# kjenike/panagram

Measured on AMD Instinct MI355X. Metric: anchored k-mers/sec building pan-kmer bitmap, higher is better.
Workload: dtype u64

## Files before the change

### panagram_amd/csrc/pg_anchor.hip

```cpp
#include "pg_kernels.h"

#ifndef PG_ANCHOR_PART
#define PG_ANCHOR_PART -1
#endif
#define PG_HAS_PART(n) (PG_ANCHOR_PART == -1 || PG_ANCHOR_PART == (n))
#define PG_MAIN_PART (PG_ANCHOR_PART <= 0)
#if defined(PG_PHASE_TIMING) && PG_ANCHOR_PART != -1
#error "a -DPG_PHASE_TIMING build keeps its counters in one device variable: compile pg_anchor.hip as ONE unit (PG_ANCHOR_PART unset)"
#endif

namespace pg {

hipError_t probe_part0(hipStream_t s, uint32_t w, uint32_t ntiles, const SubTable &st, const uint64_t *seqw, const uint32_t *nmw, const uint32_t *has_n,
                       const SeqDesc *sd, const AnchorDesc *ad, const uint32_t *tile_contig, const uint32_t *sched, uint32_t tile_base, uint8_t *out1,
                       uint32_t nbytes, const RowCols &rc, int rowmode, const FuseArgs *fuse);
hipError_t probe_part1(hipStream_t s, uint32_t w, uint32_t ntiles, const SubTable &st, const uint64_t *seqw, const uint32_t *nmw, const uint32_t *has_n,
                       const SeqDesc *sd, const AnchorDesc *ad, const uint32_t *tile_contig, const uint32_t *sched, uint32_t tile_base, uint8_t *out1,
                       uint32_t nbytes, const RowCols &rc, int rowmode, const FuseArgs *fuse);
hipError_t probe_part2(hipStream_t s, uint32_t w, uint32_t ntiles, const SubTable &st, const uint64_t *seqw, const uint32_t *nmw, const uint32_t *has_n,
                       const SeqDesc *sd, const AnchorDesc *ad, const uint32_t *tile_contig, const uint32_t *sched, uint32_t tile_base, uint8_t *out1,
                       uint32_t nbytes, const RowCols &rc, int rowmode, const FuseArgs *fuse);
hipError_t insert_part0(hipStream_t s, uint32_t win, uint32_t ntiles, const SubTable &st, int w, uint32_t bits, uint32_t count_mode, const uint64_t *seqw,
                        const uint32_t *nmw, const uint32_t *has_n, const SeqDesc *sd, const uint32_t *tile0, uint32_t ncontigs,
                        unsigned long long *counters, uint32_t max_probe);
hipError_t insert_part1(hipStream_t s, uint32_t win, uint32_t ntiles, const SubTable &st, int w, uint32_t bits, uint32_t count_mode, const uint64_t *seqw,
                        const uint32_t *nmw, const uint32_t *has_n, const SeqDesc *sd, const uint32_t *tile0, uint32_t ncontigs,
                        unsigned long long *counters, uint32_t max_probe);
hipError_t insert_part2(hipStream_t s, uint32_t win, uint32_t ntiles, const SubTable &st, int w, uint32_t bits, uint32_t count_mode, const uint64_t *seqw,
                        const uint32_t *nmw, const uint32_t *has_n, const SeqDesc *sd, const uint32_t *tile0, uint32_t ncontigs,
                        unsigned long long *counters, uint32_t max_probe);
hipError_t preload_part1();
hipError_t preload_part2();

constexpr int PROBE_SEQW = ((PROBE_TILE + 31) / 32 + 6 + 3) & ~3;
#ifndef PG_ABLATE
#define PG_ABLATE 0
#endif
constexpr uint32_t PROBE_SEQ_BASES = 32u * PROBE_SEQW;
#ifdef PG_PHASE_TIMING
__device__ unsigned long long pg_phase_cycles[1024 * 16];
#define PG_PH_DECL uint32_t ph_acc[12] = {0, 0, 0, 0, 0, 0, 0, 0, 0, 0, 0, 0}; uint32_t ph_t = (uint32_t)__builtin_readcyclecounter();
#define PG_PH(i) { const uint32_t ph_n = (uint32_t)__builtin_readcyclecounter(); ph_acc[i] += ph_n - ph_t; ph_t = ph_n; }
#define PG_PH_FLUSH { if (threadIdx.x == 0) { for (int ph_i = 0; ph_i < 9; ++ph_i) atomicAdd(&pg_phase_cycles[(blockIdx.x & 1023u) * 16u + ph_i], (unsigned long long)ph_acc[ph_i]); atomicAdd(&pg_phase_cycles[(blockIdx.x & 1023u) * 16u + 9], 1ull); atomicAdd(&pg_phase_cycles[(blockIdx.x & 1023u) * 16u + 10], (unsigned long long)ph_acc[10]); } }
#else
#define PG_PH_DECL
#define PG_PH(i)
#define PG_PH_FLUSH
#endif
__device__ __forceinline__ uint64_t revcomp_window(const uint64_t *rw, uint32_t p, uint64_t kmask, uint32_t rcb) {
    return extract_bases32(reinterpret_cast<const uint32_t *>(rw), rcb - p) & kmask;
}

__device__ __forceinline__ void stage_chunk(uint4 *line, uint32_t slot, int slots, const uint4 v) {
    uint2 *const p = reinterpret_cast<uint2 *>(line);
    p[slot] = make_uint2(v.x, v.y);
    p[slots + slot] = make_uint2(v.z, v.w);
}
template <bool TWO, int SLOTS>
__device__ __forceinline__ int scan_line_lds(const uint4 *line, uint64_t key, uint32_t &m0, uint32_t &m1) {
    uint64_t kk[SLOTS];
#pragma unroll
    for (int j = 0; j < SLOTS / 2; ++j) {
        const uint4 v = line[j];
        kk[2 * j] = (uint64_t)v.x | ((uint64_t)v.y << 32);
        kk[2 * j + 1] = (uint64_t)v.z | ((uint64_t)v.w << 32);
    }
    constexpr uint32_t SLOT_BYTES = 8u, MASK0 = 8u * SLOTS;
    m0 = m1 = 0;
    if constexpr (SLOTS == 8) {
        unsigned long long e[8];
#pragma unroll
        for (int sl = 0; sl < 8; ++sl) e[sl] = __builtin_amdgcn_ballot_w64(kk[sl] == key);
        const unsigned long long b0 = e[1] | e[3] | e[5] | e[7], b1 = e[2] | e[3] | e[6] | e[7], b2 = e[4] | e[5] | e[6] | e[7];
        const unsigned long long any = b0 | b1 | b2 | e[0];
        const bool hit = __builtin_amdgcn_inverse_ballot_w64(any);
#if PG_ABLATE == 6
        if (hit) m0 = (uint32_t)b0 | 1u;
        return hit ? 1 : (kk[SLOTS - 1] == EMPTY_KEY ? 0 : -1);
#elif PG_ABLATE == 7
        m0 = (uint32_t)(kk[0] ^ kk[1] ^ kk[2] ^ kk[3] ^ kk[4] ^ kk[5] ^ kk[6] ^ kk[7]) | 1u;
        return (kk[0] ^ kk[3]) == key ? -1 : 1;
#endif
        if (hit) {
            const uint32_t off = (__builtin_amdgcn_inverse_ballot_w64(b0) ? SLOT_BYTES : 0u) | (__builtin_amdgcn_inverse_ballot_w64(b1) ? 2u * SLOT_BYTES : 0u) |
                                 (__builtin_amdgcn_inverse_ballot_w64(b2) ? 4u * SLOT_BYTES : 0u);
            if constexpr (TWO) {
                const uint2 mk = *reinterpret_cast<const uint2 *>(reinterpret_cast<const uint8_t *>(line) + off + MASK0);
                m0 = mk.x;
                m1 = mk.y;
            } else {
                m0 = *reinterpret_cast<const uint32_t *>(reinterpret_cast<const uint8_t *>(line) + off + MASK0);
            }
        }
        return hit ? 1 : (kk[SLOTS - 1] == EMPTY_KEY ? 0 : -1);
    } else {
        int hit = -1;
#pragma unroll
        for (int sl = 0; sl < SLOTS; ++sl) hit = (kk[sl] == key) ? sl : hit;
        if (hit >= 0) {
            const uint2 mk = *reinterpret_cast<const uint2 *>(reinterpret_cast<const uint8_t *>(line) + (uint32_t)hit * SLOT_BYTES + MASK0);
            m0 = mk.x;
            if (TWO) m1 = mk.y;
        }
        return hit >= 0 ? 1 : (kk[SLOTS - 1] == EMPTY_KEY ? 0 : -1);
    }
}


template <bool TWO, int SLOTS>
__device__ __forceinline__ int scan_line_global(const SubTable &st, uint32_t b, uint64_t key, uint32_t &m0, uint32_t &m1) {
    const uint4 *line = reinterpret_cast<const uint4 *>(st.buckets + (uint64_t)b * (16 * SLOTS));
    uint4 v[SLOTS];
#pragma unroll
    for (int sl = 0; sl < SLOTS; ++sl) v[sl] = line[sl];
    m0 = m1 = 0;
#pragma unroll
    for (int sl = 0; sl < SLOTS; ++sl) {
        const uint64_t kk = (uint64_t)v[sl].x | ((uint64_t)v[sl].y << 32);
        const bool hit = (kk == key);
        m0 = hit ? v[sl].z : m0;
        if (TWO) m1 = hit ? v[sl].w : m1;
    }
    const uint64_t last = (uint64_t)v[SLOTS - 1].x | ((uint64_t)v[SLOTS - 1].y << 32);
    return (m0 | m1) ? 1 : (last == EMPTY_KEY ? 0 : -1);
}

template <bool TWO, int SLOTS>
__device__ __forceinline__ void lane_chase(const SubTable &st, uint64_t key, uint32_t level, uint32_t b, uint32_t step,
                                           uint32_t &m0, uint32_t &m1) {
    for (uint64_t n = 0; n < st.nbuckets + GROUP_CHAIN; ++n) {
        if (scan_line_global<TWO, SLOTS>(st, b, key, m0, m1) >= 0) return;
        level = min(level + 1, GROUP_CHAIN + 1);
        advance_line(key, level, st.nbuckets, b, step);
    }
    m0 = m1 = 0;
}

template <bool FIRST = false>
__device__ __forceinline__ int scan_keys16_lds(const uint4 *line, uint64_t key, uint32_t &slot1) {
    uint64_t kk[16];
#pragma unroll
    for (int c = 0; c < 8; ++c) {
        const uint4 v = line[c];
        kk[2 * c] = (uint64_t)v.x | ((uint64_t)v.y << 32);
        kk[2 * c + 1] = (uint64_t)v.z | ((uint64_t)v.w << 32);
    }
    unsigned long long e[16];
#pragma unroll
    for (int sl = 0; sl < 16; ++sl) e[sl] = __builtin_amdgcn_ballot_w64(kk[sl] == key);
    if constexpr (FIRST) {
        unsigned long long seen = e[0];
#pragma unroll
        for (int sl = 1; sl < 16; ++sl) {
            const unsigned long long m = e[sl];
            e[sl] = m & ~seen;
            seen |= m;
        }
    }
    unsigned long long b[4] = {0, 0, 0, 0}, any = e[0];
#pragma unroll
    for (int sl = 1; sl < 16; ++sl) {
        any |= e[sl];
#pragma unroll
        for (int bit = 0; bit < 4; ++bit)
            if (sl & (1 << bit)) b[bit] |= e[sl];
    }
    const bool hit = __builtin_amdgcn_inverse_ballot_w64(any);
    slot1 = 0;
    if (hit)
        slot1 = 1u + ((__builtin_amdgcn_inverse_ballot_w64(b[0]) ? 1u : 0u) | (__builtin_amdgcn_inverse_ballot_w64(b[1]) ? 2u : 0u) |
                      (__builtin_amdgcn_inverse_ballot_w64(b[2]) ? 4u : 0u) | (__builtin_amdgcn_inverse_ballot_w64(b[3]) ? 8u : 0u));
    return hit ? 1 : (kk[15] == EMPTY_KEY ? 0 : -1);
}

__device__ __forceinline__ void lane_chase_wide(const SubTable &st, uint64_t key, uint32_t level, uint32_t b, uint32_t step,
                                                uint32_t &hline, uint32_t &slot1) {
    hline = slot1 = 0;
    for (uint64_t n = 0; n < st.nbuckets + GROUP_CHAIN; ++n) {
        const uint4 *line = reinterpret_cast<const uint4 *>(st.buckets + (uint64_t)b * (8u * SPLIT_KEYS));
        uint4 v[8];
#pragma unroll
        for (int c = 0; c < 8; ++c) v[c] = line[c];
        uint32_t found = 0;
#pragma unroll
        for (int c = 0; c < 8; ++c) {
            if (((uint64_t)v[c].x | ((uint64_t)v[c].y << 32)) == key) found = 2 * c + 1;
            if (((uint64_t)v[c].z | ((uint64_t)v[c].w << 32)) == key) found = 2 * c + 2;
        }
        if (found) {
            hline = b;
            slot1 = found;
            return;
        }
        if (((uint64_t)v[7].z | ((uint64_t)v[7].w << 32)) == EMPTY_KEY) return;
        level = min(level + 1, GROUP_CHAIN + 1);
        advance_line(key, level, st.nbuckets, b, step);
    }
}

template <int NW>
struct __attribute__((packed, aligned(4))) WordsN {
    uint32_t w[NW];
};
template <int NW, bool NT = false>
__device__ __forceinline__ void copy_words(const uint32_t *src, uint8_t *dst, bool hit) {
    WordsN<NW> v;
#pragma unroll
    for (int i = 0; i < NW; ++i) v.w[i] = 0;
    if (hit) v = *reinterpret_cast<const WordsN<NW> *>(src);
    if constexpr (NW == 4 && NT) {
        typedef uint32_t u32x4 __attribute__((ext_vector_type(4)));
        u32x4 q = {v.w[0], v.w[1], v.w[2], v.w[3]};
        __builtin_nontemporal_store(q, reinterpret_cast<u32x4 *>(dst));
    } else {
        *reinterpret_cast<WordsN<NW> *>(dst) = v;
    }
}
template <int NS>
__device__ __forceinline__ void copy_words_tail(const uint32_t *src, uint8_t *dst, bool hit, uint32_t tail) {
    WordsN<NS + 1> v;
#pragma unroll
    for (int i = 0; i <= NS; ++i) v.w[i] = 0;
    if (hit) v = *reinterpret_cast<const WordsN<NS + 1> *>(src);
    if constexpr (NS > 0) {
        WordsN<NS> o;
#pragma unroll
        for (int i = 0; i < NS; ++i) o.w[i] = v.w[i];
        *reinterpret_cast<WordsN<NS> *>(dst) = o;
    }
    if (NS > 0 && tail > 1) {
        struct __attribute__((packed)) U32 { uint32_t v; };
        reinterpret_cast<U32 *>(dst + 4 * NS + tail - 4)->v = __builtin_amdgcn_alignbit(v.w[NS], v.w[NS > 0 ? NS - 1 : 0], 8u * tail);
    } else {
        for (uint32_t bb = 0; bb < tail; ++bb) dst[4 * NS + bb] = (uint8_t)(v.w[NS] >> (8 * bb));
    }
}
__device__ __forceinline__ void store_row_wide(const uint8_t *masks, uint32_t W, uint32_t nbytes, uint8_t *row, uint32_t hline,
                                               uint32_t slot1) {
    const bool hit = slot1 != 0;
    const uint32_t *mp = reinterpret_cast<const uint32_t *>(masks) + ((uint64_t)hline * SPLIT_KEYS + (slot1 - 1u)) * W;
    uint32_t d = 0;
    const uint32_t full = nbytes / 4;
    const uint32_t tail = nbytes % 4;
    if (nbytes == 16) {
        copy_words<4, true>(mp, row, hit);
        return;
    }
    for (; d + 4 <= full; d += 4) copy_words<4>(mp + d, row + 4 * d, hit);
    if (!tail) {
        if (full - d == 3) copy_words<3>(mp + d, row + 4 * d, hit);
        else if (full - d == 2) copy_words<2>(mp + d, row + 4 * d, hit);
        else if (full - d == 1) copy_words<1>(mp + d, row + 4 * d, hit);
    } else {
        if (full - d == 3) copy_words_tail<3>(mp + d, row + 4 * d, hit, tail);
        else if (full - d == 2) copy_words_tail<2>(mp + d, row + 4 * d, hit, tail);
        else if (full - d == 1) copy_words_tail<1>(mp + d, row + 4 * d, hit, tail);
        else copy_words_tail<0>(mp + d, row + 4 * d, hit, tail);
    }
}

__device__ __forceinline__ int scan_keys_inl(const uint4 *line, uint64_t key, uint32_t S, uint32_t &slot1) {
    uint64_t kk[6];
#pragma unroll
    for (int c = 0; c < 3; ++c) {
        const uint4 v = line[c];
        kk[2 * c] = (uint64_t)v.x | ((uint64_t)v.y << 32);
        kk[2 * c + 1] = (uint64_t)v.z | ((uint64_t)v.w << 32);
    }
    const bool six = S >= 6u;
    slot1 = (six && kk[5] == key) ? 6u : 0u;
#pragma unroll
    for (int sl = 4; sl >= 0; --sl) slot1 = (kk[sl] == key) ? (uint32_t)(sl + 1) : slot1;
    const uint64_t last = six ? kk[5] : kk[4];
    return slot1 ? 1 : (last == EMPTY_KEY ? 0 : -1);
}
__device__ __forceinline__ void masks_inl(const uint4 *line, uint32_t S, uint32_t W, uint32_t slot, uint32_t (&w)[4]) {
    const WordsN<4> v = *reinterpret_cast<const WordsN<4> *>(reinterpret_cast<const uint8_t *>(line) + 8u * S + 4u * W * slot);
    w[0] = v.w[0], w[1] = v.w[1], w[2] = v.w[2], w[3] = v.w[3];
}
template <int NS>
__device__ __forceinline__ void store_words_tail(const uint32_t (&v)[4], uint8_t *dst, uint32_t tail) {
    if (NS == 3 && tail == 0) {
        typedef uint32_t u32x3 __attribute__((ext_vector_type(3), aligned(4)));
        u32x3 q = {v[0], v[1], v[2]};
        __builtin_nontemporal_store(q, reinterpret_cast<u32x3 *>(dst));
        return;
    }
    WordsN<NS> o;
#pragma unroll
    for (int i = 0; i < NS; ++i) o.w[i] = v[i];
    *reinterpret_cast<WordsN<NS> *>(dst) = o;
    if (tail > 1) {
        struct __attribute__((packed)) U32 { uint32_t v; };
        reinterpret_cast<U32 *>(dst + 4 * NS + tail - 4)->v = __builtin_amdgcn_alignbit(v[NS & 3], v[NS - 1], 8u * tail);
    } else if (tail == 1) {
        dst[4 * NS] = (uint8_t)v[NS & 3];
    }
}
__device__ __forceinline__ void store_row_regs(uint8_t *row, uint32_t nbytes, const uint32_t (&w)[4]) {
    if (nbytes == 16) {
        typedef uint32_t u32x4 __attribute__((ext_vector_type(4)));
        u32x4 q = {w[0], w[1], w[2], w[3]};
        __builtin_nontemporal_store(q, reinterpret_cast<u32x4 *>(row));
    } else if (nbytes >= 12) {
        store_words_tail<3>(w, row, nbytes - 12u);
    } else {
        store_words_tail<2>(w, row, nbytes - 8u);
    }
}
__device__ __forceinline__ void store_row_fused(uint8_t *row, uint32_t nbytes, const uint32_t (&w)[4], uint32_t nxt) {
    const uint32_t t = nbytes & 3u;
    const uint32_t keep = (1u << (8u * t)) - 1u;
    typedef uint32_t u32x4u __attribute__((ext_vector_type(4), aligned(1)));
    typedef uint32_t u32x3u __attribute__((ext_vector_type(3), aligned(1)));
    if (nbytes > 12u) {
        u32x4u q = {w[0], w[1], w[2], (w[3] & keep) | (nxt << (8u * t))};
        __builtin_nontemporal_store(q, reinterpret_cast<u32x4u *>(row));
    } else {
        u32x3u q = {w[0], w[1], (w[2] & keep) | (nxt << (8u * t))};
        __builtin_nontemporal_store(q, reinterpret_cast<u32x3u *>(row));
    }
}
__device__ __forceinline__ void lane_chase_inl(const SubTable &st, uint64_t key, uint32_t level, uint32_t b, uint32_t step, uint32_t (&w)[4]) {
// ... 157 lines not shown
        __syncthreads();
        if (level > LEVELS) {
            for (uint32_t e = lane; e < qn; e += 64) {
                uint32_t m0, m1;
                const uint64_t key = canonical_from_le(extract_bases(sw, q_pl[e]), k);
                if constexpr (WIDE && INL) {
                    uint32_t rw4[4];
                    lane_chase_inl(st, key, (uint32_t)level, q_line[e], q_step[e], rw4);
                    if (rw4[0] | rw4[1] | rw4[2] | rw4[3]) store_row_regs(tile_rows + (uint64_t)q_pl[e] * nbytes, nbytes, rw4);
                } else if constexpr (WIDE) {
                    lane_chase_wide(st, key, (uint32_t)level, q_line[e], q_step[e], m0, m1);
                    if (m1) store_row_wide(st.masks, st.W, nbytes, tile_rows + (uint64_t)q_pl[e] * nbytes, m0, m1);
                } else {
                    lane_chase<TWO, SLOTS>(st, key, (uint32_t)level, q_line[e], q_step[e], m0, m1);
                    if constexpr (ROWMODE == 3) cols_or_position(reinterpret_cast<unsigned long long *>(tile_rows), q_pl[e], m0);
                    else if (m0 | m1) store_row<ROWMODE>(tile_rows + (uint64_t)q_pl[e] * nbytes, m0, m1, rc);
                }
            }
            break;
        }
        uint32_t kept = 0;
        for (uint32_t i0 = 0; i0 < qn; i0 += 64) {
            const uint32_t e = i0 + lane;
            const bool act = e < qn;
            const uint32_t ec = act ? e : qn - 1;
            uint32_t line = q_line[ec], step = q_step[ec];
            if (GROUP_CHAIN > 1 && level == 1) {
                step = step_of_group(step, st.nbuckets);
                line = next_line(line, step, st.nbuckets);
            }
            const uint32_t pl = q_pl[ec];
            const uint64_t kmask = kmer_mask(k);
            const uint64_t X = extract_bases32(reinterpret_cast<const uint32_t *>(sw), pl) & kmask;
            const uint64_t key = canonical_from_xb(X, revcomp_window(rw, pl, kmask, PROBE_SEQ_BASES - (uint32_t)k), k);
            const uint32_t prev_line = lane_up1(line);
            const bool leader = act && (lane == 0 || line != prev_line);
            const unsigned long long lmask = __builtin_amdgcn_ballot_w64(leader);
            const uint32_t rid = lanes_le_index(lmask, 0u);
            const uint32_t nruns = (uint32_t)__popcll(lmask);
            uint32_t m0 = 0, m1 = 0;
            [[maybe_unused]] uint32_t rw4[4] = {0, 0, 0, 0};
            int rcode = 0;
            const uint32_t padline = lmask ? (uint32_t)__builtin_amdgcn_readlane((int)line, __builtin_ctzll(lmask)) : 0u;
            for (uint32_t r0 = 0; r0 < nruns; r0 += MAXRUN) {
                const uint32_t nl = min((uint32_t)MAXRUN, nruns - r0);
                if (lane < MAXRUN) lines_w[lane] = padline;
                if (leader && rid - r0 < nl) lines_w[rid - r0] = line;
                __syncthreads();
                uint4 v[STAGE_ITERS];
                uint32_t ln[STAGE_ITERS];
#pragma unroll
                for (int u = 0; u < STAGE_ITERS; ++u) ln[u] = lines_w[u * (64 / SLOTS) + lane / SLOTS];
#pragma unroll
                for (int u = 0; u < STAGE_ITERS; ++u) v[u] = *reinterpret_cast<const uint4 *>(chunk_base + (uint64_t)ln[u] * lbytes);
#pragma unroll
                for (int u = 0; u < STAGE_ITERS; ++u) {
                    const uint32_t idx = u * 64 + lane;
                    if constexpr (WIDE) buf[(idx / SLOTS) * LDS_LINE_U4 + (idx % SLOTS)] = v[u];
                    else stage_chunk(buf + (idx / SLOTS) * LDS_LINE_U4, idx % SLOTS, SLOTS, v[u]);
                }
                __syncthreads();
                if (act && rid - r0 < nl) {
                    if constexpr (WIDE && INL) {
                        rcode = scan_keys_inl(buf + (rid - r0) * LDS_LINE_U4, key, st.slots, m1);
                        if (m1) masks_inl(buf + (rid - r0) * LDS_LINE_U4, st.slots, st.W, m1 - 1u, rw4);
                    } else if constexpr (WIDE) {
                        rcode = scan_keys16_lds(buf + (rid - r0) * LDS_LINE_U4, key, m1);
                        m0 = line;
                    } else {
                        rcode = scan_line_lds<TWO, SLOTS>(buf + (rid - r0) * LDS_LINE_U4, key, m0, m1);
                    }
                }
                __syncthreads();
            }
            const bool again = act && rcode < 0;
            if constexpr (WIDE && INL) {
                if (act && m1) store_row_regs(tile_rows + (uint64_t)pl * nbytes, nbytes, rw4);
            } else if constexpr (WIDE) {
                if (act && m1) store_row_wide(st.masks, st.W, nbytes, tile_rows + (uint64_t)pl * nbytes, m0, m1);
            } else {
                if constexpr (ROWMODE == 3) {
                    if (act) cols_or_position(reinterpret_cast<unsigned long long *>(tile_rows), pl, m0);
                } else {
                    if (act && (m0 | m1)) store_row<ROWMODE>(tile_rows + (uint64_t)pl * nbytes, m0, m1, rc);
                }
            }
            const unsigned long long kmask2 = __builtin_amdgcn_ballot_w64(again);
            if (again) {
                const uint32_t slot = set_lane_index(kmask2, kept);
                uint32_t nl2 = line, ns2 = step;
                if constexpr (LEVELS + 1 < (int)GROUP_CHAIN) nl2 = next_line(line, step, st.nbuckets);
                else advance_line(key, (uint32_t)level + 1, st.nbuckets, nl2, ns2);
                q_line[slot] = nl2;
                q_step[slot] = ns2;
                q_pl[slot] = (uint16_t)pl;
            }
            kept += (uint32_t)__popcll(kmask2);
            __syncthreads();
        }
        qn = kept;
    }
}

#ifndef PG_FUSE_LOAD_SC1
#define PG_FUSE_LOAD_SC1 1
#endif
typedef const __attribute__((address_space(1))) uint8_t *GlobalBytes;
template <int NW>
__device__ __forceinline__ void fuse_load_row(GlobalBytes base, uint32_t off, uint32_t (&w)[NW]) {
    GlobalBytes p = base + off;
#if PG_FUSE_LOAD_SC1
#pragma unroll
    for (int i = 0; i + 1 < NW; i += 2) {
        const unsigned long long v = __hip_atomic_load(reinterpret_cast<const __attribute__((address_space(1))) unsigned long long *>(p + 4 * i), __ATOMIC_RELAXED,
                                                       __HIP_MEMORY_SCOPE_AGENT);
        w[i] = (uint32_t)v, w[i + 1] = (uint32_t)(v >> 32);
    }
    if constexpr (NW & 1)
        w[NW - 1] = __hip_atomic_load(reinterpret_cast<const __attribute__((address_space(1))) uint32_t *>(p + 4 * (NW - 1)), __ATOMIC_RELAXED, __HIP_MEMORY_SCOPE_AGENT);
#else
    const WordsN<NW> v = *reinterpret_cast<const __attribute__((address_space(1))) WordsN<NW> *>(p);
#pragma unroll
    for (int i = 0; i < NW; ++i) w[i] = v.w[i];
#endif
}
__device__ __forceinline__ void fuse_flush_word(const uint32_t (&pl)[5], uint32_t *out16, int lane) {
    uint32_t R[16];
#pragma unroll
    for (int q = 0; q < 8; ++q) {
        uint32_t v = 0;
#pragma unroll
        for (int i = 0; i < 5; ++i) v |= ((pl[i] >> q) & 0x01010101u) << i;
        R[2 * q] = v & 0x00FF00FFu;
        R[2 * q + 1] = (v >> 8) & 0x00FF00FFu;
    }
#define PG_XCHG(HALF, BIT)                                                  \
    {                                                                       \
        const bool up = (lane & BIT) != 0;                                  \
        _Pragma("unroll") for (int i = 0; i < HALF; ++i) {                  \
            const uint32_t send = up ? R[i] : R[i + HALF];                  \
            const uint32_t keep = up ? R[i + HALF] : R[i];                  \
            R[i] = keep + (uint32_t)__shfl_xor((int)send, BIT);             \
        }                                                                   \
    }
    PG_XCHG(8, 32)
    PG_XCHG(4, 16)
    PG_XCHG(2, 8)
    PG_XCHG(1, 4)
#undef PG_XCHG
    R[0] += (uint32_t)__shfl_xor((int)R[0], 2);
    R[0] += (uint32_t)__shfl_xor((int)R[0], 1);
    if ((lane & 3) == 0) {
        const uint32_t idx = (uint32_t)lane >> 2;
        out16[(idx >> 1) + ((idx & 1u) ? 8u : 0u)] = R[0];
    }
}
template <int NWP, bool LASTPASS>
__device__ __forceinline__ void tile_statistics_pass(uint32_t *Hc, GlobalBytes rs, uint32_t npos, uint32_t nbytes, uint32_t woff,
                                                     uint32_t keep_last, uint32_t split, uint32_t N, uint32_t (&pcs)[4], uint32_t *cs_out, int lane) {
    const uint32_t N1 = N + 1u;
    uint32_t ones[NWP], twos[NWP], fours[NWP], eights[NWP], sixteens[NWP], hold4[NWP], hold8[NWP];
#pragma unroll
    for (int w = 0; w < NWP; ++w) ones[w] = twos[w] = fours[w] = eights[w] = sixteens[w] = hold4[w] = hold8[w] = 0;
    uint32_t nx[4][NWP];
    auto request = [&](int g, uint32_t (&dst)[4][NWP]) __attribute__((always_inline)) {
#pragma unroll
        for (int i = 0; i < 4; ++i) {
            const uint32_t r = (uint32_t)(4 * g + i) * 64u + (uint32_t)lane;
            fuse_load_row<NWP>(rs, min(r, npos - 1u) * nbytes + woff, dst[i]);
        }
    };
    request(0, nx);
#pragma unroll
    for (int g = 0; g < 4; ++g) {
        uint32_t rw[4][NWP];
#pragma unroll
        for (int i = 0; i < 4; ++i)
#pragma unroll
            for (int w = 0; w < NWP; ++w) rw[i][w] = nx[i][w];
        if (g < 3) request(g + 1, nx);
        uint32_t pc4 = pcs[g];
#pragma unroll
        for (int i = 0; i < 4; ++i) {
            const uint32_t r = (uint32_t)(4 * g + i) * 64u + (uint32_t)lane;
            const uint32_t vmask = (uint32_t)((int32_t)(r - npos) >> 31);
            if (LASTPASS) rw[i][NWP - 1] &= keep_last;
            uint32_t pc = 0;
#pragma unroll
            for (int w = 0; w < NWP; ++w) {
                rw[i][w] &= vmask;
                pc += (uint32_t)__popc(rw[i][w]);
            }
            if (LASTPASS) {
                pc = min(pc + ((pc4 >> (8 * i)) & 0xFFu), N);
                const uint32_t idx = pc + (N1 & (uint32_t)((int32_t)(split - 1u - r) >> 31));
                atomicAdd(&Hc[idx], vmask & 1u);
            } else {
                pc4 += pc << (8 * i);
            }
        }
        if (!LASTPASS) pcs[g] = pc4;
#pragma unroll
        for (int w = 0; w < NWP; ++w) {
            uint32_t u = ones[w] ^ rw[0][w];
            const uint32_t c2a = (ones[w] & rw[0][w]) | (u & rw[1][w]);
            ones[w] = u ^ rw[1][w];
            u = ones[w] ^ rw[2][w];
            const uint32_t c2b = (ones[w] & rw[2][w]) | (u & rw[3][w]);
            ones[w] = u ^ rw[3][w];
            u = twos[w] ^ c2a;
            const uint32_t c4 = (twos[w] & c2a) | (u & c2b);
            twos[w] = u ^ c2b;
            if ((g & 1) == 0) {
                hold4[w] = c4;
            } else {
                u = fours[w] ^ hold4[w];
                const uint32_t c8 = (fours[w] & hold4[w]) | (u & c4);
                fours[w] = u ^ c4;
                if (g == 1) {
                    hold8[w] = c8;
                } else {
                    u = eights[w] ^ hold8[w];
                    sixteens[w] = (eights[w] & hold8[w]) | (u & c8);
                    eights[w] = u ^ c8;
                }
            }
        }
    }
#pragma unroll
    for (int w = 0; w < NWP; ++w) {
        const uint32_t pl[5] = {ones[w], twos[w], fours[w], eights[w], sixteens[w]};
        fuse_flush_word(pl, cs_out + 16 * w, lane);
    }
}

template <int NW>
__device__ __forceinline__ void tile_statistics(uint32_t *H, const uint8_t *tile_rows, uint32_t npos, uint32_t nbytes, const AnchorDesc &a,
                                                uint32_t tile_start, uint32_t tile, const FuseArgs &fo, int lane) {
    const uint32_t N = fo.ngenomes, N1 = N + 1u, hw = fo.hw;
    const uint32_t nh = 2u * N1;
#ifdef PG_PHASE_TIMING
    uint32_t tph[5] = {0, 0, 0, 0, 0}, tph_t = (uint32_t)__builtin_readcyclecounter();
#define PG_TPH(i) { const uint32_t n_ = (uint32_t)__builtin_readcyclecounter(); tph[i] += n_ - tph_t; tph_t = n_; }
#else
#define PG_TPH(i)
#endif
    __builtin_amdgcn_s_waitcnt(0x0F70);
    __syncthreads();
    PG_TPH(0)
    const uint64_t base = reinterpret_cast<uint64_t>(tile_rows);
    GlobalBytes rs = reinterpret_cast<GlobalBytes>(((uint64_t)(uint32_t)__builtin_amdgcn_readfirstlane((int)(uint32_t)(base >> 32)) << 32) |
                                                   (uint32_t)__builtin_amdgcn_readfirstlane((int)(uint32_t)base));
    const uint32_t r100 = (100u - tile_start % 100u) % 100u + 100u * (uint32_t)lane;
    const bool want100 = fo.out100 != nullptr && r100 < npos;
    uint32_t w100[NW];
    fuse_load_row<NW>(rs, min(r100, npos - 1u) * nbytes, w100);
    for (uint32_t i = lane; i < 4u * nh; i += 64) H[i] = 0;
    const uint64_t bin_end = ((uint64_t)(tile_start / a.binlen) + 1u) * a.binlen;
    const uint32_t split = (uint32_t)min((uint64_t)npos, bin_end - tile_start);
    const uint32_t keep = (nbytes & 3u) ? ((1u << (8u * (nbytes & 3u))) - 1u) : ~0u;
    uint32_t *const Hc = H + ((uint32_t)lane & 3u) * nh;
    uint32_t *cs_out = fo.tile_cs + (uint64_t)tile * fo.csw;
    uint32_t pcs[4] = {0, 0, 0, 0};
    __syncthreads();
    PG_TPH(1)
    if constexpr (NW <= 2) {
        tile_statistics_pass<NW, true>(Hc, rs, npos, nbytes, 0u, keep, split, N, pcs, cs_out, lane);
        PG_TPH(2)
    } else {
        tile_statistics_pass<2, false>(Hc, rs, npos, nbytes, 0u, ~0u, split, N, pcs, cs_out, lane);
        PG_TPH(2)
        tile_statistics_pass<NW - 2, true>(Hc, rs, npos, nbytes, 8u, keep, split, N, pcs, cs_out + 32, lane);
    }
    if (want100) {
        uint8_t *dst = fo.out100 + a.out100_off + (uint64_t)((tile_start + r100) / 100u) * nbytes;
#pragma unroll
        for (int i = 0; i < NW; ++i)
#pragma unroll
            for (int b = 0; b < 4; ++b)
                if ((uint32_t)(4 * i + b) < nbytes) dst[4 * i + b] = (uint8_t)(w100[i] >> (8 * b));
    }
    __syncthreads();
    PG_TPH(3)
    uint32_t *th = fo.tile_hist + (uint64_t)tile * hw;
    for (uint32_t i = lane; i < hw; i += 64) {
        const uint32_t lo = H[2u * i] + H[nh + 2u * i] + H[2u * nh + 2u * i] + H[3u * nh + 2u * i];
        const uint32_t hi = H[2u * i + 1u] + H[nh + 2u * i + 1u] + H[2u * nh + 2u * i + 1u] + H[3u * nh + 2u * i + 1u];
        th[i] = lo | (hi << 16);
    }
    PG_TPH(4)
#ifdef PG_PHASE_TIMING
    if (lane == 0)
        for (int i = 0; i < 5; ++i) atomicAdd(&pg_phase_cycles[(blockIdx.x & 1023u) * 16u + 11 + i], (unsigned long long)tph[i]);
#endif
#undef PG_TPH
}

template <bool TWO, int ROWMODE, int SLOTS, bool WIDE>
constexpr bool probe_pipelined = SLOTS == 8 && !WIDE && ROWMODE != 3 && (ROWMODE == 1 || ROWMODE >= 4 || TWO);
template <int W_C, bool TWO, int ROWMODE, int SLOTS, bool M64, bool WIDE = false, bool INL = false, bool FUSE = false>
__global__ __launch_bounds__(64, ((probe_pipelined<TWO, ROWMODE, SLOTS, WIDE> || INL || FUSE) ? 8 : 1))
__attribute__((amdgpu_num_sgpr(80))) void k_probe(const SubTable st, const uint64_t *__restrict__ seqw,
                                              const uint32_t *__restrict__ nmw, const uint32_t *__restrict__ has_n,
                                              const SeqDesc *__restrict__ sd, const AnchorDesc *__restrict__ ad,
                                              const uint32_t *__restrict__ tile_contig,
                                              const uint32_t *__restrict__ sched, uint32_t tile_base,
                                              uint8_t *__restrict__ out1, uint32_t nbytes, const RowCols rc, const FuseArgs fo) {
    constexpr int LDS_LINE_U4 = SLOTS + 1;
    constexpr int MAXRUN = PROBE_MAXRUN;
    constexpr int STAGE_ITERS = (MAXRUN * SLOTS + 63) / 64;
    constexpr int BUF_U4 = ((STAGE_ITERS * 64 + SLOTS - 1) / SLOTS) * LDS_LINE_U4;
    constexpr int OFF_RW = PROBE_SEQW * 8, OFF_NW = OFF_RW + (PROBE_SEQW + 1) * 8, OFF_LW = OFF_NW + PROBE_SEQW * 4;
    constexpr int QCAP = PROBE_QCAP;
    constexpr int OFF_BUF = (OFF_LW + MAXRUN * 4 + 15) & ~15, OFF_QL = OFF_BUF + BUF_U4 * 16, OFF_QS = OFF_QL + QCAP * 4;
    constexpr int OFF_QP = OFF_QS + QCAP * 4, LDS_BYTES = OFF_QP + QCAP * 2;
    static_assert(OFF_LW <= 1020 || PROBE_TILE > 1024, "the sequence words must stay within reach of ds_read2_b32's offsets");
    __shared__ __attribute__((aligned(16))) uint8_t lds[LDS_BYTES];
    uint64_t *const sw = reinterpret_cast<uint64_t *>(lds);
    uint64_t *const rw = reinterpret_cast<uint64_t *>(lds + OFF_RW);
    uint32_t *const nw = reinterpret_cast<uint32_t *>(lds + OFF_NW);
    uint32_t(*const lines_w)[MAXRUN] = reinterpret_cast<uint32_t(*)[MAXRUN]>(lds + OFF_LW);
    uint4(*const buf)[BUF_U4] = reinterpret_cast<uint4(*)[BUF_U4]>(lds + OFF_BUF);
    uint32_t *const q_line = reinterpret_cast<uint32_t *>(lds + OFF_QL);
    uint32_t *const q_step = reinterpret_cast<uint32_t *>(lds + OFF_QS);
    uint16_t *const q_pl = reinterpret_cast<uint16_t *>(lds + OFF_QP);
    PG_PH_DECL
    const int lane = threadIdx.x;
    const int k = (int)st.k;
    if constexpr (W_C != 0) __builtin_assume(k >= 20 && k <= 32);
    const uint32_t tile = sched ? sched[blockIdx.x + tile_base] : blockIdx.x + tile_base;
    const uint32_t c = tile_contig[tile];
    const AnchorDesc a = ad[c];
    const SeqDesc s = sd[c];
    const uint32_t tile_start = (tile - a.tile0) * PROBE_TILE;
    const uint32_t npos = min((uint32_t)PROBE_TILE, a.nkmers - tile_start);
    const bool hasn = has_n[c] != 0;

    for (int i = lane; i < PROBE_SEQW; i += 64) {
        const uint64_t wi = (uint64_t)(tile_start >> 5) + i;
        const uint64_t wv = wi < s.nwords ? seqw[s.seq_off + wi] : 0ull;
        sw[i] = wv;
        rw[PROBE_SEQW - 1 - i] = pair_reverse64(~wv);
        nw[i] = (hasn && wi < s.nwords) ? nmw[s.seq_off + wi] : 0u;
    }
    if (lane == 0) rw[PROBE_SEQW] = 0;
    __syncthreads();

    const uint64_t kmask = W_C ? (((uint64_t)(k == 32 ? ~0u : ((1u << (2 * k - 32)) - 1u)) << 32) | 0xFFFFFFFFull) : kmer_mask(k);
    const uint32_t rcb = PROBE_SEQ_BASES - (uint32_t)k;
    constexpr int HALO = W_C ? W_C - 1 : 0;
    constexpr bool CARRY = W_C >= 2;
    constexpr bool CUT = W_C != 0;
    const uint32_t m = W_C ? (uint32_t)k - W_C + 1 : 0;
    const uint64_t mm64 = (m >= 32) ? ~0ull : ((1ull << (2 * (m ? m : 1))) - 1);
    __shared__ unsigned long long cols[ROWMODE == 3 ? TILE_SLOTS * COLS_G : 1];
    if constexpr (ROWMODE == 3) {
        for (uint32_t i = lane; i < TILE_SLOTS * COLS_G; i += 64) cols[i] = 0;
        __syncthreads();
    }
#if PG_ABLATE == 9 || PG_ABLATE == 10
    uint8_t *tile_rows = out1 + (uint64_t)(blockIdx.x & 255u) * PROBE_TILE * nbytes;
#else
    uint8_t *tile_rows = ROWMODE == 3 ? reinterpret_cast<uint8_t *>(cols) : out1 + a.out_off + (uint64_t)tile_start * nbytes;
#endif
    uint32_t qn = 0;

    const uint8_t *chunk_base = st.buckets + (uint32_t)(lane % SLOTS) * 16u;
    const uint32_t lbytes = INL ? st.layout * 64u : st.slots * (WIDE ? 8u : 16u);

    struct Front {
        uint64_t key;
        uint32_t grp, line, rid, nruns, padline;
        uint32_t adv;
        uint32_t ln[STAGE_ITERS];
        unsigned long long rmask, amask, lmask;
    };
    auto carry_at = [&](const uint32_t b0) __attribute__((always_inline)) {
        uint32_t y = ~0u;
        if constexpr (CARRY) {
            const uint32_t q = b0 + (uint32_t)min(lane, HALO - 1);
            const uint64_t fa = extract_bases32(reinterpret_cast<const uint32_t *>(sw), q) & mm64;
            const uint64_t fr = extract_bases32(reinterpret_cast<const uint32_t *>(rw), PROBE_SEQ_BASES - q - m) & mm64;
            const uint32_t h = M64 ? mmer_rank(fa < fr ? fa : fr) : mz_order(min((uint32_t)fa, (uint32_t)fr));
            y = h;
        }
        return y;
    };
    uint32_t carry = ~0u;
    auto front = [&](const uint32_t b0) __attribute__((always_inline)) {
        Front f;
        const int32_t pl = (int32_t)(b0 + lane);
        f.rmask = __builtin_amdgcn_ballot_w64(pl < (int32_t)npos);
        const uint32_t pq = (uint32_t)pl;
        const uint64_t X = extract_bases32(reinterpret_cast<const uint32_t *>(sw), pq) & kmask;
        const uint64_t B = revcomp_window(rw, pq, kmask, rcb);
        f.key = ~(X > B ? X : B) & kmask;
        f.amask = f.rmask;
        if (hasn) f.amask &= __builtin_amdgcn_ballot_w64(extract_nmask(nw, pq, k) == 0);
        [[maybe_unused]] uint32_t own = 0;
        if (W_C) {
            constexpr uint32_t off = (uint32_t)HALO;
            if constexpr (!M64) {
                const uint32_t mm32 = (uint32_t)mm64;
                const uint32_t fa = __builtin_amdgcn_alignbit((uint32_t)(X >> 32), (uint32_t)X, 2 * off) & mm32;
                const uint32_t fr = __builtin_amdgcn_alignbit((uint32_t)(B >> 32), (uint32_t)B, 2 * (HALO - off)) & mm32;
                f.grp = mz_order(min(fa, fr));
            } else {
                const uint64_t fa = (X >> (2 * off)) & mm64;
                const uint64_t fr = (B >> (2 * (HALO - off))) & mm64;
                f.grp = mmer_rank(fa < fr ? fa : fr);
            }
#ifdef PG_DUMMY_VALU
            {
                uint32_t dm = f.grp;
#pragma unroll
                for (int i = 0; i < PG_DUMMY_VALU; ++i) asm volatile("v_alignbit_b32 %0, %0, %1, 3" : "+v"(dm) : "v"((uint32_t)lane));
                if (dm == 0x12345u && lane == 77) out1[0] = 1;
            }
#endif
            if constexpr (CARRY) {
                own = f.grp;
                uint32_t suffix = __builtin_amdgcn_inverse_ballot_w64((1ull << HALO) - 1ull) ? carry : ~0u;
                f.grp = sliding_min_suffix<W_C >= 2 ? W_C : 2>(f.grp, suffix);
                f.grp = min(f.grp, suffix);
            } else {
                f.grp = sliding_min<W_C ? W_C : 1>(f.grp);
            }
        } else {
            f.grp = group_of_key(f.key);
        }
        f.line = home_of_group(f.grp, st.nbuckets);
        f.lmask = f.amask & (~(f.amask << 1) | differs_from_lane_below(f.line));
        f.rid = run_ids(f.lmask);
        uint32_t lanes_kept = 64u;
        if constexpr (CUT) {
            const unsigned long long keep = __builtin_amdgcn_sicmp((int32_t)f.rid, MAXRUN, 40 );
            f.amask &= keep;
            f.rmask &= keep;
            f.lmask &= keep;
            lanes_kept = (uint32_t)__popcll(keep);
        }
        f.adv = lanes_kept;
        if constexpr (CARRY) {
            carry = (uint32_t)__builtin_amdgcn_ds_bpermute((int)(((uint32_t)lane << 2) + ((lanes_kept - HALO) << 2)), (int)own);
        }
        f.nruns = (uint32_t)__popcll(f.lmask);
        int first_run;
        asm("s_ff1_i32_b64 %0, %1" : "=s"(first_run) : "s"(f.lmask));
        f.padline = (uint32_t)__builtin_amdgcn_readlane((int)f.line, first_run & 63);
#if PG_ABLATE == 3
        if (f.line != 0xDEADBEEFu) f.nruns = 0;
#endif
        const bool leader = __builtin_amdgcn_inverse_ballot_w64(f.lmask);
        if (lane < MAXRUN) lines_w[0][lane] = f.padline;
        if (leader && f.rid < (uint32_t)MAXRUN) lines_w[0][f.rid] = f.line;
        __syncthreads();
#pragma unroll
        for (int it = 0; it < STAGE_ITERS; ++it) f.ln[it] = lines_w[0][it * (64 / SLOTS) + lane / SLOTS];
        return f;
    };
    struct Lines {
        uint4 v[STAGE_ITERS];
    };
    auto issue = [&](const Front &f, const uint32_t r0) __attribute__((always_inline)) {
        Lines L;
        uint32_t ln[STAGE_ITERS];
        if (r0 != 0u) {
            const uint32_t nl = min((uint32_t)MAXRUN, f.nruns - r0);
            const bool leader = __builtin_amdgcn_inverse_ballot_w64(f.lmask);
            if (lane < MAXRUN) lines_w[0][lane] = f.padline;
            if (leader && f.rid - r0 < nl) lines_w[0][f.rid - r0] = f.line;
            __syncthreads();
        }
#pragma unroll
        for (int it = 0; it < STAGE_ITERS; ++it) {
            if (r0 != 0u) ln[it] = lines_w[0][it * (64 / SLOTS) + lane / SLOTS];
            else ln[it] = f.ln[it];
#if PG_ABLATE == 1
            ln[it] &= 511u;
#endif
        }
#pragma unroll
        for (int it = 0; it < STAGE_ITERS; ++it) L.v[it] = *reinterpret_cast<const uint4 *>(chunk_base + (uint64_t)ln[it] * lbytes);
        return L;
    };
    auto back = [&](const Front &f, const Lines &L, const uint32_t b0, auto &&after_staging) __attribute__((always_inline)) {
        const bool act = __builtin_amdgcn_inverse_ballot_w64(f.amask), inrange = __builtin_amdgcn_inverse_ballot_w64(f.rmask);
        const int32_t pl = (int32_t)(b0 + lane);
        uint32_t m0 = 0, m1 = 0;
        [[maybe_unused]] uint32_t rw4[4] = {0, 0, 0, 0};
        int rcode = 0;
        auto stage = [&](const Lines &S) __attribute__((always_inline)) {
            uint4 *const mine = buf[0] + ((uint32_t)lane / SLOTS) * LDS_LINE_U4;
#pragma unroll
            for (int it = 0; it < STAGE_ITERS; ++it) {
                if constexpr (WIDE) mine[it * (64 / SLOTS) * LDS_LINE_U4 + ((uint32_t)lane % SLOTS)] = S.v[it];
                else stage_chunk(mine + it * (64 / SLOTS) * LDS_LINE_U4, (uint32_t)lane % SLOTS, SLOTS, S.v[it]);
            }
            __syncthreads();
        };
        auto scan = [&](const uint32_t r0) __attribute__((always_inline)) {
            const uint32_t nl = min((uint32_t)MAXRUN, f.nruns - r0);
#if PG_ABLATE == 5
            if (act && f.rid - r0 < nl) {
                rcode = 1;
                m0 = m1 = reinterpret_cast<const uint32_t *>(buf[0] + (f.rid - r0) * LDS_LINE_U4)[2];
            }
#else
            if (act && f.rid - r0 < nl) {
                if constexpr (WIDE && INL) {
                    rcode = scan_keys_inl(buf[0] + (f.rid - r0) * LDS_LINE_U4, f.key, st.slots, m1);
                    if (m1) masks_inl(buf[0] + (f.rid - r0) * LDS_LINE_U4, st.slots, st.W, m1 - 1u, rw4);
                } else if constexpr (WIDE) {
                    rcode = scan_keys16_lds(buf[0] + (f.rid - r0) * LDS_LINE_U4, f.key, m1);
                    m0 = f.line;
                } else {
                    rcode = scan_line_lds<TWO, SLOTS>(buf[0] + (f.rid - r0) * LDS_LINE_U4, f.key, m0, m1);
                }
            }
#endif
            __syncthreads();
        };
        PG_PH(1)
        __builtin_amdgcn_s_waitcnt(0x0F70);
        PG_PH(2)
        stage(L);
        PG_PH(3)
        after_staging();
        PG_PH(4)
        scan(0u);
        PG_PH(5)
        if constexpr (!CUT)
        for (uint32_t r0 = MAXRUN; r0 < f.nruns; r0 += MAXRUN) {
            const Lines X = issue(f, r0);
            __builtin_amdgcn_s_waitcnt(0x0F70);
            stage(X);
            scan(r0);
        }
        const unsigned long long omask = f.amask & __builtin_amdgcn_sicmp(rcode, 0, 40);
        const bool ovf = __builtin_amdgcn_inverse_ballot_w64(omask);
        if (omask) {
            uint32_t step, nx;
            if constexpr (GROUP_CHAIN == 1) {
                key_sequence(f.key, st.nbuckets, nx, step);
            } else {
                step = f.grp;
                nx = f.line;
            }
            const uint32_t slot = set_lane_index(omask, qn);
            if (ovf) {
                q_line[slot] = nx;
                q_step[slot] = step;
                q_pl[slot] = (uint16_t)pl;
            }
            qn += (uint32_t)__popcll(omask);
        }
        PG_PH(10)
        if constexpr (WIDE && INL) {
            const bool fuse = (nbytes & 3u) != 0u && b0 + (uint32_t)__popcll(f.rmask) < npos;
            if (fuse) {
                const uint32_t mine = inrange ? rw4[0] : 0u;
                const uint32_t nxt = (uint32_t)__builtin_amdgcn_update_dpp(0, (int)mine, 0x130 , 0xf, 0xf, true);
                if (inrange) store_row_fused(tile_rows + (uint64_t)(uint32_t)pl * nbytes, nbytes, rw4, nxt);
            } else if (inrange) {
                store_row_regs(tile_rows + (uint64_t)(uint32_t)pl * nbytes, nbytes, rw4);
            }
        } else if constexpr (WIDE) {
#if PG_ABLATE == 2
            if (inrange && m0 == 0xDEADBEEFu && m1 == 77u)
#elif PG_ABLATE == 8 || PG_ABLATE == 10
            if (m1) m0 = 0, m1 = 1;
            if (inrange)
#else
            if (st.W == 4u && (nbytes & 3u) != 0u && b0 + (uint32_t)__popcll(f.rmask) < npos) {
                uint32_t v4[4] = {0, 0, 0, 0};
                if (inrange && m1) {
                    const WordsN<4> g = *reinterpret_cast<const WordsN<4> *>(reinterpret_cast<const uint32_t *>(st.masks) + ((uint64_t)m0 * SPLIT_KEYS + (m1 - 1u)) * 4u);
                    v4[0] = g.w[0], v4[1] = g.w[1], v4[2] = g.w[2], v4[3] = g.w[3];
                }
                const uint32_t nxt = (uint32_t)__builtin_amdgcn_update_dpp(0, (int)v4[0], 0x130 , 0xf, 0xf, true);
                if (inrange) store_row_fused(tile_rows + (uint64_t)(uint32_t)pl * nbytes, nbytes, v4, nxt);
            } else if (inrange)
#endif
                store_row_wide(st.masks, st.W, nbytes, tile_rows + (uint64_t)(uint32_t)pl * nbytes, m0, m1);
        } else if constexpr (ROWMODE == 3) {
            const uint32_t w0 = b0 >> 6, sh = b0 & 63u;
            for (uint32_t j = 0; j < rc.col0; ++j) {
                const unsigned long long shifted = __ballot(inrange && ((m0 >> j) & 1u));
                if (lane == 0 && shifted) {
                    cols[w0 * COLS_G + j] |= shifted << sh;
                    if (sh && (shifted >> (64u - sh))) cols[(w0 + 1) * COLS_G + j] |= shifted >> (64u - sh);
                }
            }
        } else {
            if (ROWMODE == 6 && b0 + (uint32_t)__popcll(f.rmask) < npos) {
                const uint32_t mine = inrange ? m0 : 0u;
                const uint32_t nxt = (uint32_t)__builtin_amdgcn_update_dpp(0, (int)mine, 0x130 , 0xf, 0xf, true);
                struct __attribute__((packed)) U32 { uint32_t v; };
                if (inrange) reinterpret_cast<U32 *>(tile_rows + (uint32_t)pl * 3u)->v = (m0 & 0xFFFFFFu) | (nxt << 24);
            } else if constexpr (ROWMODE == 6) {
                const uint32_t nxt = (uint32_t)__builtin_amdgcn_update_dpp(0, (int)m0, 0x130 , 0xf, 0xf, false);
                const uint32_t o4 = (uint32_t)reinterpret_cast<uintptr_t>(tile_rows) & 3u;
                const uint32_t j = ((uint32_t)pl - o4) & 3u;
                const uint32_t lo = (nxt << 24) | (m0 & 0xFFFFFFu);
                const uint32_t dw = __builtin_amdgcn_alignbit(nxt >> 8, lo, 8u * j);
                const unsigned long long nextin = f.rmask >> 1;
                const unsigned long long dmask = f.rmask & nextin & __builtin_amdgcn_ballot_w64(j != 3u);
                const unsigned long long fmask = f.rmask & (1ull | ~nextin);
                uint8_t *row = tile_rows + (uint32_t)pl * 3u;
                if (__builtin_amdgcn_inverse_ballot_w64(dmask)) *reinterpret_cast<uint32_t *>(row + j) = dw;
                if (__builtin_amdgcn_inverse_ballot_w64(fmask)) store_row<ROWMODE>(row, m0, m1, rc);
            } else
#if PG_ABLATE == 2
            if (inrange && m0 == 0xDEADBEEFu)
#else
            if (ROWMODE == 0 && TWO && rc.words == 3u && nbytes >= 5u && b0 + (uint32_t)__popcll(f.rmask) < npos) {
                const uint32_t mine = inrange ? m0 : 0u;
                const uint32_t nxt = (uint32_t)__builtin_amdgcn_update_dpp(0, (int)mine, 0x130 , 0xf, 0xf, true);
                if (inrange) {
                    typedef uint32_t u32x2u __attribute__((ext_vector_type(2), aligned(1)));
                    const uint32_t t8 = 8u * (nbytes - 4u);
                    u32x2u q = {m0, (m1 & ((1u << t8) - 1u)) | (nxt << t8)};
                    *reinterpret_cast<u32x2u *>(tile_rows + (uint32_t)pl * nbytes) = q;
                }
            } else if (inrange)
#endif
                store_row<ROWMODE>(tile_rows + (ROWMODE == 1 ? (uint32_t)pl : ROWMODE == 4 ? (uint32_t)pl * 4u : ROWMODE == 5 ? (uint32_t)pl * 2u : ROWMODE == 6 ? (uint32_t)pl * 3u : (uint32_t)pl * nbytes), m0, m1, rc);
        }
        PG_PH(6)
    };
    constexpr bool PIPE = probe_pipelined<TWO, ROWMODE, SLOTS, WIDE>;
    constexpr int LEVELS = (W_C >= 6 && !TWO && !WIDE && PROBE_STAGED_LEVELS > 1) ? 1 : PROBE_STAGED_LEVELS;
    static_assert(QCAP >= 128, "an early drain must leave room for a batch");
    constexpr uint32_t QROOM = QCAP - 64;
    uint32_t b0 = 0;
    if constexpr (PIPE) {
        Lines L;
#pragma unroll
        for (int it = 0; it < STAGE_ITERS; ++it) L.v[it] = make_uint4(0, 0, 0, 0);
        PG_PH(0)
        carry = carry_at(0u);
        Front cur = front(0u);
        L = issue(cur, 0u);
        for (;;) {
            PG_PH(7)
            const uint32_t b1 = b0 + cur.adv;
            const bool more = b1 < npos;
            Front nxt = cur;
            __builtin_amdgcn_sched_barrier(0);
            if (more) nxt = front(b1);
            __builtin_amdgcn_sched_barrier(0);
            back(cur, L, b0, [&]() __attribute__((always_inline)) {
                if (more) L = issue(nxt, 0u);
            });
            __builtin_amdgcn_sched_barrier(0);
            b0 = b1;
            if (!more || qn > QROOM) break;
            cur = nxt;
        }
    } else {
        {
            carry = carry_at(0u);
            const Front f = front(0u);
            const Lines L = issue(f, 0u);
            back(f, L, 0u, [] {});
            b0 = f.adv;
        }
        while (b0 < npos && qn <= QROOM) {
            const Front f = front(b0);
            const Lines L = issue(f, 0u);
            back(f, L, b0, [] {});
            b0 += f.adv;
        }
    }
    PG_PH(7)
    for (;;) {
        drain_queue<TWO, ROWMODE, SLOTS, MAXRUN, WIDE, LEVELS, INL>(st, qn, sw, rw, q_line, q_step, q_pl, lines_w[0], buf[0], tile_rows, nbytes, rc, lane);
        qn = 0;
        if (b0 >= npos) break;
        __syncthreads();
        carry = carry_at(b0);
        while (b0 < npos && qn <= QROOM) {
            const Front f = front(b0);
            const Lines L = issue(f, 0u);
            back(f, L, b0, [] {});
            b0 += f.adv;
        }
    }
    PG_PH(8)
    PG_PH_FLUSH
    if constexpr (FUSE) {
        static_assert(ROWMODE != 1 && ROWMODE != 3 && LDS_BYTES >= 4 * 4 * 2 * 129, "fused statistics: rows of 2..16 bytes; four copies of 2 x 129 histogram counters in LDS");
        const AnchorDesc *ad2 = ad;
        const uint32_t *tc2 = tile_contig, *sched2 = sched;
        asm volatile("" : "+s"(ad2), "+s"(tc2), "+s"(sched2));
        const uint32_t tile2 = sched2 ? sched2[blockIdx.x + tile_base] : blockIdx.x + tile_base;
        const AnchorDesc a2 = ad2[tc2[tile2]];
        if (a2.binlen >= (uint32_t)PROBE_TILE) {
            const uint32_t ts2 = (tile2 - a2.tile0) * PROBE_TILE;
            const uint32_t np2 = min((uint32_t)PROBE_TILE, a2.nkmers - ts2);
            const uint8_t *rows2 = out1 + a2.out_off + (uint64_t)ts2 * nbytes;
            uint32_t *H = reinterpret_cast<uint32_t *>(lds);
            if constexpr (WIDE) {
                if (nbytes <= 12u) tile_statistics<3>(H, rows2, np2, nbytes, a2, ts2, tile2, fo, lane);
                else tile_statistics<4>(H, rows2, np2, nbytes, a2, ts2, tile2, fo, lane);
            } else {
                tile_statistics<TWO ? 2 : 1>(H, rows2, np2, nbytes, a2, ts2, tile2, fo, lane);
            }
        }
    }
    if constexpr (ROWMODE == 3) {
        __syncthreads();
        const uint32_t width = nbytes, trel = tile - tile_base;
        unsigned long long *dst = reinterpret_cast<unsigned long long *>(out1) + (uint64_t)trel * TILE_SLOTS * width;
        for (uint32_t i = lane; i < TILE_SLOTS * width; i += 64) dst[i] = cols[(i / width) * COLS_G + i % width];
    }
}

constexpr int INSERT_QCAP = 256;

template <bool COUNT, bool CLAIM = true>
__device__ __forceinline__ int wave_insert_batch(const SubTable &st, bool valid, uint64_t key, uint32_t grp, int w, uint32_t bits,
                                                 uint32_t max_probe, int lane) {
    const uint32_t kstride = key_stride(st), slots = st.slots;
    uint32_t b = home_of_group(grp, st.nbuckets), step = step_of_group(grp, st.nbuckets), probes = 0;
    int s = -1;
    bool done = !valid, fresh = false;
    int r = 0;
    auto shfl64 = [](uint64_t v, int src) __attribute__((always_inline)) {
        return (uint64_t)(uint32_t)__shfl((int)(uint32_t)v, src) | ((uint64_t)(uint32_t)__shfl((int)(uint32_t)(v >> 32), src) << 32);
    };
    auto resolve = [&](uint32_t sl, bool claimed) __attribute__((always_inline)) {
        uint32_t *mp = mask_ptr(st, b, sl, (uint32_t)w);
        if (COUNT) {
            if (*mp < 0xFFFFFF00u) atomicAdd(mp, bits);
        } else if (claimed) {
            *reinterpret_cast<volatile uint32_t *>(mp) = bits;
        } else {
            const uint32_t cur = *mp;
            if ((cur & bits) != bits) *reinterpret_cast<volatile uint32_t *>(mp) = cur | bits;
        }
        r = claimed ? 1 : 0;
        done = true;
    };
    while (__ballot(!done)) {
        if (!done && s >= (int)slots) {
            if (++probes >= max_probe) {
                done = true;
                r = -1;
            } else {
                advance_line(key, probes, st.nbuckets, b, step);
                s = -1;
            }
        }
        if (!done && s < 0) {
            uint8_t *base = st.buckets + (uint64_t)b * line_bytes(st);
            int hit = -1, fr = -1;
            for (uint32_t s0 = 0; s0 < slots; s0 += 8) {
                uint64_t kk[8];
#pragma unroll
                for (int i = 0; i < 8; ++i) {
                    kk[i] = __hip_atomic_load(reinterpret_cast<unsigned long long *>(base + kstride * (s0 + i)), __ATOMIC_RELAXED,
                                              __HIP_MEMORY_SCOPE_AGENT);
                    if (s0 + (uint32_t)i >= slots) kk[i] = TOMB_KEY;
                }
                int h8 = -1, f8 = -1;
#pragma unroll
                for (int i = 7; i >= 0; --i) {
                    h8 = (kk[i] == key) ? i : h8;
                    f8 = (kk[i] == EMPTY_KEY) ? i : f8;
                }
                if (hit < 0 && h8 >= 0) hit = (int)s0 + h8;
                if (fr < 0 && f8 >= 0) fr = (int)s0 + f8;
            }
            if (hit >= 0) resolve((uint32_t)hit, false);
            else if (!CLAIM && fr >= 0) done = true;
            else {
                s = fr >= 0 ? fr : (int)slots;
                fresh = true;
            }
        }
        if constexpr (!CLAIM) continue;
        if (!COUNT) {
            const bool sp = !done && fresh && s < (int)slots;
            const unsigned long long spmask = __ballot(sp);
            if (spmask) {
                const uint64_t gaddr = sp ? reinterpret_cast<uint64_t>(key_ptr(st, b, (uint32_t)s)) : 0;
                const uint64_t gprev = (uint64_t)(uint32_t)__shfl_up((int)(uint32_t)gaddr, 1) | ((uint64_t)(uint32_t)__shfl_up((int)(uint32_t)(gaddr >> 32), 1) << 32);
                const bool gl = sp && (lane == 0 || gprev != gaddr);
                const unsigned long long glmask = __ballot(gl);
                const unsigned long long below = glmask & ((2ull << lane) - 1ull);
                const int g0 = below ? 63 - __builtin_clzll(below) : lane;
                const unsigned long long ends = (glmask | ~spmask) & ~((2ull << g0) - 1ull);
                const int gend = ends ? __builtin_ctzll(ends) : 64;
                const uint32_t mm = sp ? min((uint32_t)(gend - g0), slots - (uint32_t)s) : 0u;
                const int t = s + (lane - g0);
                const bool part = sp && t < (int)slots;
                uint64_t content = 0;
                bool won = false;
                if (part) {
                    const unsigned long long cur = atomicCAS(key_ptr(st, b, (uint32_t)t), (unsigned long long)EMPTY_KEY, (unsigned long long)key);
                    won = cur == EMPTY_KEY;
                    content = won ? key : cur;
                }
                int pos = -1;
                for (uint32_t i = 0; i < slots; ++i) {
                    const uint64_t c = shfl64(content, min(g0 + (int)i, 63));
                    if (i < mm && pos < 0 && c == key) pos = s + (int)i;
                }
                if (sp) {
                    if (pos >= 0) {
                        const bool mine = part && won && pos == t;
                        if (part && won && pos != t) *reinterpret_cast<volatile unsigned long long *>(key_ptr(st, b, (uint32_t)t)) = TOMB_KEY;
                        resolve((uint32_t)pos, mine);
                    } else {
                        s += (int)mm;
                    }
                }
            }
        }
        fresh = false;
        const bool want = !done && s >= 0 && s < (int)slots;
        unsigned long long *kp = want ? key_ptr(st, b, (uint32_t)s) : nullptr;
        const uint64_t addr = reinterpret_cast<uint64_t>(kp);
        const uint64_t prev = (uint64_t)(uint32_t)__shfl_up((int)(uint32_t)addr, 1) | ((uint64_t)(uint32_t)__shfl_up((int)(uint32_t)(addr >> 32), 1) << 32);
        const bool leader = want && (lane == 0 || prev != addr);
        uint64_t content = 0;
        bool won = false;
        if (leader) {
            const unsigned long long cur = atomicCAS(kp, (unsigned long long)EMPTY_KEY, (unsigned long long)key);
            won = cur == EMPTY_KEY;
            content = won ? key : cur;
        }
        const unsigned long long lmask = __builtin_amdgcn_ballot_w64(leader);
        if (__ballot(want)) {
            const unsigned long long below = lmask & ((2ull << lane) - 1ull);
            const int mine = below ? 63 - __builtin_clzll(below) : lane;
            const uint64_t got = (uint64_t)(uint32_t)__shfl((int)(uint32_t)content, mine) | ((uint64_t)(uint32_t)__shfl((int)(uint32_t)(content >> 32), mine) << 32);
            if (want) {
                if (got == key) resolve((uint32_t)s, leader && won);
                else ++s;
            }
        }
    }
    return r;
}

template <int W_C, bool M64>
__global__ __launch_bounds__(64) void k_insert_tile(const SubTable st, int w, uint32_t bits, uint32_t count_mode,
                                                    const uint64_t *__restrict__ seqw, const uint32_t *__restrict__ nmw,
                                                    const uint32_t *__restrict__ has_n, const SeqDesc *__restrict__ sd,
                                                    const uint32_t *__restrict__ tile0, uint32_t ncontigs,
                                                    unsigned long long *__restrict__ counters, uint32_t max_probe) {
    constexpr int SLOTS = 8;
    constexpr int LDS_LINE_U4 = SLOTS + 1;
    constexpr int STAGE_ITERS = (PROBE_MAXRUN * SLOTS + 63) / 64;
    __shared__ uint64_t sw[PROBE_SEQW];
    __shared__ uint64_t rw[PROBE_SEQW + 1];
    __shared__ uint32_t nw[PROBE_SEQW];
    __shared__ uint32_t lines_w[PROBE_MAXRUN];
    __shared__ uint4 buf[((STAGE_ITERS * 64 + SLOTS - 1) / SLOTS) * LDS_LINE_U4];
    __shared__ uint32_t q_grp[INSERT_QCAP];
    __shared__ uint16_t q_pl[INSERT_QCAP];
    const int lane = threadIdx.x;
    const int k = (int)st.k;
    const bool split = st.layout == LAYOUT_SPLIT;
    const bool update_only = (count_mode & 2u) != 0;
    count_mode &= 1u;
    const uint32_t tile = blockIdx.x;
    uint32_t c = 0;
    {
        uint32_t lo = 0, hi = ncontigs;
        while (hi - lo > 1) {
            const uint32_t mid = (lo + hi) >> 1;
            if (tile0[mid] <= tile) lo = mid;
            else hi = mid;
        }
        c = lo;
    }
    const SeqDesc s = sd[c];
    const uint32_t nkmers = (uint32_t)(s.len - (uint64_t)k + 1);
    const uint32_t tile_start = (tile - tile0[c]) * PROBE_TILE;
    const uint32_t npos = min((uint32_t)PROBE_TILE, nkmers - tile_start);
    const bool hasn = has_n[c] != 0;
    for (int i = lane; i < PROBE_SEQW; i += 64) {
        const uint64_t wi = (uint64_t)(tile_start >> 5) + i;
        const uint64_t wv = wi < s.nwords ? seqw[s.seq_off + wi] : 0ull;
        sw[i] = wv;
        rw[PROBE_SEQW - 1 - i] = pair_reverse64(~wv);
        nw[i] = (hasn && wi < s.nwords) ? nmw[s.seq_off + wi] : 0u;
    }
    if (lane == 0) rw[PROBE_SEQW] = 0;
    __syncthreads();
    const uint64_t kmask = W_C ? (((uint64_t)(k == 32 ? ~0u : ((1u << (2 * k - 32)) - 1u)) << 32) | 0xFFFFFFFFull) : kmer_mask(k);
    const uint32_t rcb = PROBE_SEQ_BASES - (uint32_t)k;
    constexpr int HALO = W_C ? W_C - 1 : 0;
    constexpr int STRIDE = 64 - HALO;
    const uint32_t m = W_C ? (uint32_t)k - W_C + 1 : 0;
    const uint64_t mm64 = (m >= 32) ? ~0ull : ((1ull << (2 * (m ? m : 1))) - 1);
    uint32_t qn = 0, claimed = 0;
    bool overflowed = false;

    auto drain = [&]() {
        __syncthreads();
        for (uint32_t e0 = 0; e0 < qn; e0 += 64) {
            const uint32_t e = e0 + lane;
            const bool valid = e < qn;
            const uint32_t ec = valid ? e : qn - 1;
            const uint64_t key = canonical_from_le(extract_bases32(reinterpret_cast<const uint32_t *>(sw), q_pl[ec]), k);
            const int r = update_only ? wave_insert_batch<false, false>(st, valid, key, q_grp[ec], w, bits, max_probe, lane)
                          : count_mode ? wave_insert_batch<true>(st, valid, key, q_grp[ec], w, bits, max_probe, lane)
                                       : wave_insert_batch<false>(st, valid, key, q_grp[ec], w, bits, max_probe, lane);
            overflowed |= __ballot(r < 0) != 0;
            claimed += (uint32_t)__popcll(__ballot(r > 0));
        }
        qn = 0;
        __syncthreads();
    };

    uint32_t adv = STRIDE;
    for (uint32_t b = 0; b < npos; b += adv) {
        const int32_t pl = (int32_t)(b + lane) - HALO;
        const bool inrange = pl >= (int32_t)b && pl < (int32_t)npos;
        const uint32_t pq = (uint32_t)max(pl, 0);
        const uint64_t X = extract_bases32(reinterpret_cast<const uint32_t *>(sw), pq) & kmask;
        const uint64_t B = revcomp_window(rw, pq, kmask, rcb);
        const uint64_t key = ~(X > B ? X : B) & kmask;
        bool act = inrange;
        if (hasn) act = act && (extract_nmask(nw, pq, k) == 0);
        uint32_t grp;
        if (W_C) {
            const uint32_t off = (uint32_t)(pl + HALO) - pq;
            if constexpr (!M64) {
                const uint32_t mm32 = (uint32_t)mm64;
                const uint32_t fa = __builtin_amdgcn_alignbit((uint32_t)(X >> 32), (uint32_t)X, 2 * off) & mm32;
                const uint32_t fr = __builtin_amdgcn_alignbit((uint32_t)(B >> 32), (uint32_t)B, 2 * (HALO - off)) & mm32;
                grp = mz_order(min(fa, fr));
            } else {
                const uint64_t fa = (X >> (2 * off)) & mm64;
                const uint64_t fr = (B >> (2 * (HALO - off))) & mm64;
                grp = mmer_rank(fa < fr ? fa : fr);
            }
            grp = sliding_min<W_C ? W_C : 1>(grp);
        } else {
            grp = group_of_key(key);
        }
        const uint32_t line = home_of_group(grp, st.nbuckets);
        const uint32_t prev_line = lane_up1(line);
        unsigned long long amask = __builtin_amdgcn_ballot_w64(act);
        unsigned long long lmask = amask & (~(amask << 1) | __builtin_amdgcn_ballot_w64(line != prev_line));
        const uint32_t rid = lanes_le_index(lmask, 0u);
        if constexpr (W_C != 0) {
            const unsigned long long keep = __builtin_amdgcn_sicmp((int32_t)rid, PROBE_MAXRUN, 40 );
            amask &= keep;
            lmask &= keep;
            act = __builtin_amdgcn_inverse_ballot_w64(amask);
            adv = (uint32_t)__popcll(keep) - HALO;
        }
        const bool leader = __builtin_amdgcn_inverse_ballot_w64(lmask);
        const uint32_t nruns = (uint32_t)__popcll(lmask);
        bool found = false, full = true;
        for (uint32_t r0 = 0; r0 < nruns; r0 += PROBE_MAXRUN) {
            const uint32_t nl = min((uint32_t)PROBE_MAXRUN, nruns - r0);
            if (leader && rid - r0 < nl) lines_w[rid - r0] = line;
            __syncthreads();
            uint4 v[STAGE_ITERS];
#pragma unroll
            for (int it = 0; it < STAGE_ITERS; ++it) {
                const uint32_t ls = min((uint32_t)(it * (64 / SLOTS) + lane / SLOTS), nl - 1u);
                v[it] = *reinterpret_cast<const uint4 *>(st.buckets + (((uint64_t)lines_w[ls] * 128u) | ((lane % SLOTS) * 16u)));
            }
#pragma unroll
            for (int it = 0; it < STAGE_ITERS; ++it) {
                const uint32_t idx = it * 64 + lane;
                buf[(idx / SLOTS) * LDS_LINE_U4 + (idx % SLOTS)] = v[it];
            }
            __syncthreads();
            if (act && rid - r0 < nl) {
                const uint4 *ln = buf + (rid - r0) * LDS_LINE_U4;
                uint32_t *mp = nullptr;
                uint32_t cur = 0;
                if (st.layout == LAYOUT_INLINE) {
                    uint32_t slot1;
                    full = scan_keys_inl(ln, key, st.slots, slot1) < 0;
                    if (slot1) {
                        found = true;
                        mp = mask_ptr(st, line, slot1 - 1u, (uint32_t)w);
                        cur = *reinterpret_cast<const volatile uint32_t *>(mp);
                    }
                } else if (split) {
                    uint32_t slot1;
                    full = scan_keys16_lds<true>(ln, key, slot1) < 0;
                    if (slot1) {
                        found = true;
                        mp = reinterpret_cast<uint32_t *>(st.masks) + ((uint64_t)line * SPLIT_KEYS + (slot1 - 1u)) * st.W + (uint32_t)w;
                        cur = *reinterpret_cast<const volatile uint32_t *>(mp);
                    }
                } else {
                    uint32_t m0, m1;
                    uint64_t kk[8];
#pragma unroll
                    for (int sl = 0; sl < 8; ++sl) kk[sl] = *reinterpret_cast<const uint64_t *>(ln + sl);
                    unsigned long long e[8];
#pragma unroll
                    for (int sl = 0; sl < 8; ++sl) e[sl] = __builtin_amdgcn_ballot_w64(kk[sl] == key);
                    {
                        unsigned long long seen = e[0];
#pragma unroll
                        for (int sl = 1; sl < 8; ++sl) {
                            const unsigned long long m = e[sl];
                            e[sl] = m & ~seen;
                            seen |= m;
                        }
                    }
                    const unsigned long long b0 = e[1] | e[3] | e[5] | e[7], b1 = e[2] | e[3] | e[6] | e[7], b2 = e[4] | e[5] | e[6] | e[7];
                    full = kk[7] != EMPTY_KEY;
                    (void)m0;
                    (void)m1;
                    if (__builtin_amdgcn_inverse_ballot_w64(b0 | b1 | b2 | e[0])) {
                        found = true;
                        const uint32_t off = (__builtin_amdgcn_inverse_ballot_w64(b0) ? 16u : 0u) | (__builtin_amdgcn_inverse_ballot_w64(b1) ? 32u : 0u) |
                                             (__builtin_amdgcn_inverse_ballot_w64(b2) ? 64u : 0u);
                        cur = *reinterpret_cast<const uint32_t *>(reinterpret_cast<const uint8_t *>(ln) + off + 8 + 4 * w);
                        mp = reinterpret_cast<uint32_t *>(st.buckets + (uint64_t)line * 128u + off + 8 + 4 * w);
                    }
                }
                if (found) {
                    if (count_mode) {
                        if (cur < 0xFFFFFF00u) atomicAdd(mp, bits);
                    } else if ((cur & bits) != bits) {
                        *reinterpret_cast<volatile uint32_t *>(mp) = cur | bits;
                    }
                }
            }
            __syncthreads();
        }
        const bool todo = act && !found && (!update_only || full);
        const unsigned long long tmask = __builtin_amdgcn_ballot_w64(todo);
        if (tmask) {
            if (qn + 64 > (uint32_t)INSERT_QCAP) drain();
            if (todo) {
                const uint32_t slot = lanes_le_index(tmask, qn);
                q_grp[slot] = grp;
                q_pl[slot] = (uint16_t)pl;
            }
            qn += (uint32_t)__popcll(tmask);
        }
    }
    if (qn) drain();
    if (lane == 0) {
        if (claimed) atomicAdd(&counters[0], (unsigned long long)claimed);
        if (overflowed) atomicOr(reinterpret_cast<unsigned int *>(&counters[1]), 1u);
    }
}

template <int W_C, bool TWO, int ROWMODE, int SLOTS>
static hipError_t probe_t(hipStream_t s, uint32_t ntiles, const SubTable &st, const uint64_t *seqw, const uint32_t *nmw,
                          const uint32_t *has_n, const SeqDesc *sd, const AnchorDesc *ad, const uint32_t *tile_contig,
                          const uint32_t *sched, uint32_t tile_base, uint8_t *out1, uint32_t nbytes, const RowCols &rc, const FuseArgs *fuse) {
    const bool m64 = W_C && st.m > 16;
    if constexpr (SLOTS == 8 && ROWMODE != 1 && ROWMODE != 3) {
        if (fuse) {
            if (m64)
                hipLaunchKernelGGL((k_probe<W_C, TWO, ROWMODE, SLOTS, true, false, false, true>), dim3(ntiles), dim3(64), 0, s, st, seqw, nmw, has_n, sd, ad,
                                   tile_contig, sched, tile_base, out1, nbytes, rc, *fuse);
            else
                hipLaunchKernelGGL((k_probe<W_C, TWO, ROWMODE, SLOTS, false, false, false, true>), dim3(ntiles), dim3(64), 0, s, st, seqw, nmw, has_n, sd, ad,
                                   tile_contig, sched, tile_base, out1, nbytes, rc, *fuse);
            return hipGetLastError();
        }
    }
    if (fuse) return hipErrorInvalidValue;
    const FuseArgs none = {nullptr, nullptr, nullptr, 0, 0, 0};
    if (m64)
        hipLaunchKernelGGL((k_probe<W_C, TWO, ROWMODE, SLOTS, true>), dim3(ntiles), dim3(64), 0, s, st, seqw, nmw, has_n, sd, ad,
                           tile_contig, sched, tile_base, out1, nbytes, rc, none);
    else
        hipLaunchKernelGGL((k_probe<W_C, TWO, ROWMODE, SLOTS, false>), dim3(ntiles), dim3(64), 0, s, st, seqw, nmw, has_n, sd, ad,
                           tile_contig, sched, tile_base, out1, nbytes, rc, none);
    return hipGetLastError();
}

template <int W_C>
static hipError_t probe_w(hipStream_t s, uint32_t ntiles, const SubTable &st, const uint64_t *seqw, const uint32_t *nmw,
                          const uint32_t *has_n, const SeqDesc *sd, const AnchorDesc *ad, const uint32_t *tile_contig,
                          const uint32_t *sched, uint32_t tile_base, uint8_t *out1, uint32_t nbytes, const RowCols &rc, int rowmode,
                          const FuseArgs *fuse = nullptr) {
#define PG_A s, ntiles, st, seqw, nmw, has_n, sd, ad, tile_contig, sched, tile_base, out1, nbytes, rc, fuse
#define PG_K s, st, seqw, nmw, has_n, sd, ad, tile_contig, sched, tile_base, out1, nbytes, rc
    const FuseArgs none = {nullptr, nullptr, nullptr, 0, 0, 0};
    const bool m64 = W_C && st.m > 16;
    if (st.layout == LAYOUT_INLINE || st.layout == LAYOUT_SPLIT) {
        const bool inl = st.layout == LAYOUT_INLINE;
        if (fuse && (nbytes > 16u || !PG_FUSE_WIDE)) return hipErrorInvalidValue;
        if (inl) {
            if (fuse) {
#if PG_FUSE_WIDE
                if (m64) hipLaunchKernelGGL((k_probe<W_C, false, 0, 8, true, true, true, true>), dim3(ntiles), dim3(64), 0, PG_K, *fuse);
                else hipLaunchKernelGGL((k_probe<W_C, false, 0, 8, false, true, true, true>), dim3(ntiles), dim3(64), 0, PG_K, *fuse);
#endif
            } else {
                if (m64) hipLaunchKernelGGL((k_probe<W_C, false, 0, 8, true, true, true>), dim3(ntiles), dim3(64), 0, PG_K, none);
                else hipLaunchKernelGGL((k_probe<W_C, false, 0, 8, false, true, true>), dim3(ntiles), dim3(64), 0, PG_K, none);
            }
        } else {
            if (fuse) {
#if PG_FUSE_WIDE
                if (m64) hipLaunchKernelGGL((k_probe<W_C, false, 0, 8, true, true, false, true>), dim3(ntiles), dim3(64), 0, PG_K, *fuse);
                else hipLaunchKernelGGL((k_probe<W_C, false, 0, 8, false, true, false, true>), dim3(ntiles), dim3(64), 0, PG_K, *fuse);
#endif
            } else {
                if (m64) hipLaunchKernelGGL((k_probe<W_C, false, 0, 8, true, true>), dim3(ntiles), dim3(64), 0, PG_K, none);
                else hipLaunchKernelGGL((k_probe<W_C, false, 0, 8, false, true>), dim3(ntiles), dim3(64), 0, PG_K, none);
            }
        }
        return hipGetLastError();
    }
    if (st.slots == 16) {
        if (st.W == 2) {
            if (rowmode == 2) return probe_t<W_C, true, 2, 16>(PG_A);
            return probe_t<W_C, true, 0, 16>(PG_A);
        }
        if (rowmode == 1) return probe_t<W_C, false, 1, 16>(PG_A);
        return probe_t<W_C, false, 0, 16>(PG_A);
    }
    if (st.W == 2) {
        if (rowmode == 2) return probe_t<W_C, true, 2, 8>(PG_A);
        return probe_t<W_C, true, 0, 8>(PG_A);
    }
    if (rowmode == 3) return probe_t<W_C, false, 3, 8>(PG_A);
    if (rowmode == 1) return probe_t<W_C, false, 1, 8>(PG_A);
    if (rowmode == 4) return probe_t<W_C, false, 4, 8>(PG_A);
    if (rowmode == 5) return probe_t<W_C, false, 5, 8>(PG_A);
    if (rowmode == 6) return probe_t<W_C, false, 6, 8>(PG_A);
    return probe_t<W_C, false, 0, 8>(PG_A);
#undef PG_A
#undef PG_K
}

template <int W_C>
static hipError_t insert_tiles_w(hipStream_t s, uint32_t ntiles, const SubTable &st, int w, uint32_t bits, uint32_t count_mode,
                                 const uint64_t *seqw, const uint32_t *nmw, const uint32_t *has_n, const SeqDesc *sd,
                                 const uint32_t *tile0, uint32_t ncontigs, unsigned long long *counters, uint32_t max_probe) {
    if (W_C && st.m > 16)
        hipLaunchKernelGGL((k_insert_tile<W_C, true>), dim3(ntiles), dim3(64), 0, s, st, w, bits, count_mode, seqw, nmw, has_n, sd,
                           tile0, ncontigs, counters, max_probe);
    else
        hipLaunchKernelGGL((k_insert_tile<W_C, false>), dim3(ntiles), dim3(64), 0, s, st, w, bits, count_mode, seqw, nmw, has_n, sd,
                           tile0, ncontigs, counters, max_probe);
    return hipGetLastError();
}

#define PG_PROBE_ARGS hipStream_t s, uint32_t w, uint32_t ntiles, const SubTable &st, const uint64_t *seqw, const uint32_t *nmw, const uint32_t *has_n, \
                      const SeqDesc *sd, const AnchorDesc *ad, const uint32_t *tile_contig, const uint32_t *sched, uint32_t tile_base, uint8_t *out1,          \
                      uint32_t nbytes, const RowCols &rc, int rowmode, const FuseArgs *fuse
#define PG_PROBE_CASE(W) case W: return probe_w<W>(s, ntiles, st, seqw, nmw, has_n, sd, ad, tile_contig, sched, tile_base, out1, nbytes, rc, rowmode, fuse);
#define PG_INSERT_ARGS hipStream_t s, uint32_t win, uint32_t ntiles, const SubTable &st, int w, uint32_t bits, uint32_t count_mode, const uint64_t *seqw, \
                       const uint32_t *nmw, const uint32_t *has_n, const SeqDesc *sd, const uint32_t *tile0, uint32_t ncontigs,                          \
                       unsigned long long *counters, uint32_t max_probe
#define PG_INSERT_CASE(W) case W: return insert_tiles_w<W>(s, ntiles, st, w, bits, count_mode, seqw, nmw, has_n, sd, tile0, ncontigs, counters, max_probe);
#if PG_HAS_PART(1)
hipError_t preload_part1() {
    hipFuncAttributes fa;
    return hipFuncGetAttributes(&fa, reinterpret_cast<const void *>(k_insert_tile<6, false>));
}
#endif
#if PG_HAS_PART(2)
hipError_t preload_part2() {
    hipFuncAttributes fa;
    return hipFuncGetAttributes(&fa, reinterpret_cast<const void *>(k_insert_tile<7, false>));
}
#endif
#if PG_HAS_PART(0)
hipError_t probe_part0(PG_PROBE_ARGS) {
    switch (w) { PG_PROBE_CASE(0) PG_PROBE_CASE(3) PG_PROBE_CASE(4) default: return hipErrorInvalidValue; }
}
hipError_t insert_part0(PG_INSERT_ARGS) {
    switch (win) { PG_INSERT_CASE(0) PG_INSERT_CASE(3) PG_INSERT_CASE(4) default: return hipErrorInvalidValue; }
}
#endif
#if PG_HAS_PART(1)
hipError_t probe_part1(PG_PROBE_ARGS) {
    switch (w) { PG_PROBE_CASE(5) PG_PROBE_CASE(6) default: return hipErrorInvalidValue; }
}
hipError_t insert_part1(PG_INSERT_ARGS) {
    switch (win) { PG_INSERT_CASE(5) PG_INSERT_CASE(6) default: return hipErrorInvalidValue; }
}
#endif
#if PG_HAS_PART(2)
hipError_t probe_part2(PG_PROBE_ARGS) {
    switch (w) { PG_PROBE_CASE(7) PG_PROBE_CASE(8) default: return hipErrorInvalidValue; }
}
hipError_t insert_part2(PG_INSERT_ARGS) {
    switch (win) { PG_INSERT_CASE(7) PG_INSERT_CASE(8) default: return hipErrorInvalidValue; }
}
#endif
#undef PG_PROBE_ARGS
#undef PG_PROBE_CASE
#undef PG_INSERT_ARGS
#undef PG_INSERT_CASE

#if PG_MAIN_PART
static hipError_t probe_window(hipStream_t s, uint32_t w, uint32_t ntiles, const SubTable &st, const uint64_t *seqw, const uint32_t *nmw,
                               const uint32_t *has_n, const SeqDesc *sd, const AnchorDesc *ad, const uint32_t *tile_contig, const uint32_t *sched,
                               uint32_t tile_base, uint8_t *out1, uint32_t nbytes, const RowCols &rc, int rowmode, const FuseArgs *fuse) {
    auto *part = (w == 0 || w == 3 || w == 4) ? probe_part0 : (w == 5 || w == 6) ? probe_part1 : (w == 7 || w == 8) ? probe_part2 : nullptr;
    if (!part) return hipErrorInvalidValue;
    return part(s, w, ntiles, st, seqw, nmw, has_n, sd, ad, tile_contig, sched, tile_base, out1, nbytes, rc, rowmode, fuse);
}

static int row_mode(uint32_t nbytes, const RowCols &rc) {
    if (nbytes == 1) return 1;
    if (nbytes == 8 && rc.col0 == 0 && rc.nb0 == 4 && rc.nb1 == 4) return 2;
    if (nbytes == 4 && rc.col0 == 0 && rc.nb0 == 4 && rc.nb1 == 0) return 4;
    if (nbytes == 2 && rc.col0 == 0 && rc.nb1 == 0) return 5;
    if (nbytes == 3 && rc.col0 == 0 && rc.nb1 == 0) return 6;
    return 0;
}

hipError_t launch_anchor(hipStream_t s, const TableDesc &T, const uint64_t *seqw, const uint32_t *nmw,
                         const uint32_t *has_n, const SeqDesc *sd, const AnchorDesc *ad, const uint32_t *tile_contig,
                         const uint32_t *sched, uint32_t tile_base, uint32_t ntiles, uint8_t *out1, uint64_t out1_bytes,
                         uint32_t columns_width, const FuseArgs *fuse) {
    if (ntiles == 0) return hipSuccess;
    const uint32_t nbytes = (T.ngenomes + 7) / 8;
    hipError_t e = hipSuccess;
    (void)out1_bytes;
    if (fuse && (columns_width || T.nsub != 1 || !fuse_rows_ok(nbytes) || fuse->ngenomes != T.ngenomes ||
                 (T.sub[0].layout == LAYOUT_SLOTS && T.sub[0].slots != 8)))
        return hipErrorInvalidValue;
    if (columns_width) {
        const SubTable &st = T.sub[0];
        if (T.nsub != 1 || st.layout != LAYOUT_SLOTS || st.W != 1 || st.slots != 8 || T.ngenomes > (uint32_t)COLS_G ||
            columns_width > (uint32_t)COLS_G || columns_width < T.ngenomes)
            return hipErrorInvalidValue;
        RowCols rc;
        rc.col0 = T.ngenomes;
        rc.nb0 = rc.nb1 = rc.words = 0;
        const uint32_t w = st.m ? st.k - st.m + 1 : 0;
        return probe_window(s, w, ntiles, st, seqw, nmw, has_n, sd, ad, tile_contig, sched, tile_base, out1, columns_width, rc, 3, nullptr);
    }
    for (uint32_t si = 0; si < T.nsub; ++si) {
        const SubTable &st = T.sub[si];
        RowCols rc;
        rc.col0 = 4 * st.word0;
        rc.nb0 = min(4u, nbytes - rc.col0);
        rc.nb1 = (st.W == 2 && nbytes > rc.col0 + 4) ? min(4u, nbytes - rc.col0 - 4) : 0;
        rc.words = (nbytes % 4 == 0 && rc.nb0 == 4 && (rc.nb1 == 0 || rc.nb1 == 4)) ? 1u : (nbytes == 2 ? 2u : 0u);
        if (T.nsub == 1 && (nbytes == 3 || (nbytes >= 5 && nbytes <= 7))) rc.words = 3u;
        if (rc.words == 1 && rc.nb1 == 4 && rc.col0 % 8 == 0 && nbytes % 8 == 0) rc.words = 4u;
        const int rm = (T.nsub == 1) ? row_mode(nbytes, rc) : 0;
        const uint32_t w = st.m ? st.k - st.m + 1 : 0;
        e = probe_window(s, w, ntiles, st, seqw, nmw, has_n, sd, ad, tile_contig, sched, tile_base, out1, nbytes, rc, rm, fuse);
        if (e != hipSuccess) return e;
    }
    return e;
}

#ifdef PG_PHASE_TIMING
}
extern "C" int pg_debug_phase_cycles(unsigned long long *out16, int reset) {
    hipDeviceSynchronize();
    static unsigned long long all[1024 * 16];
    if (hipMemcpyFromSymbol(all, HIP_SYMBOL(pg::pg_phase_cycles), sizeof all) != hipSuccess) return -1;
    for (int i = 0; i < 16; ++i) out16[i] = 0;
    for (int b = 0; b < 1024; ++b)
        for (int i = 0; i < 16; ++i) out16[i] += all[b * 16 + i];
    if (reset) {
        for (auto &x : all) x = 0;
        if (hipMemcpyToSymbol(HIP_SYMBOL(pg::pg_phase_cycles), all, sizeof all) != hipSuccess) return -1;
    }
    return 0;
}
namespace pg {
#endif
hipError_t preload_anchor_kernels() {
    hipFuncAttributes fa;
    hipError_t e = hipFuncGetAttributes(&fa, reinterpret_cast<const void *>(k_insert_tile<4, false>));
    if (e == hipSuccess) e = preload_part1();
    if (e == hipSuccess) e = preload_part2();
    return e;
}

hipError_t launch_insert_tiles(hipStream_t s, const SubTable &st, int w, uint32_t bits, int count_mode, const uint64_t *seqw,
                               const uint32_t *nmw, const uint32_t *has_n, const SeqDesc *sd, const uint32_t *tile0,
                               uint32_t ncontigs, uint32_t ntiles, unsigned long long *counters, uint32_t max_probe) {
    if (ntiles == 0) return hipSuccess;
    const uint32_t win = st.m ? st.k - st.m + 1 : 0;
    auto *part = (win == 0 || win == 3 || win == 4) ? insert_part0 : (win == 5 || win == 6) ? insert_part1 : (win == 7 || win == 8) ? insert_part2 : nullptr;
    if (!part) return hipErrorInvalidValue;
    return part(s, win, ntiles, st, w, bits, (uint32_t)count_mode, seqw, nmw, has_n, sd, tile0, ncontigs, counters, max_probe);
}
#endif

}
```

### panagram_amd/csrc/pg_api.hip

```cpp
#include "../../include/panagram_hip.h"
#include "pg_kernels.h"
#include "pg_guard.h"

#include <algorithm>
#include <atomic>
#include <condition_variable>
#include <cmath>
#include <cstdarg>
#include <cstdio>
#include <cstdlib>
#include <cstring>
#include <memory>
#include <mutex>
#include <string>
#include <system_error>
#include <thread>
#include <vector>

using namespace pg;

static thread_local std::string g_err;

static int fail(int code, const char *fmt, ...) {
    char buf[512];
    va_list ap;
    va_start(ap, fmt);
    vsnprintf(buf, sizeof buf, fmt, ap);
    va_end(ap);
    g_err = buf;
    return code;
}

#define HIP_TRY(expr)                                                                          \
    do {                                                                                       \
        hipError_t e_ = (expr);                                                                \
        if (e_ != hipSuccess)                                                                  \
            return fail(PG_E_HIP, "%s failed: %s (%s:%d)", #expr, hipGetErrorString(e_), __FILE__, __LINE__); \
    } while (0)

extern "C" const char *pg_last_error(void) { return g_err.c_str(); }
int pg_set_error(int code, const char *msg) {
    g_err = msg ? msg : "";
    return code;
}
extern "C" const char *pg_version(void) { return "panagram_hip 0.2 gfx950"; }
extern "C" uint32_t pg_tile_positions(void) { return (uint32_t)PROBE_TILE; }

struct pg_ctx {
    int device;
    hipStream_t own_stream;
    hipStream_t stream;
    hipStream_t aux_stream;
    std::atomic<int> refs{0};
    bool dead = false;
    struct DfSet {
        uint8_t *d_slots[2] = {nullptr, nullptr}, *d_packed[2] = {nullptr, nullptr}, *h_slots[2] = {nullptr, nullptr};
        uint32_t *d_sizes[2] = {nullptr, nullptr}, *d_offs[2] = {nullptr, nullptr}, *h_sizes[2] = {nullptr, nullptr};
        uint32_t *d_crc = nullptr, *d_hist = nullptr;
        void *d_code = nullptr;
        bool ready = false, busy = false;
    } df[4];
    std::mutex df_mu;
    std::condition_variable df_cv;
    struct RowBuf {
        uint8_t *p;
        uint64_t cap;
    };
    std::vector<RowBuf> row_cache;
    std::mutex row_mu;
};

struct SubHost {
    SubTable d;
    uint64_t count;
};

struct pg_table {
    pg_ctx *ctx;
    int k, ngenomes, ndbs;
    uint32_t m;
    bool m_pinned = false;
    uint32_t cosched = 0;
    uint64_t expected = 0;
    double load0 = 0.375;
    uint64_t first_len = 0;
    uint64_t max_len = 0;
    std::vector<SubHost> subs;
    unsigned long long *d_counters;
    unsigned long long *h_counters = nullptr;
    uint32_t *d_tile0 = nullptr;
    size_t tile0_cap = 0;
    double spill = 0;
    std::atomic<int> refs{0};
    bool dead = false;
    std::mutex write_mu;
};
#define TABLE_WRITER(t) std::lock_guard<std::mutex> writer_guard_((t)->write_mu)

struct pg_seqset {
    pg_ctx *ctx;
    uint32_t n;
    std::vector<SeqDesc> desc;
    uint64_t total_words;
    uint64_t *d_seqw;
    uint32_t *d_nmw;
    uint32_t *d_has_n;
    SeqDesc *d_desc;
    void *d_stage;
    size_t stage_cap;
    std::vector<std::string> names;
    std::atomic<int> refs{0};
    bool dead = false;
};

struct pg_result {
    pg_ctx *ctx;
    pg_table *tbl;
    const pg_seqset *seqs;
    uint32_t N;
    int k;
    uint32_t flags;
    uint32_t lowres_step = 100;
    std::vector<AnchorDesc> ad;
    std::vector<uint64_t> nrows100;
    AnchorDesc *d_ad;
    uint32_t *d_tile_contig;
    uint32_t *d_sched = nullptr;
    std::vector<uint32_t> sched_bounds;
    uint32_t ntiles;
    uint8_t *d_out1;
    uint64_t out1_bytes;
    uint64_t out1_cap = 0;
    uint8_t *d_out100;
    uint64_t out100_bytes;
    uint32_t *d_bins;
    uint64_t total_bins;
    unsigned long long *d_colsums;
    hipEvent_t ev[4];
    bool ev_ok, ev_epi;
    bool rows_valid = false;
    struct EvSet {
        hipEvent_t e[4];
        bool probe, epi;
    };
    std::vector<EvSet> ev_hist, ev_free;
    struct Chunk {
        uint32_t s0, s1, r0, nr, tiles;
    };
    std::vector<Chunk> chunks;
    uint2 *d_ranges = nullptr;
    bool chunks_ready = false;
    std::vector<hipEvent_t> chunk_ev;
    size_t hist_skip = 0;
    double probe_ms_sum = 0, epi_ms_sum = 0;
    uint32_t probe_runs = 0, epi_runs = 0;
    int fuse_state = 0;
    uint32_t *d_tile_hist = nullptr, *d_tile_cs = nullptr;
    uint2 *d_small = nullptr;
    uint32_t n_small = 0, small_tiles = 0;
    uint32_t fused_runs = 0;
};
static constexpr size_t EV_RING = 128;

static constexpr uint32_t MAX_PROBE = 512;
static constexpr double GROW_AT = 0.55;
#ifndef PG_INLINE_LAYOUT
#define PG_INLINE_LAYOUT 1
#endif
static constexpr double TARGET_LOAD = 0.375;
static constexpr double HARD_LOAD = 0.85;

static int use_device(const pg_ctx *c) {
    HIP_TRY(hipSetDevice(c->device));
    return PG_OK;
}

extern "C" int pg_ctx_create(int device_id, pg_ctx **out) {
    PG_API_BEGIN
    if (!out) return fail(PG_E_INVALID, "pg_ctx_create: out is NULL");
    int n = 0;
    hipError_t e = hipGetDeviceCount(&n);
    if (e != hipSuccess || n == 0)
        return fail(PG_E_HIP, "no HIP device visible (%s); libpanagram_hip has no CPU fallback",
                    e == hipSuccess ? "device count 0" : hipGetErrorString(e));
    if (device_id < 0 || device_id >= n) return fail(PG_E_INVALID, "device %d out of range (0..%d)", device_id, n - 1);
    HIP_TRY(hipSetDevice(device_id));
    pg_ctx *c = new pg_ctx();
    c->device = device_id;
    hipError_t se = hipStreamCreateWithFlags(&c->own_stream, hipStreamNonBlocking);
    if (se != hipSuccess) {
        delete c;
        return fail(PG_E_HIP, "hipStreamCreate failed: %s", hipGetErrorString(se));
    }
    c->stream = c->own_stream;
    se = hipStreamCreateWithFlags(&c->aux_stream, hipStreamNonBlocking);
    if (se != hipSuccess) {
        hipStreamDestroy(c->own_stream);
        delete c;
        return fail(PG_E_HIP, "hipStreamCreate failed: %s", hipGetErrorString(se));
    }
    hipError_t pe = preload_table_kernels();
    if (pe == hipSuccess) pe = preload_anchor_kernels();
    if (pe == hipSuccess) pe = preload_rows_kernels();
    if (pe == hipSuccess) pe = preload_deflate_kernels();
    if (pe != hipSuccess) {
        hipStreamDestroy(c->aux_stream);
        hipStreamDestroy(c->own_stream);
        delete c;
        return fail(PG_E_HIP, "loading the gfx950 kernels failed: %s (is this an MI355X?)", hipGetErrorString(pe));
    }
    *out = c;
    return PG_OK;
    PG_API_END
}

static void df_free_buffers(pg_ctx::DfSet &d);
static void ctx_free(pg_ctx *c) {
    hipSetDevice(c->device);
    hipStreamSynchronize(c->stream);
    hipStreamSynchronize(c->aux_stream);
    for (auto &b : c->row_cache) hipFree(b.p);
    c->row_cache.clear();
    for (auto &d : c->df) df_free_buffers(d);
    hipStreamDestroy(c->aux_stream);
    hipStreamDestroy(c->own_stream);
    delete c;
}
static void ctx_release(pg_ctx *c) {
    if (--c->refs == 0 && c->dead) ctx_free(c);
}

static constexpr uint64_t ROW_CACHE_MIN = 1ull << 30;
static void row_cache_trim(pg_ctx *c) {
    std::lock_guard<std::mutex> lk(c->row_mu);
    for (auto &b : c->row_cache) hipFree(b.p);
    c->row_cache.clear();
}
static hipError_t row_alloc(pg_ctx *c, uint64_t bytes, uint8_t **out, uint64_t *cap) {
    {
        std::lock_guard<std::mutex> lk(c->row_mu);
        for (size_t i = 0; i < c->row_cache.size(); ++i)
            if (c->row_cache[i].cap >= bytes && c->row_cache[i].cap <= 2 * bytes) {
                *out = c->row_cache[i].p;
                *cap = c->row_cache[i].cap;
                c->row_cache.erase(c->row_cache.begin() + (long)i);
                return hipSuccess;
            }
    }
    hipError_t e = hipMalloc(reinterpret_cast<void **>(out), bytes);
    if (e != hipSuccess) {
        (void)hipGetLastError();
        row_cache_trim(c);
        e = hipMalloc(reinterpret_cast<void **>(out), bytes);
    }
    *cap = bytes;
    return e;
}
static void row_free(pg_ctx *c, uint8_t *p, uint64_t cap) {
    if (!p) return;
    if (cap >= ROW_CACHE_MIN && !c->dead) {
        std::lock_guard<std::mutex> lk(c->row_mu);
        if (c->row_cache.size() < 2) {
            c->row_cache.push_back({p, cap});
            return;
        }
    }
    hipFree(p);
}

extern "C" int pg_host_alloc(pg_ctx *c, uint64_t nbytes, void **out) {
    PG_API_BEGIN
    if (!c || !out) return fail(PG_E_INVALID, "pg_host_alloc: NULL argument");
    if (int r = use_device(c)) return r;
    *out = nullptr;
    hipError_t e = hipHostMalloc(out, std::max<uint64_t>(nbytes, 1), hipHostMallocDefault);
    if (e != hipSuccess) {
        (void)hipGetLastError();
        *out = nullptr;
        return fail(PG_E_HIP, "hipHostMalloc(%llu bytes) failed: %s", (unsigned long long)nbytes, hipGetErrorString(e));
    }
    return PG_OK;
    PG_API_END
}

extern "C" int pg_host_free(pg_ctx *c, void *p) {
    PG_API_BEGIN
    if (!c) return fail(PG_E_INVALID, "ctx is NULL");
    if (!p) return PG_OK;
    if (int r = use_device(c)) return r;
    HIP_TRY(hipHostFree(p));
    return PG_OK;
    PG_API_END
}

extern "C" int pg_ctx_mem_info(pg_ctx *c, uint64_t *free_bytes, uint64_t *total_bytes) {
    PG_API_BEGIN
    if (!c) return fail(PG_E_INVALID, "ctx is NULL");
    if (int r = use_device(c)) return r;
    size_t f = 0, t = 0;
    HIP_TRY(hipMemGetInfo(&f, &t));
    {
        std::lock_guard<std::mutex> lk(c->row_mu);
        for (auto &b : c->row_cache) f += b.cap;
    }
    if (free_bytes) *free_bytes = f;
    if (total_bytes) *total_bytes = t;
    return PG_OK;
    PG_API_END
}

extern "C" int pg_ctx_trim(pg_ctx *c) {
    PG_API_BEGIN
    if (!c) return fail(PG_E_INVALID, "ctx is NULL");
    if (int r = use_device(c)) return r;
    row_cache_trim(c);
    return PG_OK;
    PG_API_END
}

extern "C" int pg_ctx_destroy(pg_ctx *c) {
    PG_API_BEGIN
    if (!c || c->dead) return PG_OK;
    c->dead = true;
    if (c->refs == 0) ctx_free(c);
    return PG_OK;
    PG_API_END
}

extern "C" int pg_device_alloc(pg_ctx *c, uint64_t bytes, void **out) {
    PG_API_BEGIN
    if (!c || !out) return fail(PG_E_INVALID, "pg_device_alloc: NULL argument");
    if (int r = use_device(c)) return r;
    void *p = nullptr;
    HIP_TRY(hipMalloc(&p, std::max<uint64_t>(bytes, 16)));
    hipError_t e = hipMemsetAsync(p, 0, std::max<uint64_t>(bytes, 16), c->stream);
    if (e != hipSuccess) {
        hipFree(p);
        return fail(PG_E_HIP, "hipMemsetAsync failed: %s", hipGetErrorString(e));
    }
    *out = p;
    return PG_OK;
    PG_API_END
}
extern "C" int pg_device_memset(pg_ctx *c, void *p, int value, uint64_t bytes) {
    PG_API_BEGIN
    if (!c || (!p && bytes)) return fail(PG_E_INVALID, "pg_device_memset: NULL argument");
    if (int r = use_device(c)) return r;
    if (bytes) HIP_TRY(hipMemsetAsync(p, value, bytes, c->stream));
    return PG_OK;
    PG_API_END
}
extern "C" int pg_device_free(pg_ctx *c, void *p) {
    PG_API_BEGIN
    if (!c) return fail(PG_E_INVALID, "ctx is NULL");
    if (!p) return PG_OK;
    if (int r = use_device(c)) return r;
    HIP_TRY(hipStreamSynchronize(c->stream));
    HIP_TRY(hipFree(p));
    return PG_OK;
    PG_API_END
}

extern "C" int pg_ctx_set_stream(pg_ctx *c, void *s, int use_own) {
    PG_API_BEGIN
    if (!c) return fail(PG_E_INVALID, "ctx is NULL");
    c->stream = use_own ? c->own_stream : reinterpret_cast<hipStream_t>(s);
    return PG_OK;
    PG_API_END
}

extern "C" int pg_ctx_synchronize(pg_ctx *c) {
    PG_API_BEGIN
    if (!c) return fail(PG_E_INVALID, "ctx is NULL");
    if (int r = use_device(c)) return r;
    HIP_TRY(hipStreamSynchronize(c->stream));
    HIP_TRY(hipStreamSynchronize(c->aux_stream));
    return PG_OK;
    PG_API_END
}

static uint64_t next_prime(uint64_t n) {
    if (n < 3) return 3;
    n |= 1;
    for (;; n += 2) {
        bool prime = true;
        for (uint64_t d = 3; d * d <= n; d += 2)
            if (n % d == 0) {
                prime = false;
                break;
            }
        if (prime) return n;
    }
}

static void free_sub(SubTable &d) {
    if (d.buckets) hipFree(d.buckets);
    if (d.masks) hipFree(d.masks);
    d.buckets = d.masks = nullptr;
}

static int alloc_sub(pg_ctx *ctx, uint32_t W, uint32_t word0, uint32_t k, uint32_t m, uint32_t slots, uint64_t nbuckets,
                     uint32_t layout, SubTable *out) {
    if (nbuckets < 64) nbuckets = 64;
    nbuckets = next_prime(nbuckets);
    if (nbuckets > 0x80000000ull) return fail(PG_E_CAPACITY, "sub-table would exceed 2^31 lines (256 GB of key lines)");
    SubTable t;
    t.W = W;
    t.word0 = word0;
    t.k = k;
    t.m = m;
    t.slots = slots;
    t.layout = layout;
    t.nbuckets = nbuckets;
    t.buckets = t.masks = nullptr;
    auto grab = [&](uint64_t bytes, uint8_t **p) {
        hipError_t e = hipMalloc(reinterpret_cast<void **>(p), bytes);
        if (e != hipSuccess) {
            (void)hipGetLastError();
            row_cache_trim(ctx);
            e = hipMalloc(reinterpret_cast<void **>(p), bytes);
        }
        return e;
    };
    const uint64_t key_bytes = nbuckets * line_bytes(t), mask_bytes = layout == LAYOUT_SPLIT ? nbuckets * slots * 4ull * W : 0;
    hipError_t e = grab(key_bytes, &t.buckets);
    if (e == hipSuccess && mask_bytes) e = grab(mask_bytes, &t.masks);
    if (e != hipSuccess) {
        free_sub(t);
        return fail(PG_E_HIP, "hipMalloc(%llu bytes) for k-mer table failed: %s", (unsigned long long)(key_bytes + mask_bytes),
                    hipGetErrorString(e));
// ... 1319 lines not shown
        if (e_up == hipSuccess && hipMalloc(reinterpret_cast<void **>(&d_hdr), (size_t)HDR_CAP * 8) == hipSuccess &&
            hipMalloc(reinterpret_cast<void **>(&d_nhdr), 4) == hipSuccess) {
            hipStream_t st = ctx->stream;
            if (launch_text_headers(st, d_text, nbytes, d_hdr, HDR_CAP, d_nhdr) == hipSuccess &&
                hipMemcpyAsync(&nh, d_nhdr, 4, hipMemcpyDeviceToHost, st) == hipSuccess && hipStreamSynchronize(st) == hipSuccess && nh <= HDR_CAP) {
                hdrs.resize(nh);
                if (nh == 0 || hipMemcpy(hdrs.data(), d_hdr, (size_t)nh * 8, hipMemcpyDeviceToHost) == hipSuccess) {
                    std::sort(hdrs.begin(), hdrs.end());
                    have_hdrs = true;
                }
            }
        }
        (void)hipGetLastError();
        if (d_hdr) hipFree(d_hdr);
        if (d_nhdr) hipFree(d_nhdr);
    }
    size_t hdr_at = 0;
    auto next_header = [&](uint64_t from) -> uint64_t {
        if (have_hdrs) {
            while (hdr_at < hdrs.size() && hdrs[hdr_at] < from) ++hdr_at;
            return hdr_at < hdrs.size() ? hdrs[hdr_at] : nbytes;
        }
        uint64_t p = from;
        while (p < nbytes) {
            const void *q = memchr(text + p, '>', nbytes - p);
            if (!q) return nbytes;
            p = (uint64_t)(static_cast<const unsigned char *>(q) - text);
            if (p == 0 || text[p - 1] == '\n') return p;
            ++p;
        }
        return nbytes;
    };
    uint64_t h = next_header(0);
    while (h < nbytes) {
        const void *q = memchr(text + h, '\n', nbytes - h);
        const uint64_t eol = q ? (uint64_t)(static_cast<const unsigned char *>(q) - text) : nbytes;
        uint64_t a = h + 1;
        while (a < eol && host_is_ws(text[a])) ++a;
        uint64_t b = a;
        while (b < eol && !host_is_ws(text[b])) ++b;
        Rec r;
        r.name.assign(reinterpret_cast<const char *>(text + a), b - a);
        r.s = std::min<uint64_t>(eol + 1, nbytes);
        const uint64_t hn = next_header(r.s);
        r.e = hn;
        recs.push_back(r);
        h = hn;
    }
    const uint32_t nrec = (uint32_t)recs.size();
    std::vector<uint64_t> ub(nrec);
    std::vector<TextChunk> chunks;
    std::vector<uint64_t> chunk0(nrec + 1, 0);
    for (uint32_t i = 0; i < nrec; ++i) {
        ub[i] = recs[i].e - recs[i].s;
        chunk0[i] = chunks.size();
        for (uint64_t p = recs[i].s; p < recs[i].e;) {
            const uint64_t lim = std::min<uint64_t>(recs[i].e, (p / 4096 + 1) * 4096);
            TextChunk c;
            c.off = p;
            c.len = (uint32_t)(lim - p);
            c.rec = i;
            chunks.push_back(c);
            p = lim;
        }
    }
    chunk0[nrec] = chunks.size();
    pg_seqset *s = nullptr;
    if (int r = pg_seqset_create(ctx, nrec, ub.data(), &s)) return r;
    for (auto &r : recs) s->names.push_back(r.name);
    if (nrec == 0) {
        *out = s;
        return PG_OK;
    }
    hipStream_t st = ctx->stream;
    const uint64_t nch = chunks.size();
    TextChunk *d_chunks = nullptr;
    uint64_t *d_chunk0 = nullptr, *d_base = nullptr, *d_len = nullptr;
    uint32_t *d_counts = nullptr;
    std::vector<uint64_t> lens(nrec, 0);
    hipError_t e = hipSuccess;
    auto ok = [&](hipError_t x) {
        if (e == hipSuccess) e = x;
        return e == hipSuccess;
    };
    if (ok(hipMalloc(reinterpret_cast<void **>(&d_chunks), std::max<uint64_t>(nch, 1) * sizeof(TextChunk))) &&
        ok(hipMalloc(reinterpret_cast<void **>(&d_chunk0), (nrec + 1) * 8)) &&
        ok(hipMalloc(reinterpret_cast<void **>(&d_base), std::max<uint64_t>(nch, 1) * 8)) &&
        ok(hipMalloc(reinterpret_cast<void **>(&d_len), nrec * 8)) &&
        ok(hipMalloc(reinterpret_cast<void **>(&d_counts), std::max<uint64_t>(nch, 1) * 4))) {
        if (up.th.joinable()) up.th.join();
        ok(e_up);
        if (nch) ok(hipMemcpyAsync(d_chunks, chunks.data(), nch * sizeof(TextChunk), hipMemcpyHostToDevice, st));
        ok(hipMemcpyAsync(d_chunk0, chunk0.data(), (nrec + 1) * 8, hipMemcpyHostToDevice, st));
        if (e == hipSuccess)
            ok(launch_text_pack(st, d_text, d_chunks, nch, d_chunk0, nrec, d_counts, d_base, d_len, s->d_desc, s->d_seqw,
                                s->d_nmw, s->d_has_n));
        ok(hipMemcpyAsync(lens.data(), d_len, nrec * 8, hipMemcpyDeviceToHost, st));
        ok(hipStreamSynchronize(st));
        if (e == hipSuccess) {
            for (uint32_t i = 0; i < nrec; ++i) s->desc[i].len = lens[i];
            ok(hipMemcpyAsync(s->d_desc, s->desc.data(), nrec * sizeof(SeqDesc), hipMemcpyHostToDevice, st));
            ok(hipStreamSynchronize(st));
        }
    }
    if (e != hipSuccess) (void)hipStreamSynchronize(st);
    hipFree(d_chunks);
    hipFree(d_chunk0);
    hipFree(d_base);
    hipFree(d_len);
    hipFree(d_counts);
    if (e != hipSuccess) {
        pg_seqset_destroy(s);
        return fail(PG_E_HIP, "FASTA packing failed: %s", hipGetErrorString(e));
    }
    *out = s;
    return PG_OK;
    PG_API_END
}

static int seqset_concat(pg_ctx *ctx, const pg_seqset *const *sets, const uint32_t *first, const uint32_t *count,
                         uint32_t nsets, pg_seqset **out) {
    if (!ctx || !out || (nsets && !sets)) return fail(PG_E_INVALID, "pg_seqset_concat: NULL argument");
    std::vector<uint64_t> lens;
    for (uint32_t i = 0; i < nsets; ++i) {
        if (!sets[i] || sets[i]->ctx != ctx) return fail(PG_E_INVALID, "pg_seqset_concat: seqset %u is NULL or of another context", i);
        const uint32_t f = first ? first[i] : 0, n = first ? count[i] : sets[i]->n;
        if ((uint64_t)f + n > sets[i]->n) return fail(PG_E_INVALID, "pg_seqset_concat_ranges: contigs %u..%u of seqset %u out of range", f, f + n, i);
        for (uint32_t j = f; j < f + n; ++j) lens.push_back(sets[i]->desc[j].len);
    }
    pg_seqset *s = nullptr;
    if (int r = pg_seqset_create(ctx, (uint32_t)lens.size(), lens.data(), &s)) return r;
    hipStream_t st = ctx->stream;
    hipError_t e = hipSuccess;
    std::vector<SeqCopy> jobs;
    jobs.reserve(lens.size());
    uint64_t max_words = 0;
    uint32_t c = 0;
    for (uint32_t i = 0; i < nsets; ++i) {
        const pg_seqset *src = sets[i];
        const uint32_t f = first ? first[i] : 0, n = first ? count[i] : src->n;
        for (uint32_t j = f; j < f + n; ++j, ++c) {
            SeqCopy q;
            q.src_seqw = src->d_seqw;
            q.src_nmw = src->d_nmw;
            q.src_has_n = src->d_has_n + j;
            q.src_off = src->desc[j].seq_off;
            q.dst_off = s->desc[c].seq_off;
            q.nwords = std::min(src->desc[j].nwords, s->desc[c].nwords);
            max_words = std::max(max_words, q.nwords);
            jobs.push_back(q);
            s->names.push_back(j < src->names.size() ? src->names[j] : std::string());
        }
    }
    SeqCopy *d_jobs = nullptr;
    if (!jobs.empty()) {
        e = hipMalloc(reinterpret_cast<void **>(&d_jobs), jobs.size() * sizeof(SeqCopy));
        if (e == hipSuccess) e = hipMemcpyAsync(d_jobs, jobs.data(), jobs.size() * sizeof(SeqCopy), hipMemcpyHostToDevice, st);
        if (e == hipSuccess) e = launch_seq_gather(st, d_jobs, (uint32_t)jobs.size(), max_words, s->d_seqw, s->d_nmw, s->d_has_n);
    }
    if (e == hipSuccess) e = hipStreamSynchronize(st);
    if (d_jobs) hipFree(d_jobs);
    if (e != hipSuccess) {
        pg_seqset_destroy(s);
        return fail(PG_E_HIP, "pg_seqset_concat: %s", hipGetErrorString(e));
    }
    *out = s;
    return PG_OK;
}

extern "C" int pg_seqset_concat(pg_ctx *ctx, const pg_seqset *const *sets, uint32_t nsets, pg_seqset **out) {
    PG_API_BEGIN
    return seqset_concat(ctx, sets, nullptr, nullptr, nsets, out);
    PG_API_END
}

extern "C" int pg_seqset_concat_ranges(pg_ctx *ctx, const pg_seqset *const *sets, const uint32_t *first_contig,
                                       const uint32_t *ncontigs, uint32_t nsets, pg_seqset **out) {
    PG_API_BEGIN
    if (nsets && (!first_contig || !ncontigs)) return fail(PG_E_INVALID, "pg_seqset_concat_ranges: NULL argument");
    return seqset_concat(ctx, sets, first_contig, ncontigs, nsets, out);
    PG_API_END
}

extern "C" int pg_seqset_slice(pg_ctx *ctx, const pg_seqset *src, uint32_t n, const uint32_t *contig, const uint64_t *start,
                               const uint64_t *len, pg_seqset **out) {
    PG_API_BEGIN
    if (!ctx || !src || !out || (n && (!contig || !start || !len))) return fail(PG_E_INVALID, "pg_seqset_slice: NULL argument");
    if (src->ctx != ctx) return fail(PG_E_INVALID, "pg_seqset_slice: the seqset belongs to another context");
    for (uint32_t i = 0; i < n; ++i) {
        if (contig[i] >= src->n) return fail(PG_E_INVALID, "pg_seqset_slice: contig %u out of range (0..%u)", contig[i], src->n ? src->n - 1 : 0);
        if (start[i] & 31u) return fail(PG_E_INVALID, "pg_seqset_slice: piece %u starts at base %llu — starts must be multiples of 32", i, (unsigned long long)start[i]);
        if (start[i] > src->desc[contig[i]].len || len[i] > src->desc[contig[i]].len - start[i])
            return fail(PG_E_INVALID, "pg_seqset_slice: piece %u (%llu + %llu) exceeds contig %u of %llu bases", i, (unsigned long long)start[i],
                        (unsigned long long)len[i], contig[i], (unsigned long long)src->desc[contig[i]].len);
    }
    pg_seqset *s = nullptr;
    if (int r = pg_seqset_create(ctx, n, len, &s)) return r;
    hipStream_t st = ctx->stream;
    hipError_t e = hipSuccess;
    for (uint32_t i = 0; i < n && e == hipSuccess; ++i) {
        const SeqDesc &from = src->desc[contig[i]];
        const uint64_t w0 = start[i] >> 5, nw = (len[i] + 31) >> 5;
        if (nw) {
            e = hipMemcpyAsync(s->d_seqw + s->desc[i].seq_off, src->d_seqw + from.seq_off + w0, nw * 8, hipMemcpyDeviceToDevice, st);
            if (e == hipSuccess)
                e = hipMemcpyAsync(s->d_nmw + s->desc[i].seq_off, src->d_nmw + from.seq_off + w0, nw * 4, hipMemcpyDeviceToDevice, st);
        }
        if (e == hipSuccess) e = hipMemcpyAsync(s->d_has_n + i, src->d_has_n + contig[i], 4, hipMemcpyDeviceToDevice, st);
        std::string nm = contig[i] < src->names.size() ? src->names[contig[i]] : std::string();
        s->names.push_back(nm + ":" + std::to_string((unsigned long long)start[i]));
    }
    if (e == hipSuccess) e = launch_seq_tailmask(st, s->d_desc, n, s->d_seqw, s->d_nmw);
    if (e == hipSuccess) e = hipStreamSynchronize(st);
    if (e != hipSuccess) {
        pg_seqset_destroy(s);
        return fail(PG_E_HIP, "pg_seqset_slice: %s", hipGetErrorString(e));
    }
    *out = s;
    return PG_OK;
    PG_API_END
}

extern "C" uint32_t pg_seqset_ncontigs(const pg_seqset *s) { return s ? s->n : 0; }

extern "C" int pg_seqset_contig(const pg_seqset *s, uint32_t idx, const char **name, uint64_t *len) {
    PG_API_BEGIN
    if (!s) return fail(PG_E_INVALID, "seqset is NULL");
    if (idx >= s->n) return fail(PG_E_INVALID, "contig %u out of range", idx);
    if (name) *name = idx < s->names.size() ? s->names[idx].c_str() : "";
    if (len) *len = s->desc[idx].len;
    return PG_OK;
    PG_API_END
}

extern "C" int pg_seqset_describe(const pg_seqset *s, uint64_t *lens, char *names, uint64_t names_cap, uint64_t *names_bytes) {
    PG_API_BEGIN
    if (!s) return fail(PG_E_INVALID, "seqset is NULL");
    uint64_t need = 0;
    for (uint32_t i = 0; i < s->n; ++i) {
        if (lens) lens[i] = s->desc[i].len;
        need += (i < s->names.size() ? s->names[i].size() : 0) + 1;
    }
    if (names_bytes) *names_bytes = need;
    if (names) {
        if (names_cap < need) return fail(PG_E_INVALID, "pg_seqset_describe: %llu bytes of names, room for %llu", (unsigned long long)need, (unsigned long long)names_cap);
        char *p = names;
        for (uint32_t i = 0; i < s->n; ++i) {
            if (i < s->names.size()) {
                memcpy(p, s->names[i].data(), s->names[i].size());
                p += s->names[i].size();
            }
            *p++ = 0;
        }
    }
    return PG_OK;
    PG_API_END
}

extern "C" int pg_seqset_unpack(const pg_seqset *s, uint32_t idx, char *out) {
    PG_API_BEGIN
    if (!s || !out) return fail(PG_E_INVALID, "pg_seqset_unpack: NULL argument");
    if (idx >= s->n) return fail(PG_E_INVALID, "contig %u out of range", idx);
    if (int r = use_device(s->ctx)) return r;
    const SeqDesc &d = s->desc[idx];
    const uint64_t nw = (d.len + 31) / 32;
    std::vector<uint64_t> w(nw);
    std::vector<uint32_t> nm(nw);
    if (nw) {
        HIP_TRY(hipMemcpyAsync(w.data(), s->d_seqw + d.seq_off, nw * 8, hipMemcpyDeviceToHost, s->ctx->stream));
        HIP_TRY(hipMemcpyAsync(nm.data(), s->d_nmw + d.seq_off, nw * 4, hipMemcpyDeviceToHost, s->ctx->stream));
        HIP_TRY(hipStreamSynchronize(s->ctx->stream));
    }
    for (uint64_t i = 0; i < d.len; ++i)
        out[i] = ((nm[i >> 5] >> (i & 31)) & 1u) ? 'N' : "ACGT"[(w[i >> 5] >> (2 * (i & 31))) & 3u];
    return PG_OK;
    PG_API_END
}

extern "C" uint64_t pg_seqset_total_kmers(const pg_seqset *s, int k) {
    uint64_t t = 0;
    if (s)
        for (auto &d : s->desc)
            if (d.len >= (uint64_t)k) t += d.len - k + 1;
    return t;
}

static TableDesc make_desc(const pg_table *t) {
    TableDesc T;
    memset(&T, 0, sizeof T);
    T.nsub = (uint32_t)t->subs.size();
    for (uint32_t i = 0; i < T.nsub; ++i) T.sub[i] = t->subs[i].d;
    T.ndbs = t->ndbs;
    T.k = t->k;
    T.ngenomes = t->ngenomes;
    return T;
}

struct ResultGeom {
    uint32_t lowres_step = 100;
    uint64_t max_bin_len = 200000;
    uint32_t min_bin_count = 100;
};

static int result_create(pg_ctx *ctx, pg_table *t, int k, uint32_t N, const pg_seqset *sq, uint32_t flags,
                         const ResultGeom &geo, pg_result **out) {
    if (ctx != sq->ctx) return fail(PG_E_INVALID, "table / context and seqset belong to different contexts");
    if (geo.lowres_step < 1 || geo.max_bin_len < 1 || geo.min_bin_count < 1)
        return fail(PG_E_INVALID, "lowres_step, max_bin_len and min_bin_count must be >= 1");
    if (int r = use_device(ctx)) return r;
    const uint32_t nbytes = (N + 7) / 8;
    pg_result *r = new pg_result();
    r->ctx = ctx;
    r->tbl = t;
    r->seqs = sq;
    r->N = N;
    r->k = k;
    if (t) ++t->refs;
    else ++ctx->refs;
    ++const_cast<pg_seqset *>(sq)->refs;
    r->flags = flags;
    r->lowres_step = geo.lowres_step;
    r->d_ad = nullptr;
    r->d_tile_contig = nullptr;
    r->d_out1 = r->d_out100 = nullptr;
    r->d_bins = nullptr;
    r->d_colsums = nullptr;
    r->ev_ok = r->ev_epi = false;
    for (auto &e : r->ev) e = nullptr;
    uint64_t o1 = 0, o100 = 0, bins = 0, tiles = 0;
    std::vector<uint32_t> tile_contig;
    for (uint32_t c = 0; c < sq->n; ++c) {
        const uint64_t len = sq->desc[c].len;
        const uint64_t nk = len >= (uint64_t)k ? len - k + 1 : 0;
        if (nk > 0xFFFFFFF0ull) {
            pg_result_destroy(r);
            return fail(PG_E_INVALID, "contig %u has %llu k-mers; contigs must stay below 2^32 (as in KMC)", c, (unsigned long long)nk);
        }
        AnchorDesc a;
        a.nkmers = (uint32_t)nk;
        uint64_t binlen = geo.max_bin_len;
        if (nk / binlen < geo.min_bin_count) binlen = nk / geo.min_bin_count;
        if (binlen == 0) binlen = 1;
        a.binlen = (uint32_t)binlen;
        a.nbins = (uint32_t)((nk + binlen - 1) / binlen);
        a.out_off = o1;
        a.out100_off = o100;
        a.bin_off = bins;
        a.tile0 = (uint32_t)tiles;
        const uint64_t n100 = (nk + geo.lowres_step - 1) / geo.lowres_step;
        r->nrows100.push_back(n100);
        o1 += (nk * nbytes + 15) & ~15ull;
        o100 += n100 * nbytes;
        bins += a.nbins;
        const uint64_t nt = (nk + PROBE_TILE - 1) / PROBE_TILE;
        for (uint64_t i = 0; i < nt; ++i) tile_contig.push_back(c);
        tiles += nt;
        r->ad.push_back(a);
    }
    if (tiles > 0x7FFFFFFFull) {
        pg_result_destroy(r);
        return fail(PG_E_INVALID, "too many tiles in one launch");
    }
    r->ntiles = (uint32_t)tiles;
    r->out1_bytes = o1;
    r->out100_bytes = o100;
    r->total_bins = bins;
    hipStream_t st = ctx->stream;
    hipError_t e;
    if ((e = hipMalloc(reinterpret_cast<void **>(&r->d_ad), std::max<size_t>(1, r->ad.size()) * sizeof(AnchorDesc))) == hipSuccess &&
        (e = hipMalloc(reinterpret_cast<void **>(&r->d_tile_contig), std::max<size_t>(1, tile_contig.size()) * 4)) == hipSuccess &&
        (e = row_alloc(ctx, (flags & PG_ANCHOR_COLUMNS_ONLY) ? 16 : std::max<uint64_t>(16, o1) + 16, &r->d_out1, &r->out1_cap)) == hipSuccess &&
        (e = hipMalloc(reinterpret_cast<void **>(&r->d_out100), std::max<uint64_t>(16, o100))) == hipSuccess &&
        (e = hipMalloc(reinterpret_cast<void **>(&r->d_bins), std::max<uint64_t>(1, bins) * (N + 1) * 4)) == hipSuccess &&
        (e = hipMalloc(reinterpret_cast<void **>(&r->d_colsums), std::max<size_t>(1, r->ad.size()) * N * 8)) == hipSuccess) {
        if (!r->ad.empty())
            e = hipMemcpyAsync(r->d_ad, r->ad.data(), r->ad.size() * sizeof(AnchorDesc), hipMemcpyHostToDevice, st);
        if (e == hipSuccess && !tile_contig.empty())
            e = hipMemcpyAsync(r->d_tile_contig, tile_contig.data(), tile_contig.size() * 4, hipMemcpyHostToDevice, st);
        if (e == hipSuccess && !t) e = hipMemsetAsync(r->d_out1, 0, std::max<uint64_t>(16, o1), st);
        if (e == hipSuccess) e = hipStreamSynchronize(st);
    }
    if (e != hipSuccess) {
        pg_result_destroy(r);
        return fail(PG_E_HIP, "result allocation failed: %s", hipGetErrorString(e));
    }
    *out = r;
    return PG_OK;
}

extern "C" int pg_result_create(pg_table *t, const pg_seqset *sq, uint32_t flags, pg_result **out) {
    PG_API_BEGIN
    if (!t || !sq || !out) return fail(PG_E_INVALID, "pg_result_create: NULL argument");
    return result_create(t->ctx, t, t->k, (uint32_t)t->ngenomes, sq, flags, ResultGeom(), out);
    PG_API_END
}

extern "C" int pg_result_create_ex(pg_table *t, const pg_seqset *sq, uint32_t flags, uint32_t lowres_step,
                                   uint64_t max_bin_len, uint32_t min_bin_count, pg_result **out) {
    PG_API_BEGIN
    if (!t || !sq || !out) return fail(PG_E_INVALID, "pg_result_create_ex: NULL argument");
    ResultGeom g;
    g.lowres_step = lowres_step;
    g.max_bin_len = max_bin_len;
    g.min_bin_count = min_bin_count;
    return result_create(t->ctx, t, t->k, (uint32_t)t->ngenomes, sq, flags, g, out);
    PG_API_END
}

extern "C" int pg_result_create_rows(pg_ctx *ctx, int k, int ngenomes, const pg_seqset *sq, uint32_t flags,
                                     uint32_t lowres_step, uint64_t max_bin_len, uint32_t min_bin_count, pg_result **out) {
    PG_API_BEGIN
    if (!ctx || !sq || !out) return fail(PG_E_INVALID, "pg_result_create_rows: NULL argument");
    if (k < 1 || k > 32) return fail(PG_E_INVALID, "k=%d unsupported (1..32)", k);
    if (ngenomes < 1) return fail(PG_E_INVALID, "ngenomes must be >= 1");
    ResultGeom g;
    g.lowres_step = lowres_step;
    g.max_bin_len = max_bin_len;
    g.min_bin_count = min_bin_count;
    return result_create(ctx, nullptr, k, (uint32_t)ngenomes, sq, flags | PG_ANCHOR_ROWS_ONLY, g, out);
    PG_API_END
}

extern "C" int pg_result_destroy(pg_result *r) {
    PG_API_BEGIN
    if (!r) return PG_OK;
    hipSetDevice(r->ctx->device);
    hipStreamSynchronize(r->ctx->stream);
    hipStreamSynchronize(r->ctx->aux_stream);
    hipFree(r->d_ad);
    hipFree(r->d_tile_contig);
    row_free(r->ctx, r->d_out1, r->out1_cap);
    hipFree(r->d_out100);
    hipFree(r->d_bins);
    hipFree(r->d_colsums);
    if (r->d_sched) hipFree(r->d_sched);
    if (r->d_ranges) hipFree(r->d_ranges);
    if (r->d_tile_hist) hipFree(r->d_tile_hist);
    if (r->d_tile_cs) hipFree(r->d_tile_cs);
    if (r->d_small) hipFree(r->d_small);
    for (auto e : r->chunk_ev) hipEventDestroy(e);
    for (auto *v : {&r->ev_hist, &r->ev_free})
        for (auto &s : *v)
            for (auto &e : s.e)
                if (e) hipEventDestroy(e);
    pg_table *t = r->tbl;
    pg_ctx *c = r->ctx;
    pg_seqset *sq = const_cast<pg_seqset *>(r->seqs);
    delete r;
    if (t) table_release(t);
    else ctx_release(c);
    seqset_release(sq);
    return PG_OK;
    PG_API_END
}

static int build_chunks(pg_result *r, const uint32_t *sched) {
    r->chunks.clear();
    r->chunks_ready = true;
    if (r->d_ranges) {
        hipFree(r->d_ranges);
        r->d_ranges = nullptr;
    }
    const char *env = getenv("PG_RUN_CHUNKS");
    const uint32_t nbytes = (r->N + 7) / 8;
    uint32_t K = env ? (uint32_t)atoi(env) : ((nbytes == 8 && r->ntiles >= (4u << 20)) ? 16u : 1u);
    const char *mt = getenv("PG_CHUNK_MIN_TILES");
    K = std::min(K, r->ntiles / std::max(1u, mt ? (uint32_t)atoi(mt) : 32768u));
    if (K < 2) return PG_OK;
    std::vector<uint2> ranges;
    for (uint32_t c = 0; c < K; ++c) {
        pg_result::Chunk ch;
        ch.s0 = (uint32_t)((uint64_t)r->ntiles * c / K);
        ch.s1 = (uint32_t)((uint64_t)r->ntiles * (c + 1) / K);
        ch.r0 = (uint32_t)ranges.size();
        ch.tiles = ch.s1 - ch.s0;
        if (!sched) {
            ranges.push_back(make_uint2(ch.s0, ch.s1));
        } else {
            std::vector<uint2> runs;
            for (uint32_t i = ch.s0; i < ch.s1; ++i) {
                if (!runs.empty() && runs.back().y == sched[i]) ++runs.back().y;
                else runs.push_back(make_uint2(sched[i], sched[i] + 1));
            }
            std::sort(runs.begin(), runs.end(), [](const uint2 &a, const uint2 &b) { return a.x < b.x; });
            for (const uint2 &u : runs) {
                if (ranges.size() > ch.r0 && ranges.back().y == u.x) ranges.back().y = u.y;
                else ranges.push_back(u);
            }
        }
        ch.nr = (uint32_t)ranges.size() - ch.r0;
        if (ch.nr > 512) {
            r->chunks.clear();
            return PG_OK;
        }
        r->chunks.push_back(ch);
    }
    HIP_TRY(hipMalloc(reinterpret_cast<void **>(&r->d_ranges), ranges.size() * sizeof(uint2)));
    HIP_TRY(hipMemcpy(r->d_ranges, ranges.data(), ranges.size() * sizeof(uint2), hipMemcpyHostToDevice));
    while (r->chunk_ev.size() < r->chunks.size()) {
        hipEvent_t e;
        HIP_TRY(hipEventCreateWithFlags(&e, hipEventDisableTiming));
        r->chunk_ev.push_back(e);
    }
    return PG_OK;
}

static int coschedule(pg_result *r, const uint32_t *contig_group, uint32_t piece_tiles, const uint32_t *range_first,
                      uint32_t nranges, const uint32_t *contig_class = nullptr) {
    if (int e = use_device(r->ctx)) return e;
    hipStream_t st = r->ctx->stream;
    HIP_TRY(hipStreamSynchronize(st));
    HIP_TRY(hipStreamSynchronize(r->ctx->aux_stream));
    if (r->d_sched) {
        hipFree(r->d_sched);
        r->d_sched = nullptr;
    }
    r->sched_bounds.clear();
    r->chunks.clear();
    r->chunks_ready = false;
    if (!contig_group || r->ntiles == 0) return PG_OK;
    const bool auto_piece = piece_tiles == 0;
    const size_t nc = r->ad.size();
    std::vector<uint32_t> firsts;
    if (range_first && nranges) {
        for (uint32_t i = 0; i < nranges; ++i) {
            if (range_first[i] >= nc || (i && range_first[i] <= range_first[i - 1]) || (!i && range_first[0] != 0))
                return fail(PG_E_INVALID, "pg_result_coschedule_ranges: range starts must begin at contig 0 and increase");
            firsts.push_back(range_first[i]);
        }
    } else {
        firsts.push_back(0);
    }
    firsts.push_back((uint32_t)nc);
    struct Piece {
        double at;
        uint32_t g, first;
    };
    std::vector<uint32_t> sched;
    sched.reserve(r->ntiles);
    std::vector<std::vector<uint32_t>> members;
    if (contig_class) {
        std::vector<std::pair<uint32_t, uint32_t>> byclass;
        for (size_t c = 0; c < nc; ++c) byclass.emplace_back(contig_class[c], (uint32_t)c);
        std::stable_sort(byclass.begin(), byclass.end(), [](auto &x, auto &y) { return x.first < y.first; });
        for (size_t i = 0; i < byclass.size(); ++i) {
            if (i == 0 || byclass[i].first != byclass[i - 1].first) members.emplace_back();
            members.back().push_back(byclass[i].second);
        }
        r->sched_bounds.push_back(0);
    } else {
        for (size_t ri = 0; ri + 1 < firsts.size(); ++ri) {
            members.emplace_back();
            for (uint32_t c = firsts[ri]; c < firsts[ri + 1]; ++c) members.back().push_back(c);
            r->sched_bounds.push_back(r->ad[firsts[ri]].tile0);
        }
    }
    for (const auto &mem : members) {
        uint32_t ngroups = 0;
        for (uint32_t c : mem) ngroups = std::max(ngroups, contig_group[c] + 1);
        std::vector<std::vector<uint32_t>> tiles(ngroups);
        for (uint32_t c : mem) {
            const uint32_t nt = (uint32_t)(((uint64_t)r->ad[c].nkmers + PROBE_TILE - 1) / PROBE_TILE);
            for (uint32_t i = 0; i < nt; ++i) tiles[contig_group[c]].push_back(r->ad[c].tile0 + i);
        }
        if (auto_piece) piece_tiles = ngroups <= 32 ? 64u : std::max(8u, 512u / ngroups);
        std::vector<Piece> pieces;
        for (uint32_t g = 0; g < ngroups; ++g) {
            const size_t np = (tiles[g].size() + piece_tiles - 1) / piece_tiles;
            for (size_t i = 0; i < np; ++i) pieces.push_back({(double)i / (double)np, g, (uint32_t)(i * piece_tiles)});
        }
        std::stable_sort(pieces.begin(), pieces.end(), [](const Piece &x, const Piece &y) { return x.at < y.at; });
        for (const Piece &p : pieces) {
            const size_t end = std::min<size_t>(tiles[p.g].size(), (size_t)p.first + piece_tiles);
            for (size_t i = p.first; i < end; ++i) sched.push_back(tiles[p.g][i]);
        }
    }
    r->sched_bounds.push_back(r->ntiles);
    if (sched.size() != r->ntiles) return fail(PG_E_INVALID, "internal: schedule does not cover the tiles");
    HIP_TRY(hipMalloc(reinterpret_cast<void **>(&r->d_sched), (size_t)r->ntiles * 4));
    HIP_TRY(hipMemcpyAsync(r->d_sched, sched.data(), (size_t)r->ntiles * 4, hipMemcpyHostToDevice, st));
    HIP_TRY(hipStreamSynchronize(st));
    if (!(r->flags & PG_ANCHOR_ROWS_ONLY)) return build_chunks(r, sched.data());
    return PG_OK;
}

extern "C" int pg_result_coschedule(pg_result *r, const uint32_t *contig_group, uint32_t piece_tiles) {
    PG_API_BEGIN
    if (!r) return fail(PG_E_INVALID, "result is NULL");
    return coschedule(r, contig_group, piece_tiles, nullptr, 0);
    PG_API_END
}

extern "C" int pg_result_coschedule_classes(pg_result *r, const uint32_t *contig_group, const uint32_t *contig_class,
                                            uint32_t piece_tiles) {
    PG_API_BEGIN
    if (!r) return fail(PG_E_INVALID, "result is NULL");
    if (contig_group && !contig_class) return fail(PG_E_INVALID, "pg_result_coschedule_classes: contig_class is NULL");
    return coschedule(r, contig_group, piece_tiles, nullptr, 0, contig_class);
    PG_API_END
}

extern "C" int pg_result_coschedule_ranges(pg_result *r, const uint32_t *contig_group, uint32_t piece_tiles,
                                           const uint32_t *range_first_contig, uint32_t nranges) {
    PG_API_BEGIN
    if (!r) return fail(PG_E_INVALID, "result is NULL");
    return coschedule(r, contig_group, piece_tiles, range_first_contig, nranges);
    PG_API_END
}

static int enqueue_epilogue(pg_result *r, hipStream_t st) {
    const uint32_t N = r->N;
    HIP_TRY(hipMemsetAsync(r->d_bins, 0, std::max<uint64_t>(1, r->total_bins) * (N + 1) * 4, st));
    HIP_TRY(hipMemsetAsync(r->d_colsums, 0, std::max<size_t>(1, r->ad.size()) * N * 8, st));
    const uint32_t kflags = (r->flags & PG_ANCHOR_COLSUMS) | (r->lowres_step == 100 ? 0u : 2u);
    HIP_TRY(launch_rows_epilogue(st, N, r->d_ad, r->d_tile_contig, r->ntiles, r->d_out1, r->d_out100, r->d_bins,
                                 r->d_colsums, kflags));
    if (r->lowres_step != 100)
        HIP_TRY(launch_lowres(st, N, r->d_ad, r->d_tile_contig, r->ntiles, r->d_out1, r->d_out100, r->lowres_step));
    return PG_OK;
}

static bool fuse_enabled() {
    const char *e = getenv("PG_FUSE_STATS");
    return e && *e == '1';
}
static bool fuse_table_ok(const TableDesc &T, uint32_t N) {
    return T.nsub == 1 && T.ngenomes == N && !(T.sub[0].layout == LAYOUT_SLOTS && T.sub[0].slots != 8);
}
static int prepare_fuse(pg_result *r, const TableDesc &T) {
    if (r->fuse_state) return PG_OK;
    r->fuse_state = -1;
    const uint32_t nbytes = (r->N + 7) / 8;
    if (!fuse_rows_ok(nbytes) || !fuse_table_ok(T, r->N)) return PG_OK;
    std::vector<uint2> small;
    uint64_t small_tiles = 0, fused_tiles = 0;
    for (const AnchorDesc &a : r->ad) {
        const uint32_t nt = (uint32_t)(((uint64_t)a.nkmers + PROBE_TILE - 1) / PROBE_TILE);
        if (!nt) continue;
        if (a.binlen >= (uint32_t)PROBE_TILE) {
            fused_tiles += nt;
            continue;
        }
        small_tiles += nt;
        if (!small.empty() && small.back().y == a.tile0) small.back().y = a.tile0 + nt;
        else small.push_back(make_uint2(a.tile0, a.tile0 + nt));
    }
    if (!fused_tiles || small.size() > 16384) return PG_OK;
    const size_t hb = (size_t)r->ntiles * fuse_hist_words(r->N) * 4, cb = (size_t)r->ntiles * fuse_cs_words(r->N) * 4;
    if (hipMalloc(reinterpret_cast<void **>(&r->d_tile_hist), hb) != hipSuccess || hipMalloc(reinterpret_cast<void **>(&r->d_tile_cs), cb) != hipSuccess ||
        (!small.empty() && hipMalloc(reinterpret_cast<void **>(&r->d_small), small.size() * sizeof(uint2)) != hipSuccess)) {
        (void)hipGetLastError();
        if (r->d_tile_hist) hipFree(r->d_tile_hist);
        if (r->d_tile_cs) hipFree(r->d_tile_cs);
        r->d_tile_hist = r->d_tile_cs = nullptr;
        return PG_OK;
    }
    if (!small.empty()) HIP_TRY(hipMemcpy(r->d_small, small.data(), small.size() * sizeof(uint2), hipMemcpyHostToDevice));
    r->n_small = (uint32_t)small.size();
    r->small_tiles = (uint32_t)small_tiles;
    r->fuse_state = 1;
    return PG_OK;
}
static FuseArgs fuse_args(const pg_result *r) {
    FuseArgs fa;
    fa.out100 = r->lowres_step == 100 ? r->d_out100 : nullptr;
    fa.tile_hist = r->d_tile_hist;
    fa.tile_cs = r->d_tile_cs;
    fa.ngenomes = r->N;
    fa.hw = fuse_hist_words(r->N);
    fa.csw = fuse_cs_words(r->N);
    return fa;
}
static int enqueue_fused_epilogue(pg_result *r, hipStream_t st, const FuseArgs &fa) {
    const uint32_t N = r->N;
    HIP_TRY(hipMemsetAsync(r->d_bins, 0, std::max<uint64_t>(1, r->total_bins) * (N + 1) * 4, st));
    HIP_TRY(hipMemsetAsync(r->d_colsums, 0, std::max<size_t>(1, r->ad.size()) * N * 8, st));
    HIP_TRY(launch_tile_reduce(st, fa, r->d_ad, r->d_tile_contig, r->ntiles, r->d_bins, r->d_colsums, (r->flags & PG_ANCHOR_COLSUMS) ? 1u : 0u));
    const uint32_t kflags = (r->flags & PG_ANCHOR_COLSUMS) | (r->lowres_step == 100 ? 0u : 2u);
    if (r->n_small)
        HIP_TRY(launch_rows_epilogue(st, N, r->d_ad, r->d_tile_contig, r->ntiles, r->d_out1, r->d_out100, r->d_bins, r->d_colsums, kflags,
                                     r->d_small, r->n_small, r->small_tiles));
    if (r->lowres_step != 100)
        HIP_TRY(launch_lowres(st, N, r->d_ad, r->d_tile_contig, r->ntiles, r->d_out1, r->d_out100, r->lowres_step));
    return PG_OK;
}

static int join_result(pg_result *r) {
    if (r->ev_epi) HIP_TRY(hipStreamWaitEvent(r->ctx->stream, r->ev[3], 0));
    return PG_OK;
}

static int fold_timing(pg_result *r, const pg_result::EvSet &s) {
    HIP_TRY(hipEventSynchronize(s.e[s.epi ? 3 : 1]));
    float a = 0, b = 0;
    if (s.probe) {
        HIP_TRY(hipEventElapsedTime(&a, s.e[0], s.e[1]));
        r->probe_ms_sum += a;
        ++r->probe_runs;
    }
    if (s.epi) {
        HIP_TRY(hipEventElapsedTime(&b, s.e[2], s.e[3]));
        r->epi_ms_sum += b;
        ++r->epi_runs;
    }
    return PG_OK;
}

static int next_events(pg_result *r, bool probe) {
    if (r->ev_hist.size() >= EV_RING) {
        if (r->hist_skip) --r->hist_skip;
        else if (int e = fold_timing(r, r->ev_hist.front())) return e;
        r->ev_free.push_back(r->ev_hist.front());
        r->ev_hist.erase(r->ev_hist.begin());
    }
    pg_result::EvSet s;
    if (!r->ev_free.empty()) {
        s = r->ev_free.back();
        r->ev_free.pop_back();
    } else {
        for (auto &e : s.e) {
            e = nullptr;
            HIP_TRY(hipEventCreate(&e));
        }
    }
    s.probe = probe;
    s.epi = false;
    r->ev_hist.push_back(s);
    for (int i = 0; i < 4; ++i) r->ev[i] = s.e[i];
    return PG_OK;
}

static int contig_tiles(const pg_result *r, uint32_t first, uint32_t n, uint32_t *t0, uint32_t *nt) {
    if ((uint64_t)first + n > r->ad.size()) return fail(PG_E_INVALID, "contigs %u..%u out of range (the result has %zu)", first, first + n, r->ad.size());
    if (n == 0) {
        *t0 = *nt = 0;
        return PG_OK;
    }
    const AnchorDesc &a = r->ad[first], &z = r->ad[first + n - 1];
    *t0 = a.tile0;
    *nt = z.tile0 + (uint32_t)(((uint64_t)z.nkmers + PROBE_TILE - 1) / PROBE_TILE) - a.tile0;
    return PG_OK;
}

static bool sched_covers(const pg_result *r, uint32_t t0, uint32_t nt) {
    if (!r->d_sched) return false;
    const auto &b = r->sched_bounds;
    return std::binary_search(b.begin(), b.end(), t0) && std::binary_search(b.begin(), b.end(), t0 + nt);
}

static int run_chunks(pg_result *r, const TableDesc &T) {
    hipStream_t st = r->ctx->stream, aux = r->ctx->aux_stream;
    if (const char *e = getenv("PG_CHUNK_SAME_STREAM"); e && *e == '1') aux = st;
    const uint32_t N = r->N;
    const uint32_t kflags = (r->flags & PG_ANCHOR_COLSUMS) | (r->lowres_step == 100 ? 0u : 2u);
    HIP_TRY(hipEventRecord(r->ev[0], st));
    for (size_t c = 0; c < r->chunks.size(); ++c) {
        const pg_result::Chunk &ch = r->chunks[c];
        HIP_TRY(launch_anchor(st, T, r->seqs->d_seqw, r->seqs->d_nmw, r->seqs->d_has_n, r->seqs->d_desc, r->d_ad, r->d_tile_contig,
                              r->d_sched, ch.s0, ch.s1 - ch.s0, r->d_out1, r->out1_bytes, 0));
        HIP_TRY(hipEventRecord(r->chunk_ev[c], st));
        HIP_TRY(hipStreamWaitEvent(aux, r->chunk_ev[c], 0));
        if (c == 0) {
            HIP_TRY(hipEventRecord(r->ev[2], aux));
            HIP_TRY(hipMemsetAsync(r->d_bins, 0, std::max<uint64_t>(1, r->total_bins) * (N + 1) * 4, aux));
            HIP_TRY(hipMemsetAsync(r->d_colsums, 0, std::max<size_t>(1, r->ad.size()) * N * 8, aux));
        }
        HIP_TRY(launch_rows_epilogue(aux, N, r->d_ad, r->d_tile_contig, r->ntiles, r->d_out1, r->d_out100, r->d_bins, r->d_colsums,
                                     kflags, r->d_ranges + ch.r0, ch.nr, ch.tiles));
    }
    HIP_TRY(hipEventRecord(r->ev[1], st));
    if (r->lowres_step != 100)
        HIP_TRY(launch_lowres(aux, N, r->d_ad, r->d_tile_contig, r->ntiles, r->d_out1, r->d_out100, r->lowres_step));
    HIP_TRY(hipEventRecord(r->ev[3], aux));
    r->ev_ok = r->ev_epi = true;
    r->ev_hist.back().epi = true;
    return PG_OK;
}

static int anchor_run(pg_result *r, uint32_t tile_base, uint32_t ntiles, bool whole, uint32_t columns_width = 0,
                      void *d_columns = nullptr) {
    pg_table *t = r->tbl;
    if (!t) return fail(PG_E_INVALID, "this result is a rows container (pg_result_create_rows): it has no table to probe");
    if (int e = use_device(r->ctx)) return e;
    hipStream_t st = r->ctx->stream, aux = r->ctx->aux_stream;
    if (int e = join_result(r)) return e;
    if (int e = next_events(r, true)) return e;
    TableDesc T = make_desc(t);
    const bool stats = whole && !columns_width && !(r->flags & PG_ANCHOR_ROWS_ONLY);
    bool fuse = false;
    if (stats && fuse_enabled()) {
        if (int e = prepare_fuse(r, T)) return e;
        fuse = r->fuse_state == 1 && fuse_table_ok(T, r->N);
    }
    if (stats && !fuse) {
        if (!r->chunks_ready)
            if (int e = build_chunks(r, nullptr)) return e;
        if (r->chunks.size() > 1) return run_chunks(r, T);
    }
    const FuseArgs fa = fuse_args(r);
    HIP_TRY(hipEventRecord(r->ev[0], st));
    HIP_TRY(launch_anchor(st, T, r->seqs->d_seqw, r->seqs->d_nmw, r->seqs->d_has_n, r->seqs->d_desc, r->d_ad,
                          r->d_tile_contig, sched_covers(r, tile_base, ntiles) ? r->d_sched : nullptr, tile_base, ntiles,
                          columns_width ? static_cast<uint8_t *>(d_columns) : r->d_out1, r->out1_bytes, columns_width, fuse ? &fa : nullptr));
    HIP_TRY(hipEventRecord(r->ev[1], st));
    r->ev_ok = true;
    r->ev_epi = false;
    if (stats) {
        HIP_TRY(hipStreamWaitEvent(aux, r->ev[1], 0));
        HIP_TRY(hipEventRecord(r->ev[2], aux));
        if (fuse) {
            if (int e = enqueue_fused_epilogue(r, aux, fa)) return e;
            ++r->fused_runs;
        } else if (int e = enqueue_epilogue(r, aux)) return e;
        HIP_TRY(hipEventRecord(r->ev[3], aux));
        r->ev_epi = true;
        r->ev_hist.back().epi = true;
    }
    return PG_OK;
}

extern "C" int pg_anchor_run(pg_result *r) {
    PG_API_BEGIN
    if (!r) return fail(PG_E_INVALID, "result is NULL");
    if (r->flags & PG_ANCHOR_COLUMNS_ONLY) return fail(PG_E_INVALID, "a PG_ANCHOR_COLUMNS_ONLY result has no rows: use pg_anchor_run_columns_range");
    return anchor_run(r, 0, r->ntiles, true);
    PG_API_END
}

extern "C" int pg_anchor_run_range(pg_result *r, uint32_t first_contig, uint32_t ncontigs) {
    PG_API_BEGIN
    if (!r) return fail(PG_E_INVALID, "result is NULL");
    if (r->flags & PG_ANCHOR_COLUMNS_ONLY) return fail(PG_E_INVALID, "a PG_ANCHOR_COLUMNS_ONLY result has no rows: use pg_anchor_run_columns_range");
    if (!(r->flags & PG_ANCHOR_ROWS_ONLY)) return fail(PG_E_INVALID, "pg_anchor_run_range needs a PG_ANCHOR_ROWS_ONLY result");
    uint32_t t0, nt;
    if (int e = contig_tiles(r, first_contig, ncontigs, &t0, &nt)) return e;
    return anchor_run(r, t0, nt, false);
    PG_API_END
}

extern "C" int pg_result_columns_direct(const pg_result *r, uint32_t width) {
    PG_API_BEGIN
    if (!r || !r->tbl) return 0;
    const pg_table *t = r->tbl;
    return t->subs.size() == 1 && t->subs[0].d.layout == LAYOUT_SLOTS && t->subs[0].d.W == 1 && t->subs[0].d.slots == 8 &&
           t->ngenomes <= 8 && width <= 8 && (int)width >= t->ngenomes;
    PG_API_END
}

extern "C" int pg_anchor_run_columns_range(pg_result *r, uint32_t first_contig, uint32_t ncontigs, uint32_t width, void *d_dst) {
    PG_API_BEGIN
    if (!r || !d_dst) return fail(PG_E_INVALID, "pg_anchor_run_columns_range: NULL argument");
    if (!pg_result_columns_direct(r, width))
        return fail(PG_E_INVALID, "pg_anchor_run_columns_range: needs a table of up to 8 genomes (8-slot lines) and width in ngenomes..8");
    uint32_t t0, nt;
    if (int e = contig_tiles(r, first_contig, ncontigs, &t0, &nt)) return e;
    return anchor_run(r, t0, nt, false, width, d_dst);
    PG_API_END
}

extern "C" int pg_result_timing(pg_result *r, float *probe_ms, float *epilogue_ms) {
    PG_API_BEGIN
    if (!r) return fail(PG_E_INVALID, "result is NULL");
    if (!r->ev_ok) return fail(PG_E_INVALID, "pg_anchor_run has not been called on this result");
    if (int e = use_device(r->ctx)) return e;
    HIP_TRY(hipEventSynchronize(r->ev[r->ev_epi ? 3 : 1]));
    float a = 0, b = 0;
    HIP_TRY(hipEventElapsedTime(&a, r->ev[0], r->ev[1]));
    if (r->ev_epi) HIP_TRY(hipEventElapsedTime(&b, r->ev[2], r->ev[3]));
    if (probe_ms) *probe_ms = a;
    if (epilogue_ms) *epilogue_ms = b;
    return PG_OK;
    PG_API_END
}

extern "C" int pg_result_fused_runs(const pg_result *r, uint32_t *n) {
    PG_API_BEGIN
    if (!r || !n) return fail(PG_E_INVALID, "pg_result_fused_runs: NULL argument");
    *n = r->fused_runs;
    return PG_OK;
    PG_API_END
}

extern "C" int pg_result_timing_reset(pg_result *r) {
    PG_API_BEGIN
    if (!r) return fail(PG_E_INVALID, "result is NULL");
    while (r->ev_hist.size() > 1) {
        r->ev_free.push_back(r->ev_hist.front());
        r->ev_hist.erase(r->ev_hist.begin());
    }
    r->hist_skip = r->ev_hist.size();
    r->probe_ms_sum = r->epi_ms_sum = 0;
    r->probe_runs = r->epi_runs = 0;
    return PG_OK;
    PG_API_END
}

extern "C" int pg_result_timing_mean(pg_result *r, double *probe_ms, double *epilogue_ms, uint32_t *nruns) {
    PG_API_BEGIN
    if (!r) return fail(PG_E_INVALID, "result is NULL");
    if (int e = use_device(r->ctx)) return e;
    const double a0 = r->probe_ms_sum, b0 = r->epi_ms_sum;
    const uint32_t pn0 = r->probe_runs, en0 = r->epi_runs;
    int rc = PG_OK;
    for (size_t i = r->hist_skip; i < r->ev_hist.size() && !rc; ++i) rc = fold_timing(r, r->ev_hist[i]);
    if (!rc) {
        if (probe_ms) *probe_ms = r->probe_runs ? r->probe_ms_sum / r->probe_runs : 0.0;
        if (epilogue_ms) *epilogue_ms = r->epi_runs ? r->epi_ms_sum / r->epi_runs : 0.0;
        if (nruns) *nruns = r->probe_runs;
    }
    r->probe_ms_sum = a0;
    r->epi_ms_sum = b0;
    r->probe_runs = pn0;
    r->epi_runs = en0;
    return rc;
    PG_API_END
}

extern "C" uint64_t pg_result_columns_bytes(const pg_result *r, uint32_t width) {
    return r ? (uint64_t)r->ntiles * (PROBE_TILE / 8) * width : 0;
}

extern "C" uint64_t pg_result_columns_bytes_range(const pg_result *r, uint32_t width, uint32_t first_contig, uint32_t ncontigs) {
    uint32_t t0, nt;
    if (!r || contig_tiles(r, first_contig, ncontigs, &t0, &nt)) return 0;
    return (uint64_t)nt * (PROBE_TILE / 8) * width;
}

extern "C" int pg_result_extract_columns_range(pg_result *r, uint32_t g0, uint32_t width, uint32_t first_contig,
                                               uint32_t ncontigs, void *d_dst) {
    PG_API_BEGIN
    if (!r || !d_dst) return fail(PG_E_INVALID, "pg_result_extract_columns: NULL argument");
    if (!r->ev_ok && !r->rows_valid) return fail(PG_E_INVALID, "the result holds no rows yet");
    uint32_t t0, nt;
    if (int e = contig_tiles(r, first_contig, ncontigs, &t0, &nt)) return e;
    if (int e = use_device(r->ctx)) return e;
    HIP_TRY(launch_cols_extract(r->ctx->stream, r->N, r->d_ad, r->d_tile_contig, t0, nt, r->d_out1, g0, width, d_dst));
    return PG_OK;
    PG_API_END
}

extern "C" int pg_result_extract_columns(pg_result *r, uint32_t g0, uint32_t width, void *d_dst) {
    PG_API_BEGIN
    if (!r) return fail(PG_E_INVALID, "pg_result_extract_columns: NULL argument");
    return pg_result_extract_columns_range(r, g0, width, 0, (uint32_t)r->ad.size(), d_dst);
    PG_API_END
}

extern "C" int pg_result_merge_columns_range(pg_result *r, const void *d_src, uint32_t part0, uint32_t nparts, uint32_t per,
                                             uint32_t first_contig, uint32_t ncontigs, int accumulate,
                                             uint64_t part_stride_bytes) {
    PG_API_BEGIN
    if (!r || !d_src) return fail(PG_E_INVALID, "pg_result_merge_columns: NULL argument");
    if (per == 0 || nparts == 0) return fail(PG_E_INVALID, "pg_result_merge_columns: empty partition");
    uint32_t t0, nt;
    if (int e = contig_tiles(r, first_contig, ncontigs, &t0, &nt)) return e;
    const uint64_t own = (uint64_t)nt * (PROBE_TILE / 8) * per;
    if (part_stride_bytes == 0) part_stride_bytes = own;
    if (part_stride_bytes < own || part_stride_bytes % 8) return fail(PG_E_INVALID, "pg_result_merge_columns_range: bad block stride");
    if (int e = use_device(r->ctx)) return e;
    if (int e = join_result(r)) return e;
    HIP_TRY(launch_cols_merge(r->ctx->stream, r->N, r->d_ad, r->d_tile_contig, t0, nt, r->d_out1, d_src, part0, nparts,
                              part_stride_bytes / 8, per, accumulate ? 1u : 0u));
    r->rows_valid = true;
    return PG_OK;
    PG_API_END
}

extern "C" int pg_result_merge_columns(pg_result *r, const void *d_src, uint32_t nparts, uint32_t per) {
    PG_API_BEGIN
    if (!r) return fail(PG_E_INVALID, "pg_result_merge_columns: NULL argument");
    return pg_result_merge_columns_range(r, d_src, 0, nparts, per, 0, (uint32_t)r->ad.size(), 0, 0);
    PG_API_END
}

extern "C" int pg_rows_epilogue(pg_result *r) {
    PG_API_BEGIN
    if (!r) return fail(PG_E_INVALID, "result is NULL");
    if (int e = use_device(r->ctx)) return e;
    if (int e = join_result(r)) return e;
    hipStream_t st = r->ctx->stream;
    if (int e = next_events(r, false)) return e;
    HIP_TRY(hipEventRecord(r->ev[0], st));
    HIP_TRY(hipEventRecord(r->ev[1], st));
    HIP_TRY(hipEventRecord(r->ev[2], st));
    if (int e = enqueue_epilogue(r, st)) return e;
    HIP_TRY(hipEventRecord(r->ev[3], st));
    r->ev_ok = true;
    r->ev_epi = true;
    r->ev_hist.back().epi = true;
    return PG_OK;
    PG_API_END
}

static constexpr uint32_t CRC_TAB_WORDS = DF_CRC_TAB_WORDS;
static const uint32_t *crc_tables_host() {
    static uint32_t tab[CRC_TAB_WORDS];
    static std::once_flag once;
    std::call_once(once, [] {
        for (uint32_t i = 0; i < 256; ++i) {
            uint32_t c = i;
            for (int k = 0; k < 8; ++k) c = (c & 1) ? 0xEDB88320u ^ (c >> 1) : c >> 1;
            tab[i] = c;
        }
        for (uint32_t k = 1; k < 4; ++k)
            for (uint32_t b = 0; b < 256; ++b) tab[256 * k + b] = (tab[256 * (k - 1) + b] >> 8) ^ tab[tab[256 * (k - 1) + b] & 255u];
        uint32_t *T0 = tab + 1024;
        for (uint32_t k = 0; k < 4; ++k)
            for (uint32_t b = 0; b < 256; ++b) {
                uint32_t s = b << (8 * k);
                for (uint32_t z = 0; z < DF_CHUNK_BYTES; ++z) s = tab[s & 255u] ^ (s >> 8);
                T0[256 * k + b] = s;
            }
        for (uint32_t j = 1; j < DF_CRC_LEVELS; ++j) {
            const uint32_t *P = tab + 1024 + 1024 * (j - 1);
            uint32_t *T = tab + 1024 + 1024 * j;
            auto apply = [&](uint32_t x) { return P[x & 255u] ^ P[256 + ((x >> 8) & 255u)] ^ P[512 + ((x >> 16) & 255u)] ^ P[768 + (x >> 24)]; };
            for (uint32_t k = 0; k < 4; ++k)
                for (uint32_t b = 0; b < 256; ++b) T[256 * k + b] = apply(apply(b << (8 * k)));
        }
    });
    return tab;
}

#ifndef PG_DF_BATCH
#define PG_DF_BATCH 1024
#endif
static constexpr uint32_t DF_BATCH = PG_DF_BATCH;

static pg_ctx::DfSet *df_acquire(pg_ctx *ctx) {
    std::unique_lock<std::mutex> lk(ctx->df_mu);
    for (;;) {
        for (auto &d : ctx->df)
            if (!d.busy) {
                d.busy = true;
                return &d;
            }
        ctx->df_cv.wait(lk);
    }
}
static void df_release(pg_ctx *ctx, pg_ctx::DfSet *D) {
    {
        std::lock_guard<std::mutex> lk(ctx->df_mu);
        D->busy = false;
    }
    ctx->df_cv.notify_one();
}
static void df_free_buffers(pg_ctx::DfSet &d) {
    for (int i = 0; i < 2; ++i) {
        if (d.d_slots[i]) hipFree(d.d_slots[i]);
        if (d.d_packed[i]) hipFree(d.d_packed[i]);
        if (d.d_sizes[i]) hipFree(d.d_sizes[i]);
        if (d.d_offs[i]) hipFree(d.d_offs[i]);
        if (d.h_slots[i]) hipHostFree(d.h_slots[i]);
        if (d.h_sizes[i]) hipHostFree(d.h_sizes[i]);
        d.d_slots[i] = d.d_packed[i] = d.h_slots[i] = nullptr;
        d.d_sizes[i] = d.d_offs[i] = d.h_sizes[i] = nullptr;
    }
    if (d.d_crc) hipFree(d.d_crc);
    if (d.d_hist) hipFree(d.d_hist);
    if (d.d_code) hipFree(d.d_code);
    d.d_crc = d.d_hist = nullptr;
    d.d_code = nullptr;
    d.ready = false;
}

static int write_bgzf_gpu(pg_result *r, const uint8_t *src, const std::vector<std::pair<uint64_t, uint64_t>> &segs_in,
                          uint64_t total, uint32_t row, const char *gz_path, const char *gzi_path) {
    static const unsigned char EOF_BLOCK[28] = {0x1f, 0x8b, 0x08, 0x04, 0, 0, 0, 0, 0, 0xff, 0x06, 0x00, 0x42, 0x43,
                                                0x02, 0x00, 0x1b, 0x00, 0x03, 0x00, 0, 0, 0, 0, 0, 0, 0, 0};
    pg_ctx *ctx = r->ctx;
    const uint64_t nblocks = (total + 65279) / 65280;
    std::vector<PaySeg> segs;
    uint64_t l = 0;
    for (auto &sg : segs_in) {
        segs.push_back({l, sg.first});
        l += sg.second;
    }
    segs.push_back({total, 0});
    FILE *f = fopen(gz_path, "wb");
    if (!f) return fail(PG_E_IO, "cannot open %s for writing", gz_path);
    pg_ctx::DfSet *D = df_acquire(ctx);
    hipStream_t cs = nullptr;
    PaySeg *d_segs = nullptr;
    hipEvent_t done[2] = {nullptr, nullptr}, copied[2] = {nullptr, nullptr};
    hipError_t e = hipStreamCreateWithFlags(&cs, hipStreamNonBlocking);
    auto ok = [&](hipError_t x) {
        if (e == hipSuccess) e = x;
        return e == hipSuccess;
    };
    if (!D->ready) {
        ok(hipMalloc(reinterpret_cast<void **>(&D->d_crc), CRC_TAB_WORDS * 4));
        ok(hipMalloc(reinterpret_cast<void **>(&D->d_hist), DF_HIST_WORDS * 4));
        ok(hipMalloc(&D->d_code, DF_CODE_BYTES));
        for (int i = 0; i < 2; ++i) {
            ok(hipMalloc(reinterpret_cast<void **>(&D->d_slots[i]), (size_t)DF_BATCH * 65536));
            ok(hipMalloc(reinterpret_cast<void **>(&D->d_packed[i]), (size_t)DF_BATCH * 65536));
            ok(hipMalloc(reinterpret_cast<void **>(&D->d_sizes[i]), (size_t)DF_BATCH * 4));
            ok(hipMalloc(reinterpret_cast<void **>(&D->d_offs[i]), (size_t)(DF_BATCH + 1) * 4));
            ok(hipHostMalloc(reinterpret_cast<void **>(&D->h_slots[i]), (size_t)DF_BATCH * 65536, 0));
            ok(hipHostMalloc(reinterpret_cast<void **>(&D->h_sizes[i]), (size_t)(DF_BATCH + 1) * 4, 0));
        }
        if (e == hipSuccess) {
            ok(hipMemcpyAsync(D->d_crc, crc_tables_host(), CRC_TAB_WORDS * 4, hipMemcpyHostToDevice, cs));
            ok(hipStreamSynchronize(cs));
        }
        D->ready = e == hipSuccess;
        if (!D->ready) df_free_buffers(*D);
    }
    ok(hipMalloc(reinterpret_cast<void **>(&d_segs), segs.size() * sizeof(PaySeg)));
    for (int i = 0; i < 2; ++i) {
        ok(hipEventCreateWithFlags(&done[i], hipEventDisableTiming));
        ok(hipEventCreateWithFlags(&copied[i], hipEventDisableTiming));
    }
    if (e == hipSuccess) {
        ok(hipMemcpyAsync(d_segs, segs.data(), segs.size() * sizeof(PaySeg), hipMemcpyHostToDevice, cs));
        ok(hipStreamWaitEvent(cs, r->ev[r->ev_epi ? 3 : 1], 0));
    }
    if (e == hipSuccess && nblocks) ok(launch_deflate_code(cs, src, d_segs, (uint32_t)segs.size() - 1, total, row, D->d_hist, D->d_code));
    std::vector<uint64_t> coffs, uoffs;
    uint64_t cpos = 0;
    int rc = PG_OK;
    auto issue = [&](uint64_t b0, int slot) {
        const uint32_t nb = (uint32_t)std::min<uint64_t>(DF_BATCH, nblocks - b0);
        hipError_t x = hipMemsetAsync(D->d_slots[slot], 0, (size_t)nb * 65536, cs);
        if (x == hipSuccess)
            x = launch_row_deflate(cs, src, d_segs, (uint32_t)segs.size() - 1, total, b0, nb, row, D->d_crc, D->d_code, D->d_slots[slot],
                                   D->d_sizes[slot], getenv("PG_DEFLATE_FORCE_STORED") ? (uint32_t)atoi(getenv("PG_DEFLATE_FORCE_STORED")) : 0u, D->d_offs[slot], D->d_packed[slot]);
        if (x == hipSuccess)
            x = hipMemcpyAsync(D->h_sizes[slot], D->d_offs[slot], (size_t)(nb + 1) * 4, hipMemcpyDeviceToHost, cs);
        if (x == hipSuccess) x = hipEventRecord(done[slot], cs);
        return x;
    };
    if (e == hipSuccess && nblocks) ok(issue(0, 0));
    int slot = 0;
    for (uint64_t b0 = 0; e == hipSuccess && rc == PG_OK && b0 < nblocks; b0 += DF_BATCH, slot ^= 1) {
        const uint32_t nb = (uint32_t)std::min<uint64_t>(DF_BATCH, nblocks - b0);
        if (!ok(hipEventSynchronize(done[slot]))) break;
        const uint32_t *offs = D->h_sizes[slot];
        const uint32_t bytes = offs[nb];
        if (bytes < 26u * nb || bytes > nb * 65536ull) {
            rc = fail(PG_E_IO, "GPU deflate produced %u bytes for %u blocks", bytes, nb);
            break;
        }
        if (!ok(hipMemcpyAsync(D->h_slots[slot], D->d_packed[slot], bytes, hipMemcpyDeviceToHost, cs))) break;
        if (!ok(hipEventRecord(copied[slot], cs))) break;
        if (b0 + DF_BATCH < nblocks && !ok(issue(b0 + DF_BATCH, slot ^ 1))) break;
        if (!ok(hipEventSynchronize(copied[slot]))) break;
        for (uint32_t i = 0; i < nb; ++i) {
            coffs.push_back(cpos + offs[i]);
            uoffs.push_back((b0 + i) * 65280ull);
        }
        if (fwrite(D->h_slots[slot], 1, bytes, f) != bytes) {
            rc = fail(PG_E_IO, "short write to BGZF file");
            break;
        }
        cpos += bytes;
    }
    if (e != hipSuccess) rc = fail(PG_E_HIP, "pg_result_write_bgzf (GPU deflate): %s", hipGetErrorString(e));
    if (cs) hipStreamSynchronize(cs);
    df_release(ctx, D);
    const std::string keep = rc ? g_err : std::string();
    if (!rc && fwrite(EOF_BLOCK, 1, sizeof EOF_BLOCK, f) != sizeof EOF_BLOCK) rc = fail(PG_E_IO, "short write of BGZF EOF block");
    if (fclose(f) != 0 && !rc) rc = fail(PG_E_IO, "fclose failed on BGZF file");
    if (!rc && gzi_path) {
        FILE *g = fopen(gzi_path, "wb");
        if (!g) rc = fail(PG_E_IO, "cannot open %s", gzi_path);
        else {
            const uint64_t ng = coffs.empty() ? 0 : coffs.size() - 1;
            bool good = fwrite(&ng, 8, 1, g) == 1;
            for (size_t i = 1; good && i < coffs.size(); ++i) good = fwrite(&coffs[i], 8, 1, g) == 1 && fwrite(&uoffs[i], 8, 1, g) == 1;
            if (fclose(g) != 0) good = false;
            if (!good) rc = fail(PG_E_IO, "short write to .gzi");
        }
    }
    if (!keep.empty()) g_err = keep;
    hipFree(d_segs);
    for (int i = 0; i < 2; ++i) {
        if (done[i]) hipEventDestroy(done[i]);
        if (copied[i]) hipEventDestroy(copied[i]);
    }
    if (cs) hipStreamDestroy(cs);
    return rc;
}

extern "C" int pg_result_write_bgzf(pg_result *r, int step, const char *gz_path, const char *gzi_path, int level,
                                    int nthreads) {
    PG_API_BEGIN
    if (!r) return fail(PG_E_INVALID, "pg_result_write_bgzf: NULL argument");
    return pg_result_write_bgzf_range(r, step, 0, (uint32_t)r->ad.size(), gz_path, gzi_path, level, nthreads);
    PG_API_END
}

extern "C" int pg_result_write_bgzf_range(pg_result *r, int step, uint32_t first_contig, uint32_t ncontigs,
                                          const char *gz_path, const char *gzi_path, int level, int nthreads) {
    PG_API_BEGIN
    if (!r || !gz_path) return fail(PG_E_INVALID, "pg_result_write_bgzf: NULL argument");
    if ((uint64_t)first_contig + ncontigs > r->ad.size())
        return fail(PG_E_INVALID, "contigs %u..%u out of range", first_contig, first_contig + ncontigs);
    if (step != 1 && step != 100 && (uint32_t)step != r->lowres_step)
        return fail(PG_E_INVALID, "step must be 1 or the result's low-resolution step (%u; 100 is accepted as its alias)", r->lowres_step);
    if (!r->ev_ok) return fail(PG_E_INVALID, "pg_anchor_run has not been called on this result");
    if (step == 100 && (r->flags & PG_ANCHOR_ROWS_ONLY) && !r->ev_epi)
        return fail(PG_E_INVALID, "rows-only result: bitmap.100 needs pg_rows_epilogue first");
    if (int e = use_device(r->ctx)) return e;
    const uint8_t *src = step == 1 ? r->d_out1 : r->d_out100;
    const uint32_t nbytes_row = (r->N + 7) / 8;
    std::vector<std::pair<uint64_t, uint64_t>> segs;
    uint64_t total = 0;
    for (size_t i = first_contig; i < (size_t)first_contig + ncontigs; ++i) {
        const uint64_t len = (step == 1 ? (uint64_t)r->ad[i].nkmers : r->nrows100[i]) * nbytes_row;
        if (len) segs.emplace_back(step == 1 ? r->ad[i].out_off : r->ad[i].out100_off, len);
        total += len;
    }
    if (level == -2 && nbytes_row < 256) return write_bgzf_gpu(r, src, segs, total, nbytes_row, gz_path, gzi_path);
    if (nthreads < 1) nthreads = 1;
    pg_bgzf *w = nullptr;
    if (level >= 0) level |= nbytes_row == 1 ? PG_BGZF_RLE : (nbytes_row < 256 ? PG_BGZF_ROWS(nbytes_row) : 0);
    if (int e = pg_bgzf_open(gz_path, level, nthreads, &w)) return e;
    const size_t chunk = (size_t)512 * 65280;
    hipStream_t cs = nullptr;
    uint8_t *pin[2] = {nullptr, nullptr};
    hipEvent_t done[2] = {nullptr, nullptr};
    int rc = PG_OK;
    hipError_t e = hipStreamCreateWithFlags(&cs, hipStreamNonBlocking);
    for (int i = 0; i < 2 && e == hipSuccess; ++i) {
        e = hipHostMalloc(reinterpret_cast<void **>(&pin[i]), std::min<uint64_t>(chunk, std::max<uint64_t>(total, 1)), 0);
        if (e == hipSuccess) e = hipEventCreateWithFlags(&done[i], hipEventDisableTiming);
    }
    if (e == hipSuccess) e = hipStreamWaitEvent(cs, r->ev[r->ev_epi ? 3 : 1], 0);
    if (e == hipSuccess) {
        size_t seg = 0;
        uint64_t seg_pos = 0;
        auto issue = [&](uint64_t off, int b) {
            const uint64_t n = std::min<uint64_t>(chunk, total - off);
            hipError_t x = hipSuccess;
            uint64_t got = 0;
            while (got < n && x == hipSuccess) {
                const uint64_t take = std::min<uint64_t>(n - got, segs[seg].second - seg_pos);
                x = hipMemcpyAsync(pin[b] + got, src + segs[seg].first + seg_pos, take, hipMemcpyDeviceToHost, cs);
                got += take;
                seg_pos += take;
                if (seg_pos == segs[seg].second) {
                    ++seg;
                    seg_pos = 0;
                }
            }
            if (x == hipSuccess) x = hipEventRecord(done[b], cs);
            return x;
        };
        uint64_t off = 0;
        int b = 0;
        if (total) e = issue(0, 0);
        while (e == hipSuccess && off < total) {
            const uint64_t n = std::min<uint64_t>(chunk, total - off);
            e = hipEventSynchronize(done[b]);
            if (e != hipSuccess) break;
            if (off + n < total) {
                e = issue(off + n, b ^ 1);
                if (e != hipSuccess) break;
            }
            if ((rc = pg_bgzf_write(w, pin[b], n))) break;
            off += n;
            b ^= 1;
        }
    }
    if (e != hipSuccess) rc = fail(PG_E_HIP, "pg_result_write_bgzf: %s", hipGetErrorString(e));
    if (cs) hipStreamSynchronize(cs);
    const std::string keep = rc ? g_err : std::string();
    const int rc2 = pg_bgzf_close(w, rc ? nullptr : gzi_path);
    if (rc) g_err = keep;
    for (int i = 0; i < 2; ++i) {
        if (pin[i]) hipHostFree(pin[i]);
        if (done[i]) hipEventDestroy(done[i]);
    }
    if (cs) hipStreamDestroy(cs);
    return rc ? rc : rc2;
    PG_API_END
}

extern "C" int pg_result_window_stats(pg_result *r, uint32_t idx, int step, uint32_t nwin, const uint64_t *starts,
                                      const uint64_t *ends, uint64_t *hist, uint64_t *colsums) {
    PG_API_BEGIN
    if (!r || (nwin && (!starts || !ends || !hist))) return fail(PG_E_INVALID, "pg_result_window_stats: NULL argument");
    if (idx >= r->ad.size()) return fail(PG_E_INVALID, "contig %u out of range", idx);
    if (step != 1 && step != 100 && (uint32_t)step != r->lowres_step)
// ... 504 lines not shown
```

### panagram_amd/csrc/pg_kernels.h

```cpp
#pragma once
#include "pg_device.h"

namespace pg {

#ifndef PG_PROBE_TILE
#define PG_PROBE_TILE 1024
#endif
#ifndef PG_PROBE_MAXRUN
#define PG_PROBE_MAXRUN 16
#endif
constexpr int PROBE_TILE = PG_PROBE_TILE;
constexpr int PROBE_MAXRUN = PG_PROBE_MAXRUN;
constexpr int COLS_G = 8;
constexpr uint32_t TILE_SLOTS = PROBE_TILE / 64;
static_assert(PROBE_TILE % 512 == 0, "the column kernels take a tile in units of 512 positions");
#ifndef PG_PROBE_STAGED_LEVELS
#define PG_PROBE_STAGED_LEVELS 2
#endif
constexpr int PROBE_STAGED_LEVELS = PG_PROBE_STAGED_LEVELS;
#ifndef PG_PROBE_QCAP
#define PG_PROBE_QCAP 192
#endif
constexpr int PROBE_QCAP = PG_PROBE_QCAP;

struct RowCols {
    uint32_t col0, nb0, nb1, words;
};

struct SeqDesc {
    uint64_t seq_off;
    uint64_t nwords;
    uint64_t len;
};

struct AnchorDesc {
    uint64_t out_off;
    uint64_t out100_off;
    uint64_t bin_off;
    uint32_t nkmers;
    uint32_t binlen;
    uint32_t tile0;
    uint32_t nbins;
};

hipError_t launch_table_init(hipStream_t st, const SubTable &t);
struct TextChunk {
    uint64_t off;
    uint32_t len, rec;
};
hipError_t launch_text_pack(hipStream_t st, const uint8_t *d_text, const TextChunk *d_chunks, uint64_t nchunks,
                            const uint64_t *d_rec_chunk0, uint32_t nrec, uint32_t *d_counts, uint64_t *d_base,
                            uint64_t *d_rec_len, const SeqDesc *sd, uint64_t *seqw, uint32_t *nmw, uint32_t *has_n);
hipError_t launch_text_headers(hipStream_t st, const uint8_t *d_text, uint64_t nbytes, uint64_t *d_out, uint32_t cap, uint32_t *d_count);
hipError_t launch_seq_tailmask(hipStream_t st, const SeqDesc *sd, uint32_t n, uint64_t *seqw, uint32_t *nmw);
struct SeqCopy {
    const uint64_t *src_seqw;
    const uint32_t *src_nmw;
    const uint32_t *src_has_n;
    uint64_t src_off, dst_off, nwords;
};
hipError_t launch_seq_gather(hipStream_t st, const SeqCopy *jobs, uint32_t n, uint64_t max_words, uint64_t *seqw, uint32_t *nmw,
                             uint32_t *has_n);
hipError_t launch_pack(hipStream_t st, const void *d_ascii, uint64_t len, uint64_t *seqw, uint32_t *nmw,
                       uint64_t nwords, uint32_t *has_n);
hipError_t launch_sketch(hipStream_t st, int k, const uint64_t *seqw, const uint32_t *nmw, const uint32_t *has_n,
                         uint64_t nkmers, uint32_t *regs);
constexpr uint32_t SKETCH_JOB = 1u << 16;
hipError_t launch_sketch_set(hipStream_t st, int k, const SeqDesc *sd, const uint2 *jobs, uint32_t njobs, const uint64_t *seqw,
                             const uint32_t *nmw, const uint32_t *has_n, uint32_t *regs);
constexpr int MINHASH_K = 21;
constexpr uint32_t MINHASH_JOB = 1u << 16;
hipError_t launch_minhash(hipStream_t st, const SeqDesc *sd, const uint2 *jobs, uint32_t njobs, const uint64_t *seqw,
                          const uint32_t *nmw, const uint32_t *has_n, uint64_t limit, uint32_t seed, uint64_t *cand, uint64_t cap,
                          unsigned long long *count, unsigned long long *bases);
hipError_t launch_insert_seq(hipStream_t st, const SubTable &t, int w, uint32_t bits, int k,
                             const uint64_t *seqw, const uint32_t *nmw, const uint32_t *has_n,
                             uint64_t nkmers, unsigned long long *counters, uint32_t max_probe, int count_mode = 0);
hipError_t launch_insert_tiles(hipStream_t st, const SubTable &t, int w, uint32_t bits, int count_mode, const uint64_t *seqw,
                               const uint32_t *nmw, const uint32_t *has_n, const SeqDesc *sd, const uint32_t *tile0,
                               uint32_t ncontigs, uint32_t ntiles, unsigned long long *counters, uint32_t max_probe);
hipError_t preload_table_kernels();
hipError_t preload_anchor_kernels();
hipError_t preload_rows_kernels();
hipError_t preload_deflate_kernels();
hipError_t launch_tile0(hipStream_t st, const SeqDesc *sd, uint32_t n, uint32_t k, uint32_t tile, uint32_t *tile0);
hipError_t launch_count_spill(hipStream_t st, const SubTable &t, unsigned long long *counters);
hipError_t launch_merge_min(hipStream_t st, const SubTable &src, const SubTable &dst, int w, uint32_t bits,
                            uint32_t min_count, unsigned long long *counters, uint32_t max_probe);
hipError_t launch_insert_keys(hipStream_t st, const SubTable &t, int w, const uint64_t *keys,
                              const uint32_t *vals, uint64_t n, unsigned long long *counters,
                              uint32_t max_probe);
hipError_t launch_import_kmc(hipStream_t st, const SubTable &t, int w, const uint8_t *rec, uint64_t first_record, uint64_t nrec,
                             const uint64_t *lut, uint64_t nlut, uint32_t prefixes_per_bin, uint32_t suffix_bytes,
                             uint32_t counter_bytes, uint32_t min_count, uint32_t max_count, unsigned long long *counters,
                             uint32_t max_probe, uint32_t phase = 2, uint32_t dense_above = 0);
hipError_t launch_rehash(hipStream_t st, const SubTable &src, const SubTable &dst,
                         unsigned long long *counters, uint32_t max_probe, uint32_t ngenomes);
hipError_t launch_export(hipStream_t st, const SubTable &t, int w, uint64_t *keys, uint32_t *vals,
                         uint64_t cap, unsigned long long *count);
hipError_t launch_counters(hipStream_t st, const SubTable &t, int w, int k, const uint64_t *seqw,
                           const uint32_t *nmw, const uint32_t *has_n, uint64_t nkmers, uint32_t *out);
struct FuseArgs {
    uint8_t *out100;
    uint32_t *tile_hist;
    uint32_t *tile_cs;
    uint32_t ngenomes, hw, csw;
};
constexpr uint32_t fuse_hist_words(uint32_t ngenomes) { return ngenomes + 1u; }
constexpr uint32_t fuse_cs_words(uint32_t ngenomes) { return 16u * ((((ngenomes + 7u) / 8u) + 3u) / 4u); }
#ifndef PG_FUSE_WIDE
#define PG_FUSE_WIDE 0
#endif
constexpr bool fuse_rows_ok(uint32_t nbytes) { return nbytes >= 2u && nbytes <= (PG_FUSE_WIDE ? 16u : 8u); }
hipError_t launch_anchor(hipStream_t st, const TableDesc &T, const uint64_t *seqw, const uint32_t *nmw,
                         const uint32_t *has_n, const SeqDesc *sd, const AnchorDesc *ad,
                         const uint32_t *tile_contig, const uint32_t *sched, uint32_t tile_base, uint32_t ntiles, uint8_t *out1,
                         uint64_t out1_bytes, uint32_t columns_width = 0, const FuseArgs *fuse = nullptr);
hipError_t launch_tile_reduce(hipStream_t st, const FuseArgs &fo, const AnchorDesc *ad, const uint32_t *tile_contig, uint32_t ntiles,
                              uint32_t *bins, unsigned long long *colsums, uint32_t want_colsums);
hipError_t launch_cols_extract(hipStream_t st, uint32_t ngenomes, const AnchorDesc *ad, const uint32_t *tile_contig,
                               uint32_t tile_base, uint32_t ntiles, const uint8_t *out1, uint32_t g0, uint32_t width, void *dst);
hipError_t launch_cols_merge(hipStream_t st, uint32_t ngenomes, const AnchorDesc *ad, const uint32_t *tile_contig,
                             uint32_t tile_base, uint32_t ntiles, uint8_t *out1, const void *src, uint32_t part0,
                             uint32_t nparts, uint64_t part_words, uint32_t per, uint32_t accumulate);
hipError_t launch_lowres(hipStream_t st, uint32_t ngenomes, const AnchorDesc *ad, const uint32_t *tile_contig,
                         uint32_t ntiles, const uint8_t *out1, uint8_t *outlow, uint32_t step);
struct PaySeg {
    uint64_t lstart, doff;
};
constexpr uint32_t DF_CHUNK_BYTES = 68, DF_CRC_LEVELS = 10, DF_CRC_TAB_WORDS = 1024 + DF_CRC_LEVELS * 1024;
constexpr uint32_t DF_CODE_BYTES = 2048, DF_HIST_WORDS = 288, DF_SAMPLE_BLOCKS = 512;
hipError_t launch_deflate_code(hipStream_t st, const uint8_t *base, const PaySeg *segs, uint32_t nseg, uint64_t total, uint32_t row,
                               uint32_t *hist, void *code);
hipError_t launch_row_deflate(hipStream_t st, const uint8_t *base, const PaySeg *segs, uint32_t nseg, uint64_t total,
                              uint64_t first_block, uint32_t nblocks, uint32_t row, const uint32_t *crc_tabs, const void *code,
                              uint8_t *slots, uint32_t *sizes, uint32_t force_stored, uint32_t *offs, uint8_t *packed);
struct InflBlock {
    uint64_t coff, roff;
    uint32_t hlen, csize, isize, pad;
};
enum : uint32_t {
    INF_E_HEADER = 1, INF_E_TYPE, INF_E_STORED, INF_E_CODES, INF_E_SYMBOL, INF_E_DISTANCE, INF_E_OVERRUN, INF_E_INPUT,
    INF_E_ISIZE, INF_E_CRC
};
hipError_t launch_bgzf_inflate(hipStream_t st, const uint32_t *comp, uint64_t comp_words, const InflBlock *blocks, uint32_t nblocks,
                               const PaySeg *segs, uint32_t nseg, uint8_t *dst, const uint32_t *crc_tabs, uint32_t *status);
hipError_t launch_window_stats(hipStream_t st, uint32_t ngenomes, const uint8_t *rows, uint64_t nrows, uint32_t nwin,
                               uint32_t pieces, const uint64_t *starts, const uint64_t *ends, unsigned long long *hist,
                               unsigned long long *cs);
hipError_t launch_bin_colsums(hipStream_t st, uint32_t ngenomes, const uint8_t *rows, uint32_t stride, uint32_t nbins,
                              uint32_t pieces, const uint64_t *base, const uint64_t *starts, const uint64_t *ends,
                              const uint32_t *keep, uint32_t omit_fixed, unsigned long long *cs, unsigned long long *kept);
hipError_t launch_rows_epilogue(hipStream_t st, uint32_t ngenomes, const AnchorDesc *ad, const uint32_t *tile_contig,
                                uint32_t ntiles, const uint8_t *out1, uint8_t *out100, uint32_t *bins,
                                unsigned long long *colsums, uint32_t flags, const uint2 *d_ranges = nullptr,
                                uint32_t nranges = 0, uint32_t range_tiles = 0);

}
```

Before: 236.1 billion.

## Precompute per-tile records to replace dependent descriptor loads in probe kernel

Builds a 32-byte TileRec per tile on the host, in schedule order, holding the sequence word offset, output row offset, words left, npos, tile id and contig. The probe kernel then does one scalar load instead of a chain of dependent loads (sched, then tile_contig, then AnchorDesc and SeqDesc). It also moves the zeroing of the bins and colsums statistics onto the aux stream at the start, so it can overlap with the probe kernel. The cost is host-side record building and extra device memory, and the tile ordering must stay consistent with the schedule.

```diff
diff --git a/panagram_amd/csrc/pg_anchor.hip b/panagram_amd/csrc/pg_anchor.hip
--- a/panagram_amd/csrc/pg_anchor.hip
+++ b/panagram_amd/csrc/pg_anchor.hip
@@ -12,13 +12,13 @@
 namespace pg {
 
 hipError_t probe_part0(hipStream_t s, uint32_t w, uint32_t ntiles, const SubTable &st, const uint64_t *seqw, const uint32_t *nmw, const uint32_t *has_n,
-                       const SeqDesc *sd, const AnchorDesc *ad, const uint32_t *tile_contig, const uint32_t *sched, uint32_t tile_base, uint8_t *out1,
+                       const TileRec *rec, const AnchorDesc *ad, const uint32_t *tile_contig, const uint32_t *sched, uint32_t tile_base, uint8_t *out1,
                        uint32_t nbytes, const RowCols &rc, int rowmode, const FuseArgs *fuse);
 hipError_t probe_part1(hipStream_t s, uint32_t w, uint32_t ntiles, const SubTable &st, const uint64_t *seqw, const uint32_t *nmw, const uint32_t *has_n,
-                       const SeqDesc *sd, const AnchorDesc *ad, const uint32_t *tile_contig, const uint32_t *sched, uint32_t tile_base, uint8_t *out1,
+                       const TileRec *rec, const AnchorDesc *ad, const uint32_t *tile_contig, const uint32_t *sched, uint32_t tile_base, uint8_t *out1,
                        uint32_t nbytes, const RowCols &rc, int rowmode, const FuseArgs *fuse);
 hipError_t probe_part2(hipStream_t s, uint32_t w, uint32_t ntiles, const SubTable &st, const uint64_t *seqw, const uint32_t *nmw, const uint32_t *has_n,
-                       const SeqDesc *sd, const AnchorDesc *ad, const uint32_t *tile_contig, const uint32_t *sched, uint32_t tile_base, uint8_t *out1,
+                       const TileRec *rec, const AnchorDesc *ad, const uint32_t *tile_contig, const uint32_t *sched, uint32_t tile_base, uint8_t *out1,
                        uint32_t nbytes, const RowCols &rc, int rowmode, const FuseArgs *fuse);
 hipError_t insert_part0(hipStream_t s, uint32_t win, uint32_t ntiles, const SubTable &st, int w, uint32_t bits, uint32_t count_mode, const uint64_t *seqw,
                         const uint32_t *nmw, const uint32_t *has_n, const SeqDesc *sd, const uint32_t *tile0, uint32_t ncontigs,
@@ -782,7 +782,7 @@
 __global__ __launch_bounds__(64, ((probe_pipelined<TWO, ROWMODE, SLOTS, WIDE> || INL || FUSE) ? 8 : 1))
 __attribute__((amdgpu_num_sgpr(80))) void k_probe(const SubTable st, const uint64_t *__restrict__ seqw,
                                               const uint32_t *__restrict__ nmw, const uint32_t *__restrict__ has_n,
-                                              const SeqDesc *__restrict__ sd, const AnchorDesc *__restrict__ ad,
+                                              const TileRec *__restrict__ rec, const AnchorDesc *__restrict__ ad,
                                               const uint32_t *__restrict__ tile_contig,
                                               const uint32_t *__restrict__ sched, uint32_t tile_base,
                                               uint8_t *__restrict__ out1, uint32_t nbytes, const RowCols rc, const FuseArgs fo) {
@@ -808,20 +808,16 @@
     const int lane = threadIdx.x;
     const int k = (int)st.k;
     if constexpr (W_C != 0) __builtin_assume(k >= 20 && k <= 32);
-    const uint32_t tile = sched ? sched[blockIdx.x + tile_base] : blockIdx.x + tile_base;
-    const uint32_t c = tile_contig[tile];
-    const AnchorDesc a = ad[c];
-    const SeqDesc s = sd[c];
-    const uint32_t tile_start = (tile - a.tile0) * PROBE_TILE;
-    const uint32_t npos = min((uint32_t)PROBE_TILE, a.nkmers - tile_start);
-    const bool hasn = has_n[c] != 0;
+    const TileRec t = rec[blockIdx.x + tile_base];
+    const uint32_t npos = t.npos;
+    const bool hasn = has_n[t.contig] != 0;
 
     for (int i = lane; i < PROBE_SEQW; i += 64) {
-        const uint64_t wi = (uint64_t)(tile_start >> 5) + i;
-        const uint64_t wv = wi < s.nwords ? seqw[s.seq_off + wi] : 0ull;
+        const bool in = (uint32_t)i < t.words_left;
+        const uint64_t wv = in ? seqw[t.seq_word0 + i] : 0ull;
         sw[i] = wv;
         rw[PROBE_SEQW - 1 - i] = pair_reverse64(~wv);
-        nw[i] = (hasn && wi < s.nwords) ? nmw[s.seq_off + wi] : 0u;
+        nw[i] = (hasn && in) ? nmw[t.seq_word0 + i] : 0u;
     }
     if (lane == 0) rw[PROBE_SEQW] = 0;
     __syncthreads();
@@ -841,7 +837,7 @@
 #if PG_ABLATE == 9 || PG_ABLATE == 10
     uint8_t *tile_rows = out1 + (uint64_t)(blockIdx.x & 255u) * PROBE_TILE * nbytes;
 #else
-    uint8_t *tile_rows = ROWMODE == 3 ? reinterpret_cast<uint8_t *>(cols) : out1 + a.out_off + (uint64_t)tile_start * nbytes;
+    uint8_t *tile_rows = ROWMODE == 3 ? reinterpret_cast<uint8_t *>(cols) : out1 + t.row_off;
 #endif
     uint32_t qn = 0;
 
@@ -1191,7 +1187,7 @@
     }
     if constexpr (ROWMODE == 3) {
         __syncthreads();
-        const uint32_t width = nbytes, trel = tile - tile_base;
+        const uint32_t width = nbytes, trel = t.tile - tile_base;
         unsigned long long *dst = reinterpret_cast<unsigned long long *>(out1) + (uint64_t)trel * TILE_SLOTS * width;
         for (uint32_t i = lane; i < TILE_SLOTS * width; i += 64) dst[i] = cols[(i / width) * COLS_G + i % width];
     }
@@ -1536,16 +1532,16 @@
 
 template <int W_C, bool TWO, int ROWMODE, int SLOTS>
 static hipError_t probe_t(hipStream_t s, uint32_t ntiles, const SubTable &st, const uint64_t *seqw, const uint32_t *nmw,
-                          const uint32_t *has_n, const SeqDesc *sd, const AnchorDesc *ad, const uint32_t *tile_contig,
+                          const uint32_t *has_n, const TileRec *rec, const AnchorDesc *ad, const uint32_t *tile_contig,
                           const uint32_t *sched, uint32_t tile_base, uint8_t *out1, uint32_t nbytes, const RowCols &rc, const FuseArgs *fuse) {
     const bool m64 = W_C && st.m > 16;
     if constexpr (SLOTS == 8 && ROWMODE != 1 && ROWMODE != 3) {
         if (fuse) {
             if (m64)
-                hipLaunchKernelGGL((k_probe<W_C, TWO, ROWMODE, SLOTS, true, false, false, true>), dim3(ntiles), dim3(64), 0, s, st, seqw, nmw, has_n, sd, ad,
+                hipLaunchKernelGGL((k_probe<W_C, TWO, ROWMODE, SLOTS, true, false, false, true>), dim3(ntiles), dim3(64), 0, s, st, seqw, nmw, has_n, rec, ad,
                                    tile_contig, sched, tile_base, out1, nbytes, rc, *fuse);
             else
-                hipLaunchKernelGGL((k_probe<W_C, TWO, ROWMODE, SLOTS, false, false, false, true>), dim3(ntiles), dim3(64), 0, s, st, seqw, nmw, has_n, sd, ad,
+                hipLaunchKernelGGL((k_probe<W_C, TWO, ROWMODE, SLOTS, false, false, false, true>), dim3(ntiles), dim3(64), 0, s, st, seqw, nmw, has_n, rec, ad,
                                    tile_contig, sched, tile_base, out1, nbytes, rc, *fuse);
             return hipGetLastError();
         }
@@ -1553,21 +1549,21 @@
     if (fuse) return hipErrorInvalidValue;
     const FuseArgs none = {nullptr, nullptr, nullptr, 0, 0, 0};
     if (m64)
-        hipLaunchKernelGGL((k_probe<W_C, TWO, ROWMODE, SLOTS, true>), dim3(ntiles), dim3(64), 0, s, st, seqw, nmw, has_n, sd, ad,
+        hipLaunchKernelGGL((k_probe<W_C, TWO, ROWMODE, SLOTS, true>), dim3(ntiles), dim3(64), 0, s, st, seqw, nmw, has_n, rec, ad,
                            tile_contig, sched, tile_base, out1, nbytes, rc, none);
     else
-        hipLaunchKernelGGL((k_probe<W_C, TWO, ROWMODE, SLOTS, false>), dim3(ntiles), dim3(64), 0, s, st, seqw, nmw, has_n, sd, ad,
+        hipLaunchKernelGGL((k_probe<W_C, TWO, ROWMODE, SLOTS, false>), dim3(ntiles), dim3(64), 0, s, st, seqw, nmw, has_n, rec, ad,
                            tile_contig, sched, tile_base, out1, nbytes, rc, none);
     return hipGetLastError();
 }
 
 template <int W_C>
 static hipError_t probe_w(hipStream_t s, uint32_t ntiles, const SubTable &st, const uint64_t *seqw, const uint32_t *nmw,
-                          const uint32_t *has_n, const SeqDesc *sd, const AnchorDesc *ad, const uint32_t *tile_contig,
+                          const uint32_t *has_n, const TileRec *rec, const AnchorDesc *ad, const uint32_t *tile_contig,
                           const uint32_t *sched, uint32_t tile_base, uint8_t *out1, uint32_t nbytes, const RowCols &rc, int rowmode,
                           const FuseArgs *fuse = nullptr) {
-#define PG_A s, ntiles, st, seqw, nmw, has_n, sd, ad, tile_contig, sched, tile_base, out1, nbytes, rc, fuse
-#define PG_K s, st, seqw, nmw, has_n, sd, ad, tile_contig, sched, tile_base, out1, nbytes, rc
+#define PG_A s, ntiles, st, seqw, nmw, has_n, rec, ad, tile_contig, sched, tile_base, out1, nbytes, rc, fuse
+#define PG_K s, st, seqw, nmw, has_n, rec, ad, tile_contig, sched, tile_base, out1, nbytes, rc
     const FuseArgs none = {nullptr, nullptr, nullptr, 0, 0, 0};
     const bool m64 = W_C && st.m > 16;
     if (st.layout == LAYOUT_INLINE || st.layout == LAYOUT_SPLIT) {
@@ -1632,9 +1628,9 @@
 }
 
 #define PG_PROBE_ARGS hipStream_t s, uint32_t w, uint32_t ntiles, const SubTable &st, const uint64_t *seqw, const uint32_t *nmw, const uint32_t *has_n, \
-                      const SeqDesc *sd, const AnchorDesc *ad, const uint32_t *tile_contig, const uint32_t *sched, uint32_t tile_base, uint8_t *out1,          \
+                      const TileRec *rec, const AnchorDesc *ad, const uint32_t *tile_contig, const uint32_t *sched, uint32_t tile_base, uint8_t *out1,          \
                       uint32_t nbytes, const RowCols &rc, int rowmode, const FuseArgs *fuse
-#define PG_PROBE_CASE(W) case W: return probe_w<W>(s, ntiles, st, seqw, nmw, has_n, sd, ad, tile_contig, sched, tile_base, out1, nbytes, rc, rowmode, fuse);
+#define PG_PROBE_CASE(W) case W: return probe_w<W>(s, ntiles, st, seqw, nmw, has_n, rec, ad, tile_contig, sched, tile_base, out1, nbytes, rc, rowmode, fuse);
 #define PG_INSERT_ARGS hipStream_t s, uint32_t win, uint32_t ntiles, const SubTable &st, int w, uint32_t bits, uint32_t count_mode, const uint64_t *seqw, \
                        const uint32_t *nmw, const uint32_t *has_n, const SeqDesc *sd, const uint32_t *tile0, uint32_t ncontigs,                          \
                        unsigned long long *counters, uint32_t max_probe
@@ -1682,11 +1678,11 @@
 
 #if PG_MAIN_PART
 static hipError_t probe_window(hipStream_t s, uint32_t w, uint32_t ntiles, const SubTable &st, const uint64_t *seqw, const uint32_t *nmw,
-                               const uint32_t *has_n, const SeqDesc *sd, const AnchorDesc *ad, const uint32_t *tile_contig, const uint32_t *sched,
+                               const uint32_t *has_n, const TileRec *rec, const AnchorDesc *ad, const uint32_t *tile_contig, const uint32_t *sched,
                                uint32_t tile_base, uint8_t *out1, uint32_t nbytes, const RowCols &rc, int rowmode, const FuseArgs *fuse) {
     auto *part = (w == 0 || w == 3 || w == 4) ? probe_part0 : (w == 5 || w == 6) ? probe_part1 : (w == 7 || w == 8) ? probe_part2 : nullptr;
     if (!part) return hipErrorInvalidValue;
-    return part(s, w, ntiles, st, seqw, nmw, has_n, sd, ad, tile_contig, sched, tile_base, out1, nbytes, rc, rowmode, fuse);
+    return part(s, w, ntiles, st, seqw, nmw, has_n, rec, ad, tile_contig, sched, tile_base, out1, nbytes, rc, rowmode, fuse);
 }
 
 static int row_mode(uint32_t nbytes, const RowCols &rc) {
@@ -1699,7 +1695,7 @@
 }
 
 hipError_t launch_anchor(hipStream_t s, const TableDesc &T, const uint64_t *seqw, const uint32_t *nmw,
-                         const uint32_t *has_n, const SeqDesc *sd, const AnchorDesc *ad, const uint32_t *tile_contig,
+                         const uint32_t *has_n, const TileRec *rec, const AnchorDesc *ad, const uint32_t *tile_contig,
                          const uint32_t *sched, uint32_t tile_base, uint32_t ntiles, uint8_t *out1, uint64_t out1_bytes,
                          uint32_t columns_width, const FuseArgs *fuse) {
     if (ntiles == 0) return hipSuccess;
@@ -1718,7 +1714,7 @@
         rc.col0 = T.ngenomes;
         rc.nb0 = rc.nb1 = rc.words = 0;
         const uint32_t w = st.m ? st.k - st.m + 1 : 0;
-        return probe_window(s, w, ntiles, st, seqw, nmw, has_n, sd, ad, tile_contig, sched, tile_base, out1, columns_width, rc, 3, nullptr);
+        return probe_window(s, w, ntiles, st, seqw, nmw, has_n, rec, ad, tile_contig, sched, tile_base, out1, columns_width, rc, 3, nullptr);
     }
     for (uint32_t si = 0; si < T.nsub; ++si) {
         const SubTable &st = T.sub[si];
@@ -1731,7 +1727,7 @@
         if (rc.words == 1 && rc.nb1 == 4 && rc.col0 % 8 == 0 && nbytes % 8 == 0) rc.words = 4u;
         const int rm = (T.nsub == 1) ? row_mode(nbytes, rc) : 0;
         const uint32_t w = st.m ? st.k - st.m + 1 : 0;
-        e = probe_window(s, w, ntiles, st, seqw, nmw, has_n, sd, ad, tile_contig, sched, tile_base, out1, nbytes, rc, rm, fuse);
+        e = probe_window(s, w, ntiles, st, seqw, nmw, has_n, rec, ad, tile_contig, sched, tile_base, out1, nbytes, rc, rm, fuse);
         if (e != hipSuccess) return e;
     }
     return e;
diff --git a/panagram_amd/csrc/pg_api.hip b/panagram_amd/csrc/pg_api.hip
--- a/panagram_amd/csrc/pg_api.hip
+++ b/panagram_amd/csrc/pg_api.hip
@@ -126,6 +126,7 @@
     AnchorDesc *d_ad;
     uint32_t *d_tile_contig;
     uint32_t *d_sched = nullptr;
+    TileRec *d_rec_tile = nullptr, *d_rec_sched = nullptr;
     std::vector<uint32_t> sched_bounds;
     uint32_t ntiles;
     uint8_t *d_out1;
@@ -2051,6 +2052,36 @@
     uint32_t min_bin_count = 100;
 };
 
+static hipError_t build_tile_recs(const pg_result *r, const uint32_t *order, TileRec **d_out) {
+    const uint32_t nbytes = (r->N + 7) / 8;
+    std::vector<TileRec> recs;
+    recs.reserve(r->ntiles);
+    for (size_t c = 0; c < r->ad.size(); ++c) {
+        const AnchorDesc &a = r->ad[c];
+        const SeqDesc &sd = r->seqs->desc[c];
+        for (uint64_t ts = 0; ts < a.nkmers; ts += PROBE_TILE) {
+            const uint64_t w0 = ts >> 5;
+            TileRec t;
+            t.seq_word0 = sd.seq_off + w0;
+            t.row_off = a.out_off + ts * nbytes;
+            t.words_left = (uint32_t)std::min<uint64_t>(sd.nwords > w0 ? sd.nwords - w0 : 0, 0xFFFFFFFFull);
+            t.npos = (uint32_t)std::min<uint64_t>(PROBE_TILE, a.nkmers - ts);
+            t.tile = (uint32_t)recs.size();
+            t.contig = (uint32_t)c;
+            recs.push_back(t);
+        }
+    }
+    if (recs.size() != r->ntiles) return hipErrorInvalidValue;
+    if (order) {
+        std::vector<TileRec> by_order(recs.size());
+        for (size_t i = 0; i < recs.size(); ++i) by_order[i] = recs[order[i]];
+        recs.swap(by_order);
+    }
+    hipError_t e = hipMalloc(reinterpret_cast<void **>(d_out), std::max<size_t>(1, recs.size()) * sizeof(TileRec));
+    if (e == hipSuccess && !recs.empty()) e = hipMemcpy(*d_out, recs.data(), recs.size() * sizeof(TileRec), hipMemcpyHostToDevice);
+    return e;
+}
+
 static int result_create(pg_ctx *ctx, pg_table *t, int k, uint32_t N, const pg_seqset *sq, uint32_t flags,
                          const ResultGeom &geo, pg_result **out) {
     if (ctx != sq->ctx) return fail(PG_E_INVALID, "table / context and seqset belong to different contexts");
@@ -2128,6 +2159,7 @@
             e = hipMemcpyAsync(r->d_tile_contig, tile_contig.data(), tile_contig.size() * 4, hipMemcpyHostToDevice, st);
         if (e == hipSuccess && !t) e = hipMemsetAsync(r->d_out1, 0, std::max<uint64_t>(16, o1), st);
         if (e == hipSuccess) e = hipStreamSynchronize(st);
+        if (e == hipSuccess && t) e = build_tile_recs(r, nullptr, &r->d_rec_tile);
     }
     if (e != hipSuccess) {
         pg_result_destroy(r);
@@ -2183,6 +2215,8 @@
     hipFree(r->d_bins);
     hipFree(r->d_colsums);
     if (r->d_sched) hipFree(r->d_sched);
+    if (r->d_rec_tile) hipFree(r->d_rec_tile);
+    if (r->d_rec_sched) hipFree(r->d_rec_sched);
     if (r->d_ranges) hipFree(r->d_ranges);
     if (r->d_tile_hist) hipFree(r->d_tile_hist);
     if (r->d_tile_cs) hipFree(r->d_tile_cs);
@@ -2264,6 +2298,10 @@
         hipFree(r->d_sched);
         r->d_sched = nullptr;
     }
+    if (r->d_rec_sched) {
+        hipFree(r->d_rec_sched);
+        r->d_rec_sched = nullptr;
+    }
     r->sched_bounds.clear();
     r->chunks.clear();
     r->chunks_ready = false;
@@ -2326,9 +2364,14 @@
     }
     r->sched_bounds.push_back(r->ntiles);
     if (sched.size() != r->ntiles) return fail(PG_E_INVALID, "internal: schedule does not cover the tiles");
+    if (r->tbl) HIP_TRY(build_tile_recs(r, sched.data(), &r->d_rec_sched));
     HIP_TRY(hipMalloc(reinterpret_cast<void **>(&r->d_sched), (size_t)r->ntiles * 4));
     HIP_TRY(hipMemcpyAsync(r->d_sched, sched.data(), (size_t)r->ntiles * 4, hipMemcpyHostToDevice, st));
     HIP_TRY(hipStreamSynchronize(st));
+    if (r->d_rec_tile) {
+        hipFree(r->d_rec_tile);
+        r->d_rec_tile = nullptr;
+    }
     if (!(r->flags & PG_ANCHOR_ROWS_ONLY)) return build_chunks(r, sched.data());
     return PG_OK;
 }
@@ -2357,10 +2400,16 @@
     PG_API_END
 }
 
+static int zero_statistics(pg_result *r, hipStream_t aux) {
+    const uint32_t N = r->N;
+    HIP_TRY(hipStreamWaitEvent(aux, r->ev[0], 0));
+    HIP_TRY(hipMemsetAsync(r->d_bins, 0, std::max<uint64_t>(1, r->total_bins) * (N + 1) * 4, aux));
+    HIP_TRY(hipMemsetAsync(r->d_colsums, 0, std::max<size_t>(1, r->ad.size()) * N * 8, aux));
+    return PG_OK;
+}
+
 static int enqueue_epilogue(pg_result *r, hipStream_t st) {
     const uint32_t N = r->N;
-    HIP_TRY(hipMemsetAsync(r->d_bins, 0, std::max<uint64_t>(1, r->total_bins) * (N + 1) * 4, st));
-    HIP_TRY(hipMemsetAsync(r->d_colsums, 0, std::max<size_t>(1, r->ad.size()) * N * 8, st));
     const uint32_t kflags = (r->flags & PG_ANCHOR_COLSUMS) | (r->lowres_step == 100 ? 0u : 2u);
     HIP_TRY(launch_rows_epilogue(st, N, r->d_ad, r->d_tile_contig, r->ntiles, r->d_out1, r->d_out100, r->d_bins,
                                  r->d_colsums, kflags));
@@ -2422,8 +2471,6 @@
 }
 static int enqueue_fused_epilogue(pg_result *r, hipStream_t st, const FuseArgs &fa) {
     const uint32_t N = r->N;
-    HIP_TRY(hipMemsetAsync(r->d_bins, 0, std::max<uint64_t>(1, r->total_bins) * (N + 1) * 4, st));
-    HIP_TRY(hipMemsetAsync(r->d_colsums, 0, std::max<size_t>(1, r->ad.size()) * N * 8, st));
     HIP_TRY(launch_tile_reduce(st, fa, r->d_ad, r->d_tile_contig, r->ntiles, r->d_bins, r->d_colsums, (r->flags & PG_ANCHOR_COLSUMS) ? 1u : 0u));
     const uint32_t kflags = (r->flags & PG_ANCHOR_COLSUMS) | (r->lowres_step == 100 ? 0u : 2u);
     if (r->n_small)
@@ -2497,23 +2544,20 @@
     return std::binary_search(b.begin(), b.end(), t0) && std::binary_search(b.begin(), b.end(), t0 + nt);
 }
 
-static int run_chunks(pg_result *r, const TableDesc &T) {
+static int run_chunks(pg_result *r, const TableDesc &T, const TileRec *rec) {
     hipStream_t st = r->ctx->stream, aux = r->ctx->aux_stream;
     if (const char *e = getenv("PG_CHUNK_SAME_STREAM"); e && *e == '1') aux = st;
     const uint32_t N = r->N;
     const uint32_t kflags = (r->flags & PG_ANCHOR_COLSUMS) | (r->lowres_step == 100 ? 0u : 2u);
     HIP_TRY(hipEventRecord(r->ev[0], st));
+    if (int e = zero_statistics(r, aux)) return e;
     for (size_t c = 0; c < r->chunks.size(); ++c) {
         const pg_result::Chunk &ch = r->chunks[c];
-        HIP_TRY(launch_anchor(st, T, r->seqs->d_seqw, r->seqs->d_nmw, r->seqs->d_has_n, r->seqs->d_desc, r->d_ad, r->d_tile_contig,
+        HIP_TRY(launch_anchor(st, T, r->seqs->d_seqw, r->seqs->d_nmw, r->seqs->d_has_n, rec, r->d_ad, r->d_tile_contig,
                               r->d_sched, ch.s0, ch.s1 - ch.s0, r->d_out1, r->out1_bytes, 0));
         HIP_TRY(hipEventRecord(r->chunk_ev[c], st));
         HIP_TRY(hipStreamWaitEvent(aux, r->chunk_ev[c], 0));
-        if (c == 0) {
-            HIP_TRY(hipEventRecord(r->ev[2], aux));
-            HIP_TRY(hipMemsetAsync(r->d_bins, 0, std::max<uint64_t>(1, r->total_bins) * (N + 1) * 4, aux));
-            HIP_TRY(hipMemsetAsync(r->d_colsums, 0, std::max<size_t>(1, r->ad.size()) * N * 8, aux));
-        }
+        if (c == 0) HIP_TRY(hipEventRecord(r->ev[2], aux));
         HIP_TRY(launch_rows_epilogue(aux, N, r->d_ad, r->d_tile_contig, r->ntiles, r->d_out1, r->d_out100, r->d_bins, r->d_colsums,
                                      kflags, r->d_ranges + ch.r0, ch.nr, ch.tiles));
     }
@@ -2535,6 +2579,9 @@
     if (int e = join_result(r)) return e;
     if (int e = next_events(r, true)) return e;
     TableDesc T = make_desc(t);
+    const bool by_sched = sched_covers(r, tile_base, ntiles);
+    if (!by_sched && !r->d_rec_tile) HIP_TRY(build_tile_recs(r, nullptr, &r->d_rec_tile));
+    const TileRec *rec = by_sched ? r->d_rec_sched : r->d_rec_tile;
     const bool stats = whole && !columns_width && !(r->flags & PG_ANCHOR_ROWS_ONLY);
     bool fuse = false;
     if (stats && fuse_enabled()) {
@@ -2544,12 +2591,14 @@
     if (stats && !fuse) {
         if (!r->chunks_ready)
             if (int e = build_chunks(r, nullptr)) return e;
-        if (r->chunks.size() > 1) return run_chunks(r, T);
+        if (r->chunks.size() > 1) return run_chunks(r, T, rec);
     }
     const FuseArgs fa = fuse_args(r);
     HIP_TRY(hipEventRecord(r->ev[0], st));
-    HIP_TRY(launch_anchor(st, T, r->seqs->d_seqw, r->seqs->d_nmw, r->seqs->d_has_n, r->seqs->d_desc, r->d_ad,
-                          r->d_tile_contig, sched_covers(r, tile_base, ntiles) ? r->d_sched : nullptr, tile_base, ntiles,
+    if (stats)
+        if (int e = zero_statistics(r, aux)) return e;
+    HIP_TRY(launch_anchor(st, T, r->seqs->d_seqw, r->seqs->d_nmw, r->seqs->d_has_n, rec, r->d_ad,
+                          r->d_tile_contig, by_sched ? r->d_sched : nullptr, tile_base, ntiles,
                           columns_width ? static_cast<uint8_t *>(d_columns) : r->d_out1, r->out1_bytes, columns_width, fuse ? &fa : nullptr));
     HIP_TRY(hipEventRecord(r->ev[1], st));
     r->ev_ok = true;
@@ -2730,6 +2779,7 @@
     hipStream_t st = r->ctx->stream;
     if (int e = next_events(r, false)) return e;
     HIP_TRY(hipEventRecord(r->ev[0], st));
+    if (int e = zero_statistics(r, st)) return e;
     HIP_TRY(hipEventRecord(r->ev[1], st));
     HIP_TRY(hipEventRecord(r->ev[2], st));
     if (int e = enqueue_epilogue(r, st)) return e;
diff --git a/panagram_amd/csrc/pg_kernels.h b/panagram_amd/csrc/pg_kernels.h
--- a/panagram_amd/csrc/pg_kernels.h
+++ b/panagram_amd/csrc/pg_kernels.h
@@ -42,6 +42,16 @@
     uint32_t tile0;
     uint32_t nbins;
 };
+
+struct __attribute__((aligned(32))) TileRec {
+    uint64_t seq_word0;
+    uint64_t row_off;
+    uint32_t words_left;
+    uint32_t npos;
+    uint32_t tile;
+    uint32_t contig;
+};
+static_assert(sizeof(TileRec) == 32, "a tile record is one 32-byte scalar load");
 
 hipError_t launch_table_init(hipStream_t st, const SubTable &t);
 struct TextChunk {
@@ -113,7 +123,7 @@
 #endif
 constexpr bool fuse_rows_ok(uint32_t nbytes) { return nbytes >= 2u && nbytes <= (PG_FUSE_WIDE ? 16u : 8u); }
 hipError_t launch_anchor(hipStream_t st, const TableDesc &T, const uint64_t *seqw, const uint32_t *nmw,
-                         const uint32_t *has_n, const SeqDesc *sd, const AnchorDesc *ad,
+                         const uint32_t *has_n, const TileRec *rec, const AnchorDesc *ad,
                          const uint32_t *tile_contig, const uint32_t *sched, uint32_t tile_base, uint32_t ntiles, uint8_t *out1,
                          uint64_t out1_bytes, uint32_t columns_width = 0, const FuseArgs *fuse = nullptr);
 hipError_t launch_tile_reduce(hipStream_t st, const FuseArgs &fo, const AnchorDesc *ad, const uint32_t *tile_contig, uint32_t ntiles,
```

After: 237.3 billion (median of 6 runs). No clear change (+0.5%).
